# Spandan7724/Audio-Watermarking-Deep-Learning-Watermarks-for-Authenticating-Speech

Hardware: AMD Instinct MI355X
Metric: 1-s@16kHz clips/sec (gen+det+loss fwd-bwd) (higher is better)
Workload: dtype f32; 1 GPU; main16 train step: Generator+Detector+6 losses fwd-bwd + Adam, B=256 clips/GPU x 1 GPU, 1-s @ 16 kHz, message_bits=16 (BASELINE configs[2]); batch_per_gpu=256, global_batch=256, clip_len=16000, optimizer=fused flat Adam (wm_adam_step), parallelism=single

## Files before the change

### audio-watermarking-deep-learning-watermarks-for-authenticating-speech_amd/csrc/conv64.hpp

```cpp
#pragma once
#include "wm_common.hpp"
using namespace wm;
typedef _Float16 h16x2 __attribute__((ext_vector_type(2)));
typedef _Float16 h16x8 __attribute__((ext_vector_type(8)));
typedef float f32x2 __attribute__((ext_vector_type(2)));

#ifdef WM_STAMP
static __device__ unsigned long long* g_wm_stamp = nullptr;
#define STAMP(var) unsigned long long var = __builtin_amdgcn_s_memtime()
#define WM_STAMP_SETTER(name) int name(unsigned long long* buf) { return (int)hipMemcpyToSymbol(HIP_SYMBOL(g_wm_stamp), &buf, sizeof(buf)); }
#else
#define STAMP(var)
#define WM_STAMP_SETTER(name)
#endif

#ifndef WM_LOADPOS
#define WM_LOADPOS 1
#endif
#ifndef WM_LOAD_H
#define WM_LOAD_H 17
#endif
#ifndef WM_XCD_MAP
#define WM_XCD_MAP 1
#endif
#ifndef WM_TILE_CONTIG
#define WM_TILE_CONTIG 0
#endif
#ifndef WM_NT_STORE
#define WM_NT_STORE 0
#endif
#ifndef WM_BF3_MANUAL
#define WM_BF3_MANUAL 1
#endif
#ifndef WM_BF3_PIN_W
#define WM_BF3_PIN_W 1
#endif
#ifndef WM_BF7_PIPE
#define WM_BF7_PIPE 1
#endif
#ifndef WM_WGRAD_PIPE
#define WM_WGRAD_PIPE 1
#endif

namespace {
enum { PRO_NONE = 0, PRO_BNRELU = 1, PRO_ADDVEC = 2, PRO_BNBWD = 3 };
enum { EPI_BIAS = 0, EPI_RELUMASK = 1, EPI_ADD = 2, EPI_NONE = 3, EPI_BNADDRELU = 4,
       EPI_BIASELU = 5, EPI_BIASADDELU = 6, EPI_MULDELU = 7,
       EPI_ADDSTATS = 8 };

struct Conv64Args {
    const float* x;
    const float* x2;
    const float* wp;
    const float* pa;
    const float* pb;
    const float* pc;
    const float* bias;
    const float* e1;
    const float* ea;
    const float* eb;
    float* y;
    float* stats;
    int B, T;
};

template <int PRO>
__device__ __forceinline__ float pro_apply(float v, float v2, float ca, float cb, float cc, float cl = 0.f) {
    if (PRO == PRO_BNRELU) return fmaxf(fmaf(v, ca, cb), 0.f);
    if (PRO == PRO_ADDVEC) return v + ca;
    if (PRO == PRO_BNBWD) return fmaf(ca, v, fmaf(cc, v2, cb)) + cl;
    return v;
}

struct Wgrad64Args {
    const float* g;  const float* g2;
    const float* ga; const float* gb; const float* gc;
    const float* x;
    const float* xa; const float* xb;
    float* partial;
    int B, T;
};

__device__ __forceinline__ int xcd_slot() {
    const int g = gridDim.x, b = blockIdx.x;
    return (g & 7) ? b : (b & 7) * (g >> 3) + (b >> 3);
}

__device__ __forceinline__ void lds_barrier() {
    asm volatile("s_waitcnt lgkmcnt(0)\n\ts_barrier" ::: "memory");
}

__global__ __launch_bounds__(256) void wgrad64_reduce_kernel(const float* __restrict__ partial, int nparts, int KW, int mode,
                                                             float* __restrict__ dw, float* __restrict__ dbias, int accumulate) {
    __shared__ double sq[4][64];
    const int il = threadIdx.x & 63, grp = threadIdx.x >> 6, i = blockIdx.x * 64 + il;
    const int stride = KW * 4096 + 64;
    const int per = (nparts + 3) / 4, p0 = grp * per, p1 = min(p0 + per, nparts);
    double s0 = 0.0, s1 = 0.0;
    if (i < stride) {
        int p = p0;
        for (; p + 1 < p1; p += 2) {
            s0 += (double)partial[(size_t)p * stride + i];
            s1 += (double)partial[(size_t)(p + 1) * stride + i];
        }
        if (p < p1) s0 += (double)partial[(size_t)p * stride + i];
    }
    sq[grp][il] = s0 + s1;
    __syncthreads();
    if (grp != 0 || i >= stride) return;
    const float s = (float)((sq[0][il] + sq[1][il]) + (sq[2][il] + sq[3][il]));
    if (i < KW * 4096) {
        const int tap = i / 4096, out = (i / 64) % 64, in = i % 64;
        const int dst = (mode == 0) ? (out * 64 + in) * KW + tap : (in * 64 + out) * KW + (KW - 1 - tap);
        dw[dst] = accumulate ? dw[dst] + s : s;
    } else if (dbias) {
        const int c = i - KW * 4096;
        dbias[c] = accumulate ? dbias[c] + s : s;
    }
}
}
```

### audio-watermarking-deep-learning-watermarks-for-authenticating-speech_amd/csrc/conv64_fwd.hip

```cpp
#include "conv64.hpp"

namespace {

template <int PRO, int EPI, bool STATS>
__global__ __launch_bounds__(256) void conv64bf_kernel(Conv64Args a) {
    constexpr int KW = 3, PAD = 1, NT = 128, ROWS = NT + 2, PITCH = 72, NP = 3;
    constexpr int NC = 4;
    constexpr bool TWO = (PRO == PRO_BNBWD);
    constexpr bool E1 = (EPI == EPI_RELUMASK || EPI == EPI_ADD || EPI == EPI_BIASADDELU || EPI == EPI_MULDELU);
    constexpr bool HASBIAS = (EPI == EPI_BIAS || EPI == EPI_BIASELU || EPI == EPI_BIASADDELU);
    extern __shared__ __align__(16) unsigned char smem_raw[];
    unsigned short* Wb = reinterpret_cast<unsigned short*>(smem_raw);
    unsigned short* Xb = Wb + NP * KW * 64 * PITCH;
    float* Cs = reinterpret_cast<float*>(Xb + NP * ROWS * PITCH);
    const int tid = threadIdx.x, lane = tid & 63, wave = tid >> 6, half = lane >> 5, l31 = lane & 31;
    const int T = a.T;
    const int tilesPerClip = (T + NT - 1) / NT, ntiles = a.B * tilesPerClip;

    float4 sa[NC], sb[NC], sa2[TWO ? NC : 1], sb2[TWO ? NC : 1];
    float hl, hl2 = 0.f;
    auto combo = [&](int i, int& cp, int& q) {
        const int idx = tid + i * 256, widx = idx >> 6, l = idx & 63;
        cp = (widx & 3) * 8 + (l & 7);
        q = (widx >> 2) * 8 + (l >> 3);
// ... 61 lines not shown
    int tile = blockIdx.x;
    if (tile < ntiles) load_tile(tile);
    for (int i = tid; i < NP * KW * 64 * 8; i += 256) {
        const int row = i >> 3, seg = i & 7;
        *reinterpret_cast<uint4*>(Wb + row * PITCH + seg * 8) = reinterpret_cast<const uint4*>(a.wp)[i];
    }
    if (tid < 64) {
        Cs[tid] = (PRO == PRO_BNRELU || PRO == PRO_BNBWD) ? a.pa[tid] : 0.f;
        Cs[64 + tid] = (PRO == PRO_BNRELU || PRO == PRO_BNBWD) ? a.pb[tid] : 0.f;
        Cs[128 + tid] = (PRO == PRO_BNBWD) ? a.pc[tid] : 0.f;
        Cs[192 + tid] = (PRO == PRO_BNBWD) ? a.pb[64 + tid] : ((HASBIAS && a.bias) ? a.bias[tid] : 0.f);
        Cs[256 + tid] = (EPI == EPI_RELUMASK) ? a.ea[tid] : 0.f;
        Cs[320 + tid] = (EPI == EPI_RELUMASK) ? a.eb[tid] : 0.f;
    }
    __syncthreads();
    if (tile < ntiles) write_tile(tile);
    __syncthreads();

    float s1[STATS ? 32 : 1], s2[STATS ? 32 : 1];
    if (STATS) {
#pragma unroll
        for (int j = 0; j < 32; ++j) { s1[j] = 0.f; s2[j] = 0.f; }
    }
#ifdef WM_STAMP
    unsigned long long tm[6] = {0, 0, 0, 0, 0, 0};
#endif
    while (tile < ntiles) {
        STAMP(ts0);
        const int next = tile + gridDim.x;
        const int b = tile / tilesPerClip, t0 = (tile - b * tilesPerClip) * NT;
        const int tcol = t0 + wave * 32 + l31;
        float e1r[E1 ? 32 : 1];
        auto issue_loads = [&]() {
            if (next < ntiles) load_tile(next);
            if (E1) {
                const float* eb1 = a.e1 + (size_t)b * 64 * T + min(tcol, T - 1);
#pragma unroll
                for (int mt = 0; mt < 2; ++mt)
#pragma unroll
                    for (int r = 0; r < 16; ++r) e1r[mt * 16 + r] = eb1[(size_t)(mt * 32 + mfma_row(r, half)) * T];
            }
        };
        if (WM_LOADPOS == 0) issue_loads();
        STAMP(ts1);
        f32x16 acc[2];
#pragma unroll
        for (int mt = 0; mt < 2; ++mt)
#pragma unroll
            for (int r = 0; r < 16; ++r) acc[mt][r] = 0.f;
        const unsigned short* wbase = Wb + l31 * PITCH + 8 * half;
        const unsigned short* xbase = Xb + (wave * 32 + l31) * PITCH + 8 * half;
#pragma unroll 1
        for (int tap = 0; tap < KW; ++tap) {
            if (WM_LOADPOS > 0 && tap == WM_LOADPOS) issue_loads();
#pragma unroll
            for (int ch = 0; ch < 4; ++ch) {
                bf16x8 A[2][NP], Bf[NP];
#pragma unroll
                for (int p = 0; p < NP; ++p) {
                    Bf[p] = *reinterpret_cast<const bf16x8*>(xbase + (p * ROWS + tap) * PITCH + 16 * ch);
#pragma unroll
                    for (int mt = 0; mt < 2; ++mt)
                        A[mt][p] = *reinterpret_cast<const bf16x8*>(wbase + ((p * KW + tap) * 64 + mt * 32) * PITCH + 16 * ch);
                }
#pragma unroll
                for (int mt = 0; mt < 2; ++mt) {
                    acc[mt] = __builtin_amdgcn_mfma_f32_32x32x16_bf16(A[mt][1], Bf[1], acc[mt], 0, 0, 0);
                    acc[mt] = __builtin_amdgcn_mfma_f32_32x32x16_bf16(A[mt][0], Bf[2], acc[mt], 0, 0, 0);
                    acc[mt] = __builtin_amdgcn_mfma_f32_32x32x16_bf16(A[mt][2], Bf[0], acc[mt], 0, 0, 0);
                    acc[mt] = __builtin_amdgcn_mfma_f32_32x32x16_bf16(A[mt][0], Bf[1], acc[mt], 0, 0, 0);
                    acc[mt] = __builtin_amdgcn_mfma_f32_32x32x16_bf16(A[mt][1], Bf[0], acc[mt], 0, 0, 0);
                    acc[mt] = __builtin_amdgcn_mfma_f32_32x32x16_bf16(A[mt][0], Bf[0], acc[mt], 0, 0, 0);
                }
            }
        }
        STAMP(ts2);
        float* yb = a.y + (size_t)b * 64 * T + tcol;
        const bool ok = tcol < T;
#pragma unroll
        for (int mt = 0; mt < 2; ++mt)
#pragma unroll
            for (int r = 0; r < 16; ++r) {
                const int co = mt * 32 + mfma_row(r, half);
                float v = acc[mt][r];
                float q = 0.f;
                if (HASBIAS) v += Cs[192 + co];
                if (EPI == EPI_RELUMASK) { q = e1r[mt * 16 + r]; v = (fmaf(q, Cs[256 + co], Cs[320 + co]) > 0.f) ? v : 0.f; }
                if (EPI == EPI_ADD || EPI == EPI_BIASADDELU) v += e1r[mt * 16 + r];
                if (EPI == EPI_BIASELU || EPI == EPI_BIASADDELU) v = elu1(v);
                if (EPI == EPI_MULDELU) { const float yy = e1r[mt * 16 + r]; v *= (yy > 0.f ? 1.f : yy + 1.f); }
                if (ok) {
                    yb[(size_t)co * T] = v;
                    if (STATS) { s1[mt * 16 + r] += v; s2[mt * 16 + r] += (EPI == EPI_RELUMASK) ? v * q : v * v; }
                }
            }
        STAMP(ts3);
        __syncthreads();
        STAMP(ts4);
        if (next < ntiles) write_tile(next);
        STAMP(ts5);
        __syncthreads();
        STAMP(ts6);
#ifdef WM_STAMP
        tm[0] += ts1 - ts0; tm[1] += ts2 - ts1; tm[2] += ts3 - ts2; tm[3] += ts4 - ts3; tm[4] += ts5 - ts4; tm[5] += ts6 - ts5;
#endif
        tile = next;
    }
#ifdef WM_STAMP
    if (g_wm_stamp && lane == 0) {
        unsigned long long* d = g_wm_stamp + ((size_t)blockIdx.x * 4 + wave) * 6;
#pragma unroll
        for (int i = 0; i < 6; ++i) d[i] = tm[i];
    }
#endif
    if (STATS) {
        float* red = reinterpret_cast<float*>(Xb);
#pragma unroll
        for (int j = 0; j < 32; ++j) { s1[j] = half_wave_sum(s1[j]); s2[j] = half_wave_sum(s2[j]); }
        if (l31 == 0) {
#pragma unroll
            for (int mt = 0; mt < 2; ++mt)
#pragma unroll
                for (int r = 0; r < 16; ++r) {
                    const int co = mt * 32 + mfma_row(r, half);
                    red[wave * 128 + co] = s1[mt * 16 + r];
                    red[wave * 128 + 64 + co] = s2[mt * 16 + r];
                }
        }
        __syncthreads();
        if (tid < 128)
            a.stats[(size_t)blockIdx.x * 128 + tid] = red[tid] + red[128 + tid] + red[256 + tid] + red[384 + tid];
    }
}

template <int PRO, int EPI, bool STATS>
int launch_conv64bf(const Conv64Args& a, hipStream_t stream) {
    constexpr size_t lds = (size_t)(3 * 3 * 64 * 72 + 3 * 130 * 72) * 2 + 6 * 64 * sizeof(float);
    static wm::DevOnce attr_done;
    auto kern = conv64bf_kernel<PRO, EPI, STATS>;
    if (int rc = wm::lds_opt_in(reinterpret_cast<const void*>(kern), lds, attr_done)) return rc;
    const int ntiles = a.B * ((a.T + 127) / 128);
    const int grid = ntiles < kNumCU ? ntiles : kNumCU;
    if (STATS && grid < kNumCU) WM_TRY(hipMemsetAsync(a.stats, 0, sizeof(float) * 128 * kNumCU, stream));
    hipLaunchKernelGGL(kern, dim3(grid), dim3(256), lds, stream, a);
    WM_CHECK_LAUNCH();
    return 0;
}


template <int PRO, int EPI, bool STATS, bool H = false>
__global__ __launch_bounds__(256) void conv64bf3_kernel(Conv64Args a) {
    constexpr int KW = 3, NT = 128, ROWS = NT + 2, PITCH = 72, NP = H ? 2 : 3, NC = 4;
    constexpr int XBUF = NP * ROWS * PITCH;
    constexpr bool TWO = (PRO == PRO_BNBWD);
    constexpr bool E1 = (EPI == EPI_RELUMASK || EPI == EPI_ADD || EPI == EPI_BNADDRELU);
    extern __shared__ __align__(16) unsigned char smem_raw[];
    unsigned short* Xb0 = reinterpret_cast<unsigned short*>(smem_raw);
    float* Cs = reinterpret_cast<float*>(Xb0 + 2 * XBUF);
    const int tid = threadIdx.x, lane = tid & 63, half = lane >> 5, l31 = lane & 31;
    const int wave = __builtin_amdgcn_readfirstlane(tid >> 6);
    const int mt = wave & 1, nh = wave >> 1;
    const int T = a.T;
    const int tilesPerClip = (T + NT - 1) / NT, ntiles = a.B * tilesPerClip;

    u32x4 Wr[12][NP];
    {
        const uint4* wg = reinterpret_cast<const uint4*>(a.wp);
#pragma unroll
        for (int s = 0; s < 12; ++s)
#pragma unroll
            for (int p = 0; p < NP; ++p) {
                const int e = ((p * KW + (s >> 2)) * 64 + 32 * mt + l31) * 64 + 16 * (s & 3) + 8 * half;
                u32x4 w_ = __builtin_bit_cast(u32x4, wg[e >> 3]);
#if WM_BF3_PIN_W
                asm volatile("" : "+a"(w_));
#endif
                Wr[s][p] = w_;
            }
    }
    const float winv = H ? reinterpret_cast<const float*>(reinterpret_cast<const unsigned short*>(a.wp) + NP * KW * 4096)[1] : 1.f;
    const float wsc = H ? reinterpret_cast<const float*>(reinterpret_cast<const unsigned short*>(a.wp) + NP * KW * 4096)[0] : 1.f;
    const int cp = wave * 8 + (lane & 7), c0 = 2 * cp, q0 = lane >> 3;
    const int hc = (tid & 127) >> 1, hh = tid & 1;
    float4 sa[NC], sb[NC], sa2[TWO ? NC : 1], sb2[TWO ? NC : 1];
    float hl, hl2 = 0.f;
    auto load_combo = [&](int tile, int i) {
        const int b = tile / tilesPerClip, t0 = (tile - b * tilesPerClip) * NT;
        const size_t o = ((size_t)b * 64 + c0) * T + t0 + 4 * (q0 + 8 * i);
        sa[i] = *reinterpret_cast<const float4*>(a.x + o);
        sb[i] = *reinterpret_cast<const float4*>(a.x + o + T);
        if (TWO) { sa2[i] = *reinterpret_cast<const float4*>(a.x2 + o); sb2[i] = *reinterpret_cast<const float4*>(a.x2 + o + T); }
    };
    auto load_halo = [&](int tile) {
        const int b = tile / tilesPerClip, t0 = (tile - b * tilesPerClip) * NT;
        const int ht = min(max(hh ? t0 + NT : t0 - 1, 0), T - 1);
        hl = a.x[((size_t)b * 64 + hc) * T + ht];
        if (TWO) hl2 = a.x2[((size_t)b * 64 + hc) * T + ht];
    };
    auto load_tile = [&](int tile) {
#pragma unroll
        for (int i = 0; i < NC; ++i) load_combo(tile, i);
        load_halo(tile);
    };

#if WM_TILE_CONTIG
    const int chunk = (ntiles + (int)gridDim.x - 1) / (int)gridDim.x, tstep = 1;
    int tile = blockIdx.x * chunk;
    const int tend = min(tile + chunk, ntiles);
#else
    const int tstep = gridDim.x, tend = ntiles;
    int tile = WM_XCD_MAP ? xcd_slot() : (int)blockIdx.x;
#endif
    load_tile(min(tile, ntiles - 1));
    if (tid < 64) {
        Cs[tid] = (PRO == PRO_BNRELU || PRO == PRO_BNBWD) ? a.pa[tid] : 0.f;
        Cs[64 + tid] = (PRO == PRO_BNRELU || PRO == PRO_BNBWD) ? a.pb[tid] : 0.f;
        Cs[128 + tid] = (PRO == PRO_BNBWD) ? a.pc[tid] : 0.f;
        Cs[192 + tid] = (PRO == PRO_BNBWD) ? a.pb[64 + tid] : (((EPI == EPI_BIAS || EPI == EPI_BNADDRELU) && a.bias) ? a.bias[tid] : 0.f);
        Cs[256 + tid] = (EPI == EPI_RELUMASK || EPI == EPI_BNADDRELU) ? a.ea[tid] : 0.f;
        Cs[320 + tid] = (EPI == EPI_RELUMASK || EPI == EPI_BNADDRELU) ? a.eb[tid] : 0.f;
    }
    __syncthreads();
    const float ka0 = Cs[c0], ka1 = Cs[c0 + 1], kb0 = Cs[64 + c0], kb1 = Cs[64 + c0 + 1];
    const float kc0 = Cs[128 + c0], kc1 = Cs[128 + c0 + 1], kl0 = TWO ? Cs[192 + c0] : 0.f, kl1 = TWO ? Cs[192 + c0 + 1] : 0.f;
    const float ha = Cs[hc], hb = Cs[64 + hc], hcc = Cs[128 + hc], hlo = TWO ? Cs[192 + hc] : 0.f;

    auto split_unit = [&](unsigned* X32, int t0, int i, int e) {
        const float4 fa = sa[i], fb = sb[i];
        float va = (e == 0) ? fa.x : (e == 1) ? fa.y : (e == 2) ? fa.z : fa.w;
        float vb = (e == 0) ? fb.x : (e == 1) ? fb.y : (e == 2) ? fb.z : fb.w;
        if (PRO != PRO_NONE) {
            float wa = 0.f, wb = 0.f;
            if (TWO) {
                const float4 ga = sa2[i], gb = sb2[i];
                wa = (e == 0) ? ga.x : (e == 1) ? ga.y : (e == 2) ? ga.z : ga.w;
                wb = (e == 0) ? gb.x : (e == 1) ? gb.y : (e == 2) ? gb.z : gb.w;
            }
            va = pro_apply<PRO>(va, wa, ka0, kb0, kc0, kl0);
            vb = pro_apply<PRO>(vb, wb, ka1, kb1, kc1, kl1);
        }
        const int o = (1 + 4 * (q0 + 8 * i) + e) * (PITCH / 2) + cp;
        if (H) {
            const h16x2 h_ = __builtin_convertvector(f32x2{va, vb}, h16x2);
            const h16x2 l_ = __builtin_convertvector(f32x2{va - (float)h_.x, vb - (float)h_.y}, h16x2);
            X32[o] = __builtin_bit_cast(unsigned, h_); X32[(ROWS * PITCH >> 1) + o] = __builtin_bit_cast(unsigned, l_);
        } else {
            unsigned p0, p1, p2;
            split3_pair(va, vb, p0, p1, p2);
            X32[o] = p0; X32[(ROWS * PITCH >> 1) + o] = p1; X32[2 * (ROWS * PITCH >> 1) + o] = p2;
        }
    };
    auto split_halo = [&](unsigned short* X, int t0) {
        {
            const int t = hh ? t0 + NT : t0 - 1;
            float v = hl;
            if (PRO != PRO_NONE) v = pro_apply<PRO>(v, hl2, ha, hb, hcc, hlo);
            if (t < 0 || t >= T) v = 0.f;
            const int o = (hh ? NT + 1 : 0) * PITCH + hc;
            if (H) {
                const _Float16 h_ = (_Float16)v;
                const _Float16 l_ = (_Float16)(v - (float)h_);
                X[o] = __builtin_bit_cast(unsigned short, h_); X[ROWS * PITCH + o] = __builtin_bit_cast(unsigned short, l_);
            } else {
                unsigned p0, p1, p2;
                split3_pair(v, 0.f, p0, p1, p2);
                X[o] = (unsigned short)p0; X[ROWS * PITCH + o] = (unsigned short)p1; X[2 * ROWS * PITCH + o] = (unsigned short)p2;
            }
        }
    };
    float sva = 0.f, svb = 0.f;
    unsigned sp0 = 0, sp1 = 0;
    auto split_pick = [&](int i, int e) {
        const float4 fa = sa[i], fb = sb[i];
        float va = (e == 0) ? fa.x : (e == 1) ? fa.y : (e == 2) ? fa.z : fa.w;
        float vb = (e == 0) ? fb.x : (e == 1) ? fb.y : (e == 2) ? fb.z : fb.w;
        if (PRO != PRO_NONE) {
            float wa = 0.f, wb = 0.f;
            if (TWO) {
                const float4 ga = sa2[i], gb = sb2[i];
                wa = (e == 0) ? ga.x : (e == 1) ? ga.y : (e == 2) ? ga.z : ga.w;
                wb = (e == 0) ? gb.x : (e == 1) ? gb.y : (e == 2) ? gb.z : gb.w;
            }
            va = pro_apply<PRO>(va, wa, ka0, kb0, kc0, kl0);
            vb = pro_apply<PRO>(vb, wb, ka1, kb1, kc1, kl1);
        }
        sva = va; svb = vb;
        asm volatile("" : "+v"(sva), "+v"(svb));
    };
    auto split_st1 = [&]() {
        if (H) {
            const h16x2 hh_ = __builtin_convertvector(f32x2{sva, svb}, h16x2);
            sp0 = __builtin_bit_cast(unsigned, hh_);
            sva -= (float)hh_.x; svb -= (float)hh_.y;
        } else {
            const bf16x2 hh_ = {(__bf16)sva, (__bf16)svb};
            sp0 = __builtin_bit_cast(unsigned, hh_);
            sva -= __uint_as_float(sp0 << 16); svb -= __uint_as_float(sp0 & 0xffff0000u);
        }
        asm volatile("" : "+v"(sva), "+v"(svb), "+v"(sp0));
    };
    auto split_st2 = [&]() {
        if (H) return;
        const bf16x2 mm_ = {(__bf16)sva, (__bf16)svb};
        sp1 = __builtin_bit_cast(unsigned, mm_);
        sva -= __uint_as_float(sp1 << 16); svb -= __uint_as_float(sp1 & 0xffff0000u);
        asm volatile("" : "+v"(sva), "+v"(svb), "+v"(sp1));
    };
    auto last_piece = [&]() -> unsigned {
        if (H) return __builtin_bit_cast(unsigned, __builtin_convertvector(f32x2{sva, svb}, h16x2));
        const bf16x2 ll_ = {(__bf16)sva, (__bf16)svb};
        return __builtin_bit_cast(unsigned, ll_);
    };
    auto split_out = [&](unsigned* X32, int i, int e) {
        const unsigned sp2 = last_piece();
        const int o = (1 + 4 * (q0 + 8 * i) + e) * (PITCH / 2) + cp;
        X32[o] = sp0; if (!H) X32[(ROWS * PITCH >> 1) + o] = sp1; X32[(NP - 1) * (ROWS * PITCH >> 1) + o] = sp2;
    };
    auto halo_pick = [&](int t0) {
        const int t = hh ? t0 + NT : t0 - 1;
        float v = hl;
        if (PRO != PRO_NONE) v = pro_apply<PRO>(v, hl2, ha, hb, hcc, hlo);
        if (t < 0 || t >= T) v = 0.f;
        sva = v; svb = 0.f;
        asm volatile("" : "+v"(sva), "+v"(svb));
    };
    auto halo_out = [&](unsigned short* X) {
        const unsigned sp2 = last_piece();
        const int o = (hh ? NT + 1 : 0) * PITCH + hc;
        X[o] = (unsigned short)sp0; if (!H) X[ROWS * PITCH + o] = (unsigned short)sp1; X[(NP - 1) * ROWS * PITCH + o] = (unsigned short)sp2;
    };
    {
        const int t0 = (min(tile, ntiles - 1) % tilesPerClip) * NT;
#pragma unroll
        for (int u = 0; u < 16; ++u) split_unit(reinterpret_cast<unsigned*>(Xb0), t0, u >> 2, u & 3);
        split_halo(Xb0, t0);
    }
    load_tile(min(tile + tstep, ntiles - 1));
    __syncthreads();
    __builtin_amdgcn_s_waitcnt(0x0F70);

    float s1[STATS ? 16 : 1], s2[STATS ? 16 : 1];
    if (STATS) {
#pragma unroll
        for (int j = 0; j < 16; ++j) { s1[j] = 0.f; s2[j] = 0.f; }
    }
    int buf = 0;
#ifdef WM_STAMP
    unsigned long long tm[6] = {0, 0, 0, 0, 0, 0};
#endif
    f32x16 accp[2];
    int pb_ = min(tile, ntiles - 1) / tilesPerClip, pt0 = (min(tile, ntiles - 1) % tilesPerClip) * NT;
    bool any_tile = false;
    float e1r[E1 ? 32 : 1];
    constexpr bool KB = (EPI == EPI_BIAS || EPI == EPI_BNADDRELU), KE = (EPI == EPI_RELUMASK || EPI == EPI_BNADDRELU);
    float kbias[KB ? 16 : 1], kea[KE ? 16 : 1], keb[KE ? 16 : 1];
#pragma unroll
    for (int r = 0; r < 16; ++r) {
        const int co = 32 * mt + mfma_row(r, half);
        if (KB) kbias[r] = Cs[192 + co];
        if (KE) { kea[r] = Cs[256 + co]; keb[r] = Cs[320 + co]; }
    }
#pragma unroll
    for (int nt = 0; nt < 2; ++nt)
#pragma unroll
        for (int r = 0; r < 16; ++r) accp[nt][r] = (EPI == EPI_BIAS) ? -kbias[r] * wsc : 0.f;
    const unsigned lcol = (unsigned)(4 * half * T + l31) * 4u;
    unsigned rowT[16];
#pragma unroll
    for (int r = 0; r < 16; ++r) rowT[r] = (unsigned)(((r & 3) + 8 * (r >> 2)) * T) * 4u;
    auto row_srd = [&](const float* base, int cb) { return make_srd(base + ((size_t)cb * 64 + 32 * mt) * T, (size_t)32 * T * sizeof(float)); };
    wm_srd_t syp = row_srd(a.y, pb_);
    unsigned vcolp = lcol + (unsigned)(pt0 + 64 * nh) * 4u;
    if (E1) {
#pragma unroll
        for (int j = 0; j < 32; ++j) e1r[j] = 0.f;
    }
    auto epi_value = [&](int idx, bool fetch, const wm_srd_t& se1c, unsigned vcolc) {
        const int nt = idx >> 4, r = idx & 15;
        float v = accp[nt][r];
        float q = 0.f;
        if (H) v *= winv;
        if (EPI == EPI_BIAS) v += kbias[r];
        if (EPI == EPI_RELUMASK) { q = e1r[idx]; v = (fmaf(q, kea[r], keb[r]) > 0.f) ? v : 0.f; }
        if (EPI == EPI_ADD) v += e1r[idx];
        if (EPI == EPI_BNADDRELU) v = fmaxf(e1r[idx] + fmaf(v + kbias[r], kea[r], keb[r]), 0.f);
        buf_store(syp, v, vcolp + 128u * nt, rowT[r]);
        if (STATS) { s1[r] += v; s2[r] = fmaf(v, (EPI == EPI_RELUMASK) ? q : v, s2[r]); }
#if WM_BF3_MANUAL
        if (STATS) asm volatile("" : "+v"(s1[r]), "+v"(s2[r]));
#endif
        if (E1 && fetch) e1r[idx] = buf_load(se1c, vcolc + 128u * nt, rowT[r]);
    };
    auto mma = [&](const u32x4& A_, const u32x4& B_, f32x16 c) -> f32x16 {
        if (H) return __builtin_amdgcn_mfma_f32_32x32x16_f16(__builtin_bit_cast(h16x8, A_), __builtin_bit_cast(h16x8, B_), c, 0, 0, 0);
        return __builtin_amdgcn_mfma_f32_32x32x16_bf16(__builtin_bit_cast(bf16x8, A_), __builtin_bit_cast(bf16x8, B_), c, 0, 0, 0);
    };
    while (tile < tend) {
        STAMP(ts0);
        const int next = min(tile + tstep, ntiles - 1), next2 = min(tile + 2 * tstep, ntiles - 1);
        const int b = tile / tilesPerClip, t0 = (tile - b * tilesPerClip) * NT;
        const int nt0 = (next % tilesPerClip) * NT;
        const wm_srd_t se1c = E1 ? row_srd(a.e1, b) : syp;
        const unsigned vcolc = lcol + (unsigned)(t0 + 64 * nh) * 4u;
        const unsigned short* xcur = Xb0 + buf * XBUF;
        unsigned short* xnxt = Xb0 + (buf ^ 1) * XBUF;
        f32x16 acc[2];
#pragma unroll
        for (int nt = 0; nt < 2; ++nt)
#pragma unroll
            for (int r = 0; r < 16; ++r) acc[nt][r] = 0.f;
        const unsigned short* xrow = xcur + (64 * nh + l31) * PITCH + 8 * half;
        u32x4 Bq[2][NP];
#pragma unroll
        for (int p = 0; p < NP; ++p) Bq[0][p] = *reinterpret_cast<const u32x4*>(xrow + p * ROWS * PITCH);
#if WM_BF3_MANUAL
#define FENCE __builtin_amdgcn_sched_barrier(0)
#define BF3_SLICE(k)                                                                                                        \
    {                                                                                                                           \
        if (h < 16) {                                                                                                           \
            if ((k) == 0) split_pick(h >> 2, h & 3);                                                                            \
            if ((k) == 1) split_st1();                                                                                          \
            if ((k) == 2) split_st2();                                                                                          \
            if ((k) == 3) { split_out(reinterpret_cast<unsigned*>(xnxt), h >> 2, h & 3); if ((h & 3) == 3) load_combo(next2, h >> 2); } \
        } else if (h == 16) {                                                                                                   \
            if ((k) == 0) halo_pick(nt0);                                                                                       \
            if ((k) == 1) split_st1();                                                                                          \
            if ((k) == 2) split_st2();                                                                                          \
            if ((k) == 3) halo_out(xnxt);                                                                                       \
        } else if (h == 17) {                                                                                                   \
            if ((k) == 0) load_halo(next2);                                                                                     \
        }                                                                                                                       \
        if (h < 8) {                                                                                                            \
            if ((k) == 4) epi_value(2 * h, true, se1c, vcolc);                                                                              \
            if ((k) == 5) epi_value(2 * h + 1, true, se1c, vcolc);                                                                          \
        } else if ((k) == 4) epi_value(8 + h, true, se1c, vcolc);                                                                           \
    }
#pragma unroll
        for (int h = 0; h < 24; ++h) {
            const int s = h >> 1, nt = h & 1;
            if (h + 1 < 24) {
                const int s1_ = (h + 1) >> 1, n1 = (h + 1) & 1;
#pragma unroll
                for (int p = 0; p < NP; ++p)
                    Bq[(h + 1) & 1][p] = *reinterpret_cast<const u32x4*>(xrow + (p * ROWS + 32 * n1 + (s1_ >> 2)) * PITCH + 16 * (s1_ & 3));
            }
            const u32x4* Bf = Bq[h & 1];
            FENCE;
            if (H) {
                acc[nt] = mma(Wr[s][1], Bf[0], acc[nt]); FENCE; BF3_SLICE(0) FENCE; BF3_SLICE(1) FENCE;
                acc[nt] = mma(Wr[s][0], Bf[1], acc[nt]); FENCE; BF3_SLICE(3) FENCE; BF3_SLICE(4) FENCE;
                acc[nt] = mma(Wr[s][0], Bf[0], acc[nt]); FENCE; BF3_SLICE(5) FENCE;
            } else {
                acc[nt] = mma(Wr[s][1], Bf[1], acc[nt]); FENCE; BF3_SLICE(0) FENCE;
                acc[nt] = mma(Wr[s][0], Bf[2], acc[nt]); FENCE; BF3_SLICE(1) FENCE;
                acc[nt] = mma(Wr[s][2], Bf[0], acc[nt]); FENCE; BF3_SLICE(2) FENCE;
                acc[nt] = mma(Wr[s][0], Bf[1], acc[nt]); FENCE; BF3_SLICE(3) FENCE;
                acc[nt] = mma(Wr[s][1], Bf[0], acc[nt]); FENCE; BF3_SLICE(4) FENCE;
                acc[nt] = mma(Wr[s][0], Bf[0], acc[nt]); FENCE; BF3_SLICE(5) FENCE;
            }
#ifdef WM_STAMP
#ifdef WM_STAMP_FINE
            if (h == 16) { STAMP(tsa); tm[0] += tsa - ts0; }
            if (h == 17) { STAMP(tsb); tm[1] += tsb - ts0; }
            if (h == 18) { STAMP(tsb); tm[3] += tsb - ts0; }
            if (h == 20) { STAMP(tsb); tm[5] += tsb - ts0; }
#else
            if (h == 3) { STAMP(tsa); tm[0] += tsa - ts0; }
            if (h == 15) { STAMP(tsb); tm[1] += tsb - ts0; }
#endif
#endif
        }
#undef FENCE
#undef BF3_SLICE
#else
#pragma unroll
        for (int h = 0; h < 24; ++h) {
            const int s = h >> 1, nt = h & 1;
            if (h + 1 < 24) {
                const int s1_ = (h + 1) >> 1, n1 = (h + 1) & 1;
#pragma unroll
                for (int p = 0; p < NP; ++p)
                    Bq[(h + 1) & 1][p] = *reinterpret_cast<const u32x4*>(xrow + (p * ROWS + 32 * n1 + (s1_ >> 2)) * PITCH + 16 * (s1_ & 3));
            }
            const u32x4* Bf = Bq[h & 1];
            static_assert(!H, "the f16 build exists in the hand-pinned schedule only");
            acc[nt] = mma(Wr[s][1], Bf[1], acc[nt]);
            acc[nt] = mma(Wr[s][0], Bf[2], acc[nt]);
            acc[nt] = mma(Wr[s][2], Bf[0], acc[nt]);
            acc[nt] = mma(Wr[s][0], Bf[1], acc[nt]);
            acc[nt] = mma(Wr[s][1], Bf[0], acc[nt]);
            acc[nt] = mma(Wr[s][0], Bf[0], acc[nt]);
            if (h < 16) {
                split_unit(reinterpret_cast<unsigned*>(xnxt), nt0, h >> 2, h & 3);
                if ((h & 3) == 3) load_combo(next2, h >> 2);
            } else if (h == 16) split_halo(xnxt, nt0);
            else if (h == 17) load_halo(next2);
            if (h < 8) { epi_value(2 * h, true, se1c, vcolc); epi_value(2 * h + 1, true, se1c, vcolc); }
            else epi_value(8 + h, true, se1c, vcolc);
            __builtin_amdgcn_sched_group_barrier(0x100, 3, 0);
#pragma unroll
            for (int kk = 0; kk < 6; ++kk) {
                __builtin_amdgcn_sched_group_barrier(0x008, 1, 0);
                __builtin_amdgcn_sched_group_barrier(0x002, 5, 0);
                __builtin_amdgcn_sched_group_barrier(0x200, 1, 0);
                __builtin_amdgcn_sched_group_barrier(0x020, 1, 0);
                __builtin_amdgcn_sched_group_barrier(0x040, 1, 0);
            }
            __builtin_amdgcn_sched_barrier(0);
#ifdef WM_STAMP
#ifdef WM_STAMP_FINE
            if (h == 16) { STAMP(tsa); tm[0] += tsa - ts0; }
            if (h == 17) { STAMP(tsb); tm[1] += tsb - ts0; }
            if (h == 18) { STAMP(tsb); tm[3] += tsb - ts0; }
            if (h == 20) { STAMP(tsb); tm[5] += tsb - ts0; }
#else
            if (h == 3) { STAMP(tsa); tm[0] += tsa - ts0; }
            if (h == 15) { STAMP(tsb); tm[1] += tsb - ts0; }
#endif
#endif
        }
#endif
        STAMP(ts1);
        accp[0] = acc[0]; accp[1] = acc[1];
        pb_ = b; pt0 = t0; any_tile = true;
        syp = row_srd(a.y, b); vcolp = vcolc;
        STAMP(ts2);
        lds_barrier();
        STAMP(ts3);
#ifdef WM_STAMP
#ifdef WM_STAMP_FINE
        tm[2] += ts1 - ts0; tm[4] += ts3 - ts2;
#else
        tm[2] += ts1 - ts0; tm[3] += ts2 - ts1; tm[4] += ts3 - ts2;
#endif
#endif
        tile += tstep;
        buf ^= 1;
    }
#ifdef WM_STAMP
    if (g_wm_stamp && lane == 0) {
        unsigned long long* d = g_wm_stamp + ((size_t)blockIdx.x * 4 + wave) * 6;
#pragma unroll
        for (int i = 0; i < 6; ++i) d[i] = tm[i];
    }
#endif
    if (any_tile) {
#pragma unroll
        for (int idx = 0; idx < 32; ++idx) epi_value(idx, false, syp, 0u);
    }
    if (STATS) {
        float* red = reinterpret_cast<float*>(Xb0);
#pragma unroll
        for (int j = 0; j < 16; ++j) { s1[j] = half_wave_sum(s1[j]); s2[j] = half_wave_sum(s2[j]); }
        __syncthreads();
        if (l31 == 0) {
#pragma unroll
            for (int r = 0; r < 16; ++r) {
                const int co = 32 * mt + mfma_row(r, half);
                red[nh * 128 + co] = s1[r];
                red[nh * 128 + 64 + co] = s2[r];
            }
        }
        __syncthreads();
        if (tid < 128) a.stats[(size_t)blockIdx.x * 128 + tid] = red[tid] + red[128 + tid];
    }
}

template <int PRO, int EPI, bool STATS, bool H = false>
int launch_conv64bf3(const Conv64Args& a, hipStream_t stream) {
    constexpr size_t lds = (size_t)(2 * (H ? 2 : 3) * 130 * 72) * 2 + 6 * 64 * sizeof(float);
    static wm::DevOnce attr_done;
    auto kern = conv64bf3_kernel<PRO, EPI, STATS, H>;
    if (int rc = wm::lds_opt_in(reinterpret_cast<const void*>(kern), lds, attr_done)) return rc;
    const int ntiles = a.B * ((a.T + 127) / 128);
    const int grid = ntiles < kNumCU ? ntiles : kNumCU;
    if (STATS && grid < kNumCU) WM_TRY(hipMemsetAsync(a.stats, 0, sizeof(float) * 128 * kNumCU, stream));
    hipLaunchKernelGGL(kern, dim3(grid), dim3(256), lds, stream, a);
    WM_CHECK_LAUNCH();
    return 0;
}

__global__ void pack_w64_bf_kernel(const float* __restrict__ w, const float* __restrict__ row_scale,
                                   unsigned short* __restrict__ wpb, int mode) {
    const int i = blockIdx.x * blockDim.x + threadIdx.x;
    if (i >= 3 * 4096) return;
    const int tap = i / 4096, out = (i / 64) % 64, in = i % 64;
    float v = (mode == 0) ? w[(out * 64 + in) * 3 + tap] : w[(in * 64 + out) * 3 + (2 - tap)];
    if (row_scale) v *= row_scale[out];
    unsigned p0, p1, p2;
    split3_pair(v, 0.f, p0, p1, p2);
    wpb[i] = (unsigned short)p0; wpb[3 * 4096 + i] = (unsigned short)p1; wpb[2 * 3 * 4096 + i] = (unsigned short)p2;
}

__global__ __launch_bounds__(1024) void pack_w64_h_kernel(const float* __restrict__ w, const float* __restrict__ row_scale,
                                                          unsigned short* __restrict__ wph, int mode) {
    __shared__ float red[16];
    float v[12];
    float mx = 0.f;
#pragma unroll
    for (int j = 0; j < 12; ++j) {
        const int i = threadIdx.x + 1024 * j, tap = i / 4096, out = (i / 64) % 64, in = i % 64;
        v[j] = (mode == 0) ? w[(out * 64 + in) * 3 + tap] : w[(in * 64 + out) * 3 + (2 - tap)];
        if (row_scale) v[j] *= row_scale[out];
        mx = fmaxf(mx, fabsf(v[j]));
    }
#pragma unroll
    for (int o = 32; o > 0; o >>= 1) mx = fmaxf(mx, __shfl_xor(mx, o));
    if ((threadIdx.x & 63) == 0) red[threadIdx.x >> 6] = mx;
    __syncthreads();
    float m = 0.f;
#pragma unroll
    for (int i = 0; i < 16; ++i) m = fmaxf(m, red[i]);
    float ws = 1.f;
    if (m > 0.f && m < 3.0e38f) ws = exp2f(floorf(log2f(1023.f / m)));
    ws = fminf(fmaxf(ws, 1.0e-30f), 1.0e30f);
    if (threadIdx.x == 0) {
        float* tail = reinterpret_cast<float*>(wph + 2 * 3 * 4096);
        tail[0] = ws; tail[1] = 1.f / ws;
    }
#pragma unroll
    for (int j = 0; j < 12; ++j) {
        const int i = threadIdx.x + 1024 * j;
        const float x = v[j] * ws;
        const _Float16 hi = (_Float16)x;
        const _Float16 lo = (_Float16)(x - (float)hi);
        wph[i] = __builtin_bit_cast(unsigned short, hi);
        wph[3 * 4096 + i] = __builtin_bit_cast(unsigned short, lo);
    }
}

}

extern "C" {

WM_STAMP_SETTER(wm_debug_set_stamp_buffer)

int wm_pack_w64_bf(const float* w, void* wpb, int mode, hipStream_t stream) {
    if (mode < 0 || mode > 1) return (int)hipErrorInvalidValue;
    hipLaunchKernelGGL(pack_w64_bf_kernel, dim3(48), dim3(256), 0, stream, w, (const float*)nullptr, reinterpret_cast<unsigned short*>(wpb), mode);
    WM_CHECK_LAUNCH();
    return 0;
}
int wm_pack_w64_bf_scaled(const float* w, const float* row_scale, void* wpb, hipStream_t stream) {
    if (!w || !row_scale || !wpb) return (int)hipErrorInvalidValue;
    hipLaunchKernelGGL(pack_w64_bf_kernel, dim3(48), dim3(256), 0, stream, w, row_scale, reinterpret_cast<unsigned short*>(wpb), 0);
    WM_CHECK_LAUNCH();
    return 0;
}

static int g_bf_schedule = 2;
int wm_set_conv_bf_schedule(int schedule, hipStream_t) { g_bf_schedule = (schedule == 2) ? 2 : 0; return 0; }

int wm_conv64_bf(const float* x, const float* x2, const void* wpb, const float* pa, const float* pb, const float* pc,
                 const float* bias, const float* e1, const float* ea, const float* eb, float* y, float* stats,
                 int B, int T, int pro, int epi, int arith, hipStream_t stream) {
    if (B <= 0 || T <= 0 || (T & 3)) return (int)hipErrorInvalidValue;
    Conv64Args a{x, x2, reinterpret_cast<const float*>(wpb), pa, pb, pc, bias, e1, ea, eb, y, stats, B, T};
    const bool st = stats != nullptr;
    if (arith == 1) {
        if (g_bf_schedule != 2 || (T & 127)) return (int)hipErrorInvalidValue;
        if (pro == PRO_BNRELU && epi == EPI_BNADDRELU && !st) return launch_conv64bf3<PRO_BNRELU, EPI_BNADDRELU, false, true>(a, stream);
        if (epi != EPI_BIAS) return (int)hipErrorInvalidValue;
        if (pro == PRO_NONE) return st ? launch_conv64bf3<PRO_NONE, EPI_BIAS, true, true>(a, stream) : launch_conv64bf3<PRO_NONE, EPI_BIAS, false, true>(a, stream);
        if (pro == PRO_BNRELU) return st ? launch_conv64bf3<PRO_BNRELU, EPI_BIAS, true, true>(a, stream) : launch_conv64bf3<PRO_BNRELU, EPI_BIAS, false, true>(a, stream);
        return (int)hipErrorInvalidValue;
    }
    if (arith != 0) return (int)hipErrorInvalidValue;
    if (pro == PRO_NONE && !st) {
        if (epi == EPI_BIASELU) return launch_conv64bf<PRO_NONE, EPI_BIASELU, false>(a, stream);
        if (epi == EPI_BIASADDELU) return launch_conv64bf<PRO_NONE, EPI_BIASADDELU, false>(a, stream);
        if (epi == EPI_MULDELU) return launch_conv64bf<PRO_NONE, EPI_MULDELU, false>(a, stream);
        if (epi == EPI_ADD) return launch_conv64bf<PRO_NONE, EPI_ADD, false>(a, stream);
        if (epi == EPI_NONE) return launch_conv64bf<PRO_NONE, EPI_NONE, false>(a, stream);
    }
    if (g_bf_schedule == 2 && (T & 127) == 0) {
        if (pro == PRO_BNRELU && epi == EPI_BNADDRELU && !st) return launch_conv64bf3<PRO_BNRELU, EPI_BNADDRELU, false>(a, stream);
        if (pro == PRO_NONE && epi == EPI_BIAS) return st ? launch_conv64bf3<PRO_NONE, EPI_BIAS, true>(a, stream) : launch_conv64bf3<PRO_NONE, EPI_BIAS, false>(a, stream);
        if (pro == PRO_BNRELU && epi == EPI_BIAS) return st ? launch_conv64bf3<PRO_BNRELU, EPI_BIAS, true>(a, stream) : launch_conv64bf3<PRO_BNRELU, EPI_BIAS, false>(a, stream);
        if (pro == PRO_BNBWD && epi == EPI_RELUMASK && st) return launch_conv64bf3<PRO_BNBWD, EPI_RELUMASK, true>(a, stream);
        if (pro == PRO_BNBWD && epi == EPI_ADD && !st) return launch_conv64bf3<PRO_BNBWD, EPI_ADD, false>(a, stream);
        if (pro == PRO_BNBWD && epi == EPI_NONE && !st) return launch_conv64bf3<PRO_BNBWD, EPI_NONE, false>(a, stream);
        return (int)hipErrorInvalidValue;
    }
    if (pro == PRO_NONE && epi == EPI_BIAS) return st ? launch_conv64bf<PRO_NONE, EPI_BIAS, true>(a, stream) : launch_conv64bf<PRO_NONE, EPI_BIAS, false>(a, stream);
    if (pro == PRO_BNRELU && epi == EPI_BIAS) return st ? launch_conv64bf<PRO_BNRELU, EPI_BIAS, true>(a, stream) : launch_conv64bf<PRO_BNRELU, EPI_BIAS, false>(a, stream);
    if (pro == PRO_BNBWD && epi == EPI_RELUMASK && st) return launch_conv64bf<PRO_BNBWD, EPI_RELUMASK, true>(a, stream);
    if (pro == PRO_BNBWD && epi == EPI_ADD && !st) return launch_conv64bf<PRO_BNBWD, EPI_ADD, false>(a, stream);
    if (pro == PRO_BNBWD && epi == EPI_NONE && !st) return launch_conv64bf<PRO_BNBWD, EPI_NONE, false>(a, stream);
    return (int)hipErrorInvalidValue;
}

int wm_pack_w64_h(const float* w, void* wph, int mode, hipStream_t stream) {
    if (!w || !wph || mode < 0 || mode > 1) return (int)hipErrorInvalidValue;
    hipLaunchKernelGGL(pack_w64_h_kernel, dim3(1), dim3(1024), 0, stream, w, (const float*)nullptr, reinterpret_cast<unsigned short*>(wph), mode);
    WM_CHECK_LAUNCH();
    return 0;
}
int wm_pack_w64_h_scaled(const float* w, const float* row_scale, void* wph, hipStream_t stream) {
    if (!w || !row_scale || !wph) return (int)hipErrorInvalidValue;
    hipLaunchKernelGGL(pack_w64_h_kernel, dim3(1), dim3(1024), 0, stream, w, row_scale, reinterpret_cast<unsigned short*>(wph), 0);
    WM_CHECK_LAUNCH();
    return 0;
}

}
```

### audio-watermarking-deep-learning-watermarks-for-authenticating-speech_amd/csrc/lstm.hip

```cpp
#include "wm_common.hpp"
#include <type_traits>
using namespace wm;

namespace {

#ifdef WM_STAMP
__device__ unsigned long long* g_lstm_stamp = nullptr;
#define LSTAMP(var, val) unsigned long long var; asm volatile("s_memtime %0\n\ts_waitcnt lgkmcnt(0)" : "=s"(var), "+v"(val))
#define LSTAMP_ACC(i, a, b) tm[i] += (b) - (a)
#else
#define LSTAMP(var, val)
#define LSTAMP_ACC(i, a, b)
#endif

__device__ __forceinline__ int gate_row(int np) { return (np & 3) * 64 + (np >> 2); }

typedef float v2f __attribute__((ext_vector_type(2)));
template <int K>
__device__ __forceinline__ float quad_bcast(float v) {
    constexpr int ctrl = K | (K << 2) | (K << 4) | (K << 6);
    return __int_as_float(__builtin_amdgcn_update_dpp(0, __float_as_int(v), ctrl, 0xf, 0xf, false));
}

__global__ __launch_bounds__(256) void lstm_xproj_kernel(const float* __restrict__ x, const float* __restrict__ w_ih,
// ... 230 lines not shown
    const int q = lane & 3, ul = lane >> 2, u = wave * 16 + ul, n = q * 64 + u, np = wave * 64 + lane;
    float wr[64];
#pragma unroll
    for (int k = 0; k < 64; k += 4) {
        const float4 v = *reinterpret_cast<const float4*>(w_hh + n * 64 + k);
        wr[k] = v.x; wr[k + 1] = v.y; wr[k + 2] = v.z; wr[k + 3] = v.w;
    }
    bf16x8 Wi[2][4][NP];
#pragma unroll
    for (int mt = 0; mt < 2; ++mt)
#pragma unroll
        for (int ks = 0; ks < 4; ++ks) {
            const float* wp = w_ih + gate_row(wave * 64 + mt * 32 + l31) * 64 + 16 * ks + 8 * half;
            const float4 v0 = *reinterpret_cast<const float4*>(wp), v1 = *reinterpret_cast<const float4*>(wp + 4);
            unsigned a[4], m[4], l[4];
            split3_pair(v0.x, v0.y, a[0], m[0], l[0]); split3_pair(v0.z, v0.w, a[1], m[1], l[1]);
            split3_pair(v1.x, v1.y, a[2], m[2], l[2]); split3_pair(v1.z, v1.w, a[3], m[3], l[3]);
            Wi[mt][ks][0] = __builtin_bit_cast(bf16x8, make_uint4(a[0], a[1], a[2], a[3]));
            Wi[mt][ks][1] = __builtin_bit_cast(bf16x8, make_uint4(m[0], m[1], m[2], m[3]));
            Wi[mt][ks][2] = __builtin_bit_cast(bf16x8, make_uint4(l[0], l[1], l[2], l[3]));
        }
    const float bias = b_ih[n] + b_hh[n];
    if (tid < 128) hsm[tid] = 0.f;
    float c = 0.f;
    const wm_srd_t sgb = make_srd(SAVE ? gates + (size_t)b * T * 256 : hout, SAVE ? (size_t)T * 256 * sizeof(float) : 0);
    const wm_srd_t scb = make_srd(SAVE ? cst + (size_t)b * T * 64 : hout, SAVE ? (size_t)T * 64 * sizeof(float) : 0);
    const wm_srd_t shb = make_srd(hout + (size_t)b * 64 * T, (size_t)64 * T * sizeof(float));
    const unsigned vgb = (unsigned)np * 4u, vcb = (q == 1) ? (unsigned)u * 4u : 0xFFFFFF00u;
    const unsigned vhb = (unsigned)(u * T + 4 * q) * 4u;
    float* hb = hout + ((size_t)b * 64 + u) * T;
    const bool is_g = (q == 2);

    const int cp = wave * 8 + (lane & 7), tq = lane >> 3;
    const float* xc = x + ((size_t)b * 64 + 2 * cp) * T + 4 * tq;
    float4 sa, sb;
    auto load_x = [&](int t0) {
        const int t = min(t0, T - 4 - 4 * tq);
        sa = *reinterpret_cast<const float4*>(xc + max(t, -4 * tq));
        sb = *reinterpret_cast<const float4*>(xc + T + max(t, -4 * tq));
    };
    auto split_x = [&]() {
        unsigned* X32 = reinterpret_cast<unsigned*>(Xb);
        const float va[4] = {sa.x, sa.y, sa.z, sa.w}, vb[4] = {sb.x, sb.y, sb.z, sb.w};
#pragma unroll
        for (int e = 0; e < 4; ++e) {
            unsigned p0, p1, p2;
            split3_pair(va[e], vb[e], p0, p1, p2);
            const int o = (4 * tq + e) * (PITCH / 2) + cp;
            X32[o] = p0; X32[CH * PITCH / 2 + o] = p1; X32[2 * (CH * PITCH / 2) + o] = p2;
        }
    };
    f32x16 acc[2];
    bf16x8 Bf[NP];
    auto mfma_one = [&](int idx) {
        const int m = idx / 6, pr = idx % 6, ks = m >> 1, mt = m & 1;
        const int pa = (pr == 0 || pr == 4) ? 1 : (pr == 2 ? 2 : 0), pb = (pr == 0 || pr == 3) ? 1 : (pr == 1 ? 2 : 0);
        if (mt == 0 && pr == 0) {
#pragma unroll
            for (int p = 0; p < NP; ++p) Bf[p] = *reinterpret_cast<const bf16x8*>(Xb + (p * CH + l31) * PITCH + 16 * ks + 8 * half);
        }
        if (ks == 0 && pr == 0) {
#pragma unroll
            for (int r = 0; r < 16; ++r) acc[mt][r] = 0.f;
        }
        acc[mt] = __builtin_amdgcn_mfma_f32_32x32x16_bf16(Wi[mt][ks][pa], Bf[pb], acc[mt], 0, 0, 0);
    };
    auto store_xp = [&](int buf) {
        float* dst = xps + (buf * CH + l31) * XPP + wave * 64 + 4 * half;
#pragma unroll
        for (int mt = 0; mt < 2; ++mt)
#pragma unroll
            for (int r = 0; r < 16; ++r) dst[mt * 32 + (r & 3) + 8 * (r >> 2)] = acc[mt][r];
    };

    load_x(0);
    __syncthreads();
    split_x();
    load_x(CH);
    __syncthreads();
#pragma unroll
    for (int i = 0; i < 48; ++i) mfma_one(i);
    store_xp(0);
    __syncthreads();

    float hk[4];
    int t0 = 0, cbuf = 0;
#ifdef WM_STAMP
    unsigned long long tm[6] = {0, 0, 0, 0, 0, 0};
#endif
    auto run8 = [&](auto sub_c) {
        constexpr int SUB = decltype(sub_c)::value;
#pragma unroll
        for (int j8 = 0; j8 < 8; ++j8) {
            const int s = SUB * 8 + j8;
            const int t = t0 + s;
            if (s == 0) { split_x(); load_x(t0 + 2 * CH); }
            if (s >= 2 && s < 26) mfma_one(2 * (s - 2));
            if (s == 28) store_xp(cbuf ^ 1);
            if (t < T) {
                LSTAMP(ls0, c);
                const float xin = xps[(cbuf * CH + s) * XPP + np] + bias;
                const float* hcur = hsm + (s & 1) * 64;
                const float4 hq4 = *reinterpret_cast<const float4*>(hcur + 4 * (lane & 15));
                float Hh[4] = {hq4.x, hq4.y, hq4.z, hq4.w};
                float hv = Hh[0];
                LSTAMP(ls1, hv);
                Hh[0] = hv;
                if (s >= 2 && s < 26) mfma_one(2 * (s - 2) + 1);
                float pre = dot64_rowbcast(Hh, wr, xin);
                LSTAMP(ls2, pre);
                float act = gate_act(pre, is_g);
                LSTAMP(ls3, act);
                const float gi = quad_bcast<0>(act), gf = quad_bcast<1>(act), gg = quad_bcast<2>(act), go = quad_bcast<3>(act);
                c = fmaf(gf, c, gi * gg);
                float h = go * tanh_s(c);
                LSTAMP(ls4, h);
                hsm[((s + 1) & 1) * 64 + rowbcast_slot(u)] = h;
                if (SAVE) {
                    buf_store(sgb, act, vgb, (unsigned)t * 1024u);
                    buf_store(scb, c, vcb, (unsigned)t * 256u);
                }
                if (((s >> 2) & 3) == q) hk[s & 3] = h;
                if ((s & 15) == 15)
                    buf_store4(shb, f32x4{hk[0], hk[1], hk[2], hk[3]}, vhb, (unsigned)(t0 + (s - 15)) * 4u);
                LSTAMP(ls5, h);
                __syncthreads();
                LSTAMP(ls6, c);
                LSTAMP_ACC(0, ls0, ls1); LSTAMP_ACC(1, ls1, ls2); LSTAMP_ACC(2, ls2, ls3); LSTAMP_ACC(3, ls3, ls4);
                LSTAMP_ACC(4, ls4, ls5); LSTAMP_ACC(5, ls5, ls6);
            }
        }
    };
    for (; t0 < T; t0 += CH, cbuf ^= 1) {
        run8(std::integral_constant<int, 0>{});
        run8(std::integral_constant<int, 1>{});
        run8(std::integral_constant<int, 2>{});
        run8(std::integral_constant<int, 3>{});
        if (t0 + CH > T && (T & 15)) {
            const int g0 = (T >> 4) << 4, tq0 = g0 + 4 * q;
#pragma unroll
            for (int j = 0; j < 4; ++j)
                if (tq0 + j < T) hb[tq0 + j] = hk[j];
        }
    }
#ifdef WM_STAMP
    if (g_lstm_stamp && lane == 0) {
        unsigned long long* d = g_lstm_stamp + ((size_t)blockIdx.x * 4 + wave) * 6;
#pragma unroll
        for (int i = 0; i < 6; ++i) d[i] = tm[i];
    }
#endif
}

template <bool SAVE>
__global__ __launch_bounds__(512) void lstm_fwd_ws_kernel(const float* __restrict__ x, const float* __restrict__ w_ih,
                                                          const float* __restrict__ b_ih, const float* __restrict__ b_hh,
                                                          const float* __restrict__ w_hh, float* __restrict__ hout,
                                                          float* __restrict__ gates, float* __restrict__ cst, int T) {
    constexpr int CH = 32, XPP = 257, PITCH = 72, NP = 3;
    extern __shared__ __align__(16) unsigned char smem_raw[];
    float* xps = reinterpret_cast<float*>(smem_raw);
    unsigned short* Xb = reinterpret_cast<unsigned short*>(xps + 2 * CH * XPP);
    float* hsm = reinterpret_cast<float*>(Xb + NP * CH * PITCH);
    const int b = blockIdx.x, tid = threadIdx.x, lane = tid & 63, half = lane >> 5, l31 = lane & 31;
    const int wave = __builtin_amdgcn_readfirstlane(tid >> 6);
    if (wave < 4) {
        __builtin_amdgcn_s_setprio(3);
        const int q = lane & 3, ul = lane >> 2, u = wave * 16 + ul, n = q * 64 + u, np = wave * 64 + lane;
        float wr[64];
#pragma unroll
        for (int k = 0; k < 64; k += 4) {
            const float4 v = *reinterpret_cast<const float4*>(w_hh + n * 64 + k);
            wr[k] = v.x; wr[k + 1] = v.y; wr[k + 2] = v.z; wr[k + 3] = v.w;
        }
        const float bias = b_ih[n] + b_hh[n];
        if (tid < 128) hsm[tid] = 0.f;
        float c = 0.f;
        const wm_srd_t sgb = make_srd(SAVE ? gates + (size_t)b * T * 256 : hout, SAVE ? (size_t)T * 256 * sizeof(float) : 0);
        const wm_srd_t scb = make_srd(SAVE ? cst + (size_t)b * T * 64 : hout, SAVE ? (size_t)T * 64 * sizeof(float) : 0);
        const wm_srd_t shb = make_srd(hout + (size_t)b * 64 * T, (size_t)64 * T * sizeof(float));
        const unsigned vgb = (unsigned)np * 4u, vcb = (q == 1) ? (unsigned)u * 4u : 0xFFFFFF00u;
        const unsigned vhb = (unsigned)(u * T + 4 * q) * 4u;
        float* hb = hout + ((size_t)b * 64 + u) * T;
        const bool is_g = (q == 2);
        __syncthreads(); __syncthreads(); __syncthreads();
        float hk[4];
        int t0 = 0, cbuf = 0;
        auto run8 = [&](auto sub_c) {
            constexpr int SUB = decltype(sub_c)::value;
#pragma unroll
            for (int j8 = 0; j8 < 8; ++j8) {
                const int s = SUB * 8 + j8;
                const int t = t0 + s;
                if (t < T) {
                    const float xin = xps[(cbuf * CH + s) * XPP + np] + bias;
                    const float* hcur = hsm + (s & 1) * 64;
                    const float4 hq4 = *reinterpret_cast<const float4*>(hcur + 4 * (lane & 15));
                    const float Hh[4] = {hq4.x, hq4.y, hq4.z, hq4.w};
                    const float pre = dot64_rowbcast(Hh, wr, xin);
                    const float act = gate_act(pre, is_g);
                    const float gi = quad_bcast<0>(act), gf = quad_bcast<1>(act), gg = quad_bcast<2>(act), go = quad_bcast<3>(act);
                    c = fmaf(gf, c, gi * gg);
                    const float h = go * tanh_s(c);
                    hsm[((s + 1) & 1) * 64 + rowbcast_slot(u)] = h;
                    if (SAVE) {
                        buf_store(sgb, act, vgb, (unsigned)t * 1024u);
                        buf_store(scb, c, vcb, (unsigned)t * 256u);
                    }
                    if (((s >> 2) & 3) == q) hk[s & 3] = h;
                    if ((s & 15) == 15)
                        buf_store4(shb, f32x4{hk[0], hk[1], hk[2], hk[3]}, vhb, (unsigned)(t0 + (s - 15)) * 4u);
                    __syncthreads();
                }
            }
        };
        for (; t0 < T; t0 += CH, cbuf ^= 1) {
            run8(std::integral_constant<int, 0>{});
            run8(std::integral_constant<int, 1>{});
            run8(std::integral_constant<int, 2>{});
            run8(std::integral_constant<int, 3>{});
            if (t0 + CH > T && (T & 15)) {
                const int g0 = (T >> 4) << 4, tq0 = g0 + 4 * q;
#pragma unroll
                for (int j = 0; j < 4; ++j)
                    if (tq0 + j < T) hb[tq0 + j] = hk[j];
            }
        }
        return;
    }
    const int hw = wave - 4;
    bf16x8 Wi[2][4][NP];
#pragma unroll
    for (int mt = 0; mt < 2; ++mt)
#pragma unroll
        for (int ks = 0; ks < 4; ++ks) {
            const float* wp = w_ih + gate_row(hw * 64 + mt * 32 + l31) * 64 + 16 * ks + 8 * half;
            const float4 v0 = *reinterpret_cast<const float4*>(wp), v1 = *reinterpret_cast<const float4*>(wp + 4);
            unsigned a[4], m[4], l[4];
            split3_pair(v0.x, v0.y, a[0], m[0], l[0]); split3_pair(v0.z, v0.w, a[1], m[1], l[1]);
            split3_pair(v1.x, v1.y, a[2], m[2], l[2]); split3_pair(v1.z, v1.w, a[3], m[3], l[3]);
            Wi[mt][ks][0] = __builtin_bit_cast(bf16x8, make_uint4(a[0], a[1], a[2], a[3]));
            Wi[mt][ks][1] = __builtin_bit_cast(bf16x8, make_uint4(m[0], m[1], m[2], m[3]));
            Wi[mt][ks][2] = __builtin_bit_cast(bf16x8, make_uint4(l[0], l[1], l[2], l[3]));
        }
    const int cp = hw * 8 + (lane & 7), tq = lane >> 3;
    const float* xc = x + ((size_t)b * 64 + 2 * cp) * T + 4 * tq;
    float4 sa, sb;
    auto load_x = [&](int t0) {
        const int t = min(t0, T - 4 - 4 * tq);
        sa = *reinterpret_cast<const float4*>(xc + max(t, -4 * tq));
        sb = *reinterpret_cast<const float4*>(xc + T + max(t, -4 * tq));
    };
    auto split_x = [&]() {
        unsigned* X32 = reinterpret_cast<unsigned*>(Xb);
        const float va[4] = {sa.x, sa.y, sa.z, sa.w}, vb[4] = {sb.x, sb.y, sb.z, sb.w};
#pragma unroll
        for (int e = 0; e < 4; ++e) {
            unsigned p0, p1, p2;
            split3_pair(va[e], vb[e], p0, p1, p2);
            const int o = (4 * tq + e) * (PITCH / 2) + cp;
            X32[o] = p0; X32[CH * PITCH / 2 + o] = p1; X32[2 * (CH * PITCH / 2) + o] = p2;
        }
    };
    f32x16 acc[2];
    bf16x8 Bf[NP];
    auto mfma_one = [&](int idx) {
        const int m = idx / 6, pr = idx % 6, ks = m >> 1, mt = m & 1;
        const int pa = (pr == 0 || pr == 4) ? 1 : (pr == 2 ? 2 : 0), pb = (pr == 0 || pr == 3) ? 1 : (pr == 1 ? 2 : 0);
        if (mt == 0 && pr == 0) {
#pragma unroll
            for (int p = 0; p < NP; ++p) Bf[p] = *reinterpret_cast<const bf16x8*>(Xb + (p * CH + l31) * PITCH + 16 * ks + 8 * half);
        }
        if (ks == 0 && pr == 0) {
#pragma unroll
            for (int r = 0; r < 16; ++r) acc[mt][r] = 0.f;
        }
        acc[mt] = __builtin_amdgcn_mfma_f32_32x32x16_bf16(Wi[mt][ks][pa], Bf[pb], acc[mt], 0, 0, 0);
    };
    auto store_xp = [&](int buf) {
        float* dst = xps + (buf * CH + l31) * XPP + hw * 64 + 4 * half;
#pragma unroll
        for (int mt = 0; mt < 2; ++mt)
#pragma unroll
            for (int r = 0; r < 16; ++r) dst[mt * 32 + (r & 3) + 8 * (r >> 2)] = acc[mt][r];
    };
    load_x(0);
    __syncthreads();
    split_x();
    load_x(CH);
    __syncthreads();
#pragma unroll
    for (int i = 0; i < 48; ++i) mfma_one(i);
    store_xp(0);
    __syncthreads();
    int cbuf = 0;
    for (int t0 = 0; t0 < T; t0 += CH, cbuf ^= 1) {
#pragma unroll
        for (int s = 0; s < CH; ++s) {
            if (s == 0) { split_x(); load_x(t0 + 2 * CH); }
            if (s >= 1 && s <= 24) { mfma_one(2 * (s - 1)); mfma_one(2 * (s - 1) + 1); }
            if (s == 26) store_xp(cbuf ^ 1);
            if (t0 + s < T) __syncthreads();
        }
    }
}

__global__ __launch_bounds__(256) void lstm_bwd_kernel(float* __restrict__ gates, const float* __restrict__ cst,
                                                       const float* __restrict__ dh_out, const float* __restrict__ w_hh,
                                                       int T) {
    __builtin_amdgcn_s_setprio(3);
    __shared__ __align__(16) float part[2][64][4];
    const int b = blockIdx.x, tid = threadIdx.x, lane = tid & 63, wave = tid >> 6;
    const int q = lane & 3, ul = lane >> 2, u = wave * 16 + ul, np = wave * 64 + lane;
    float wt[64];
#pragma unroll
    for (int j = 0; j < 64; ++j) wt[j] = w_hh[((j & 3) * 64 + wave * 16 + (j >> 2)) * 64 + lane];
    if (tid < 512 / 4) reinterpret_cast<float4*>(&part[0][0][0])[tid] = make_float4(0.f, 0.f, 0.f, 0.f);
    float dc = 0.f;
    const wm_srd_t sgb = make_srd(gates + (size_t)b * T * 256, (size_t)T * 256 * sizeof(float));
    const wm_srd_t scb = make_srd(cst + (size_t)b * T * 64, (size_t)T * 64 * sizeof(float));
    const wm_srd_t sdh = make_srd(dh_out + (size_t)b * 64 * T, (size_t)64 * T * sizeof(float));
    const unsigned vgb = (unsigned)np * 4u, vcb = (unsigned)u * 4u, vdh = (unsigned)(u * T) * 4u;

    constexpr int CH = 8;
    struct Buf { float ga[CH], cc[CH + 1], dh[CH]; };
    Buf A, Bf;
    auto prefetch = [&](Buf& f, int t1) {
#pragma unroll
        for (int j = 0; j < CH; ++j) {
            const int t = max(t1 - CH + 1 + j, 0);
            f.ga[j] = buf_load(sgb, vgb, (unsigned)t * 1024u);
            f.dh[j] = buf_load(sdh, vdh, (unsigned)t * 4u);
        }
#pragma unroll
        for (int j = 0; j <= CH; ++j) f.cc[j] = buf_load(scb, vcb, (unsigned)max(t1 - CH + j, 0) * 256u);
    };
    const bool is0 = q == 0, is1 = q == 1, is2 = q == 2, is3 = q == 3;
    int pb = 0;
#ifdef WM_STAMP
    unsigned long long tm[6] = {0, 0, 0, 0, 0, 0};
#endif
    auto run_chunk = [&](const Buf& f, int t1) {
#pragma unroll
        for (int jj = 0; jj < CH; ++jj) {
            const int j = CH - 1 - jj, t = t1 - jj;
            if (t >= 0) {
                LSTAMP(ls0, dc);
                const float4 p = *reinterpret_cast<const float4*>(&part[pb][u][0]);
                const float act = f.ga[j];
                const float gi = quad_bcast<0>(act), gf = quad_bcast<1>(act), gg = quad_bcast<2>(act), go = quad_bcast<3>(act);
                const float tc = tanh_s(f.cc[j + 1]);
                const float cprev = (t >= 1) ? f.cc[j] : 0.f;
                const float S = is0 ? gg : (is1 ? cprev : (is2 ? gi : tc));
                const float D = is2 ? fmaf(-act, act, 1.f) : act * (1.f - act);
                const float M = S * D;
                const float K = go * fmaf(-tc, tc, 1.f);
                float dht = f.dh[j] + ((p.x + p.y) + (p.z + p.w));
                LSTAMP(ls1, dht);
                const float dct = fmaf(dht, K, dc);
                float da = (is3 ? dht : dct) * M;
                dc = dct * gf;
                LSTAMP(ls2, da);
                buf_store(sgb, da, vgb, (unsigned)t * 1024u);
                float Dd[4];
                rows_replicate(da, Dd);
                float psum = dot64_rowbcast(Dd, wt);
                LSTAMP(ls3, psum);
                part[pb ^ 1][lane][wave] = psum;
                pb ^= 1;
                LSTAMP(ls4, psum);
                __syncthreads();
                LSTAMP(ls5, dc);
                LSTAMP_ACC(0, ls0, ls1); LSTAMP_ACC(1, ls1, ls2); LSTAMP_ACC(2, ls2, ls3); LSTAMP_ACC(3, ls3, ls4); LSTAMP_ACC(4, ls4, ls5);
            }
        }
    };
    prefetch(A, T - 1);
    __syncthreads();
    for (int t1 = T - 1; t1 >= 0; t1 -= 2 * CH) {
        prefetch(Bf, t1 - CH);
        run_chunk(A, t1);
        prefetch(A, t1 - 2 * CH);
        run_chunk(Bf, t1 - CH);
    }
#ifdef WM_STAMP
    if (g_lstm_stamp && lane == 0) {
        unsigned long long* d = g_lstm_stamp + ((size_t)blockIdx.x * 4 + wave) * 6;
#pragma unroll
        for (int i = 0; i < 6; ++i) d[i] = tm[i];
    }
#endif
}

__global__ __launch_bounds__(512) void lstm_bwd_ws_kernel(float* __restrict__ gates, const float* __restrict__ cst,
                                                          const float* __restrict__ dh_out, const float* __restrict__ w_hh,
                                                          const float* __restrict__ x, const float* __restrict__ hseq,
                                                          float* __restrict__ partial, int T) {
    constexpr int CT = 32, PT = 36;
    extern __shared__ __align__(16) unsigned char smem_raw[];
    float* daT = reinterpret_cast<float*>(smem_raw);
    float (*part)[64][4] = reinterpret_cast<float (*)[64][4]>(daT + 2 * 256 * PT);
    const int b = blockIdx.x, tid = threadIdx.x, lane = tid & 63;
    const int wave = __builtin_amdgcn_readfirstlane(tid >> 6);
    float* out = partial + (size_t)b * (256 * 128 + 256);
    if (wave < 4) {
        __builtin_amdgcn_s_setprio(3);
        const int q = lane & 3, ul = lane >> 2, u = wave * 16 + ul, np = wave * 64 + lane;
        float wt[64];
#pragma unroll
        for (int j = 0; j < 64; ++j) wt[j] = w_hh[((j & 3) * 64 + wave * 16 + (j >> 2)) * 64 + lane];
        if (tid < 512 / 4) reinterpret_cast<float4*>(&part[0][0][0])[tid] = make_float4(0.f, 0.f, 0.f, 0.f);
        float dc = 0.f, dbs = 0.f;
        const wm_srd_t sgb = make_srd(gates + (size_t)b * T * 256, (size_t)T * 256 * sizeof(float));
        const wm_srd_t scb = make_srd(cst + (size_t)b * T * 64, (size_t)T * 64 * sizeof(float));
        const wm_srd_t sdh = make_srd(dh_out + (size_t)b * 64 * T, (size_t)64 * T * sizeof(float));
        const unsigned vgb = (unsigned)np * 4u, vcb = (unsigned)u * 4u, vdh = (unsigned)(u * T) * 4u;
        constexpr int CH = 8;
        struct Buf { float ga[CH], cc[CH + 1], dh[CH]; };
        Buf A, Bf;
        auto prefetch = [&](Buf& f, int t1) {
#pragma unroll
            for (int j = 0; j < CH; ++j) {
                const int t = max(t1 - CH + 1 + j, 0);
                f.ga[j] = buf_load(sgb, vgb, (unsigned)t * 1024u);
                f.dh[j] = buf_load(sdh, vdh, (unsigned)t * 4u);
            }
#pragma unroll
            for (int j = 0; j <= CH; ++j) f.cc[j] = buf_load(scb, vcb, (unsigned)max(t1 - CH + j, 0) * 256u);
        };
        const bool is0 = q == 0, is1 = q == 1, is2 = q == 2, is3 = q == 3;
        int pb = 0;
        auto run_chunk = [&](const Buf& f, int t1) {
            float dav[CH];
#pragma unroll
            for (int jj = 0; jj < CH; ++jj) {
                const int j = CH - 1 - jj, t = t1 - jj;
                const float4 p = *reinterpret_cast<const float4*>(&part[pb][u][0]);
                const float act = f.ga[j];
                const float gi = quad_bcast<0>(act), gf = quad_bcast<1>(act), gg = quad_bcast<2>(act), go = quad_bcast<3>(act);
                const float tc = tanh_s(f.cc[j + 1]);
                const float cprev = (t >= 1) ? f.cc[j] : 0.f;
                const float S = is0 ? gg : (is1 ? cprev : (is2 ? gi : tc));
                const float D = is2 ? fmaf(-act, act, 1.f) : act * (1.f - act);
                const float M = S * D;
                const float K = go * fmaf(-tc, tc, 1.f);
                const float dht = f.dh[j] + ((p.x + p.y) + (p.z + p.w));
                const float dct = fmaf(dht, K, dc);
                const float da = (is3 ? dht : dct) * M;
                dc = dct * gf;
                dav[j] = da;
                buf_store(sgb, da, vgb, (unsigned)t * 1024u);
                float Dd[4];
                rows_replicate(da, Dd);
                const float psum = dot64_rowbcast(Dd, wt);
// ... 537 lines not shown
        } else {
            const int k = p & 1, i = tid + k * 256, j = i >> 3, q = i & 7;
            const size_t row = ((size_t)b * 64 + j) * T;
            if (p < 10) sx[k] = *reinterpret_cast<const float4*>(x + row + min(t0 + 4 * q, T - 4));
            else {
#pragma unroll
                for (int e = 0; e < 4; ++e) sh[k][e] = h[row + min(max(t0 + 4 * q + e - 1, 0), T - 1)];
            }
        }
    };
    auto put4 = [&](unsigned short* d, int stride_p, float v0, float v1, float v2, float v3) {
        unsigned a0, a1, a2, b0, b1, b2;
        split3_pair(v0, v1, a0, a1, a2);
        split3_pair(v2, v3, b0, b1, b2);
        *reinterpret_cast<uint2*>(d) = make_uint2(a0, b0);
        *reinterpret_cast<uint2*>(d + stride_p) = make_uint2(a1, b1);
        *reinterpret_cast<uint2*>(d + 2 * stride_p) = make_uint2(a2, b2);
    };
    auto write_tile = [&](int tile) {
        const int t0 = (tile % tilesPerClip) * NT;
#pragma unroll
        for (int p = 0; p < 8; ++p) {
            const int tt = (tid >> 6) + 4 * p;
            float4 v = sd[p];
            if (t0 + tt >= T) v = make_float4(0.f, 0.f, 0.f, 0.f);
            bs[0] += v.x; bs[1] += v.y; bs[2] += v.z; bs[3] += v.w;
            put4(Dd + tt * PDD + 4 * (tid & 63), NT * PDD, v.x, v.y, v.z, v.w);
        }
#pragma unroll
        for (int k = 0; k < 2; ++k) {
            const int i = tid + k * 256, j = i >> 3, q = i & 7;
            put4(Zb + j * PZ + 4 * q, 128 * PZ, sx[k].x, sx[k].y, sx[k].z, sx[k].w);
            float hv[4];
#pragma unroll
            for (int e = 0; e < 4; ++e) hv[e] = (t0 + 4 * q + e - 1 >= 0) ? sh[k][e] : 0.f;
            put4(Zb + (64 + j) * PZ + 4 * q, 128 * PZ, hv[0], hv[1], hv[2], hv[3]);
        }
    };
    int tile = blockIdx.x;
#pragma unroll
    for (int p = 0; p < 12; ++p) load_piece(min(tile, ntiles - 1), p);
    __syncthreads();
    write_tile(min(tile, ntiles - 1));
    __syncthreads();
    while (tile < ntiles) {
        const int next = tile + gridDim.x, nextc = min(next, ntiles - 1);
#pragma unroll
        for (int kb = 0; kb < 2; ++kb) {
            const int e0 = kb * 16 + 8 * half;
            bf16x8 Bf[4][NP];
#pragma unroll
            for (int nt = 0; nt < 4; ++nt)
#pragma unroll
                for (int p = 0; p < NP; ++p)
                    Bf[nt][p] = *reinterpret_cast<const bf16x8*>(Zb + (p * 128 + nt * 32 + l31) * PZ + e0);
#pragma unroll
            for (int mt = 0; mt < 2; ++mt) {
                bf16x8 A[NP];
#pragma unroll
                for (int p = 0; p < NP; ++p) {
                    const unsigned short* col = Dd + (p * NT + e0) * PDD + wave * 64 + mt * 32 + l31;
                    unsigned w[4];
#pragma unroll
                    for (int j = 0; j < 4; ++j) w[j] = (unsigned)col[(2 * j) * PDD] | ((unsigned)col[(2 * j + 1) * PDD] << 16);
                    A[p] = __builtin_bit_cast(bf16x8, make_uint4(w[0], w[1], w[2], w[3]));
                }
#pragma unroll
                for (int nt = 0; nt < 4; ++nt) {
                    acc[mt][nt] = mfma_bf16x6(A, Bf[nt], acc[mt][nt]);
                    if ((kb * 2 + mt) * 4 + nt < 12) load_piece(nextc, (kb * 2 + mt) * 4 + nt);
                }
            }
        }
        __syncthreads();
        if (next < ntiles) write_tile(next);
        __syncthreads();
        tile = next;
    }
    float* out = partial + (size_t)blockIdx.x * (256 * 128 + 256);
#pragma unroll
    for (int mt = 0; mt < 2; ++mt)
#pragma unroll
        for (int nt = 0; nt < 4; ++nt)
#pragma unroll
            for (int r = 0; r < 16; ++r)
                out[(wave * 64 + mt * 32 + mfma_row(r, half)) * 128 + nt * 32 + l31] = acc[mt][nt][r];
    float* red = reinterpret_cast<float*>(smem_raw);
    __syncthreads();
#pragma unroll
    for (int e = 0; e < 4; ++e) red[(tid >> 6) * 256 + 4 * (tid & 63) + e] = bs[e];
    __syncthreads();
    out[256 * 128 + tid] = (red[tid] + red[256 + tid]) + (red[512 + tid] + red[768 + tid]);
}

constexpr int kWgradSlab = 256 * 128 + 256;
__global__ __launch_bounds__(512) void lstm_wgrad_reduce_kernel(const float* __restrict__ partial, int nparts, float* dw_ih,
                                                                float* dw_hh, float* db_ih, float* db_hh, int accumulate) {
    __shared__ double sq[8][64];
    const int i = blockIdx.x * 64 + (threadIdx.x & 63);
    const float s = (float)column_sum_d<8>(partial, nparts, (size_t)kWgradSlab, i, true, sq);
    if (threadIdx.x >= 64) return;
    if (i < 256 * 128) {
        const int n = gate_row(i >> 7), j = i & 127;
        float* dst = (j < 64) ? dw_ih + n * 64 + j : dw_hh + n * 64 + (j - 64);
        *dst = accumulate ? *dst + s : s;
    } else {
        const int n = gate_row(i - 256 * 128);
        db_ih[n] = accumulate ? db_ih[n] + s : s;
        db_hh[n] = accumulate ? db_hh[n] + s : s;
    }
}
static_assert(kWgradSlab % 64 == 0, "lstm_wgrad_reduce_kernel: whole 64-column blocks");

}

extern "C" {

#ifdef WM_STAMP
int wm_debug_set_lstm_stamp_buffer(unsigned long long* buf) {
    return (int)hipMemcpyToSymbol(HIP_SYMBOL(g_lstm_stamp), &buf, sizeof(buf));
}
#endif

int wm_lstm_xproj(const float* x, const float* w_ih, const float* b_ih, const float* b_hh, float* xp, int B, int T,
                  hipStream_t stream) {
    if (T & 3) return (int)hipErrorInvalidValue;
    hipLaunchKernelGGL(lstm_xproj_kernel, dim3(B * ((T + 127) / 128)), dim3(256), 0, stream, x, w_ih, b_ih, b_hh, xp, T);
    WM_CHECK_LAUNCH();
    return 0;
}

int wm_lstm_fwd(const float* xp, const float* w_hh, float* hout, float* gates, float* cst, int B, int T, hipStream_t stream) {
    if (T & 3) return (int)hipErrorInvalidValue;
    if (gates && cst) hipLaunchKernelGGL(lstm_fwd_kernel<true>, dim3(B), dim3(256), 0, stream, xp, w_hh, hout, gates, cst, T);
    else hipLaunchKernelGGL(lstm_fwd_kernel<false>, dim3(B), dim3(256), 0, stream, xp, w_hh, hout, gates, cst, T);
    WM_CHECK_LAUNCH();
    return 0;
}

static int g_lstm_fwd_ws = 1;
int wm_set_lstm_fwd_wave_specialised(int on, hipStream_t) { g_lstm_fwd_ws = on ? 1 : 0; return 0; }

int wm_lstm_fwd_fused(const float* x, const float* w_ih, const float* b_ih, const float* b_hh, const float* w_hh, float* hout,
                      float* gates, float* cst, int B, int T, hipStream_t stream) {
    if ((T & 3) || T < 8) return (int)hipErrorInvalidValue;
    constexpr size_t lds = (size_t)2 * 32 * 257 * sizeof(float) + (size_t)3 * 32 * 72 * 2 + 128 * sizeof(float);
    static wm::DevOnce done[2];
    if (int rc = wm::lds_opt_in(reinterpret_cast<const void*>(lstm_fwd_fused_kernel<true>), lds, done[0])) return rc;
    if (int rc = wm::lds_opt_in(reinterpret_cast<const void*>(lstm_fwd_fused_kernel<false>), lds, done[1])) return rc;
    if (g_lstm_fwd_ws) {
        static wm::DevOnce donew[2];
        if (int rc = wm::lds_opt_in(reinterpret_cast<const void*>(lstm_fwd_ws_kernel<true>), lds, donew[0])) return rc;
        if (int rc = wm::lds_opt_in(reinterpret_cast<const void*>(lstm_fwd_ws_kernel<false>), lds, donew[1])) return rc;
        if (gates && cst) hipLaunchKernelGGL(lstm_fwd_ws_kernel<true>, dim3(B), dim3(512), lds, stream, x, w_ih, b_ih, b_hh, w_hh, hout, gates, cst, T);
        else hipLaunchKernelGGL(lstm_fwd_ws_kernel<false>, dim3(B), dim3(512), lds, stream, x, w_ih, b_ih, b_hh, w_hh, hout, gates, cst, T);
        WM_CHECK_LAUNCH();
        return 0;
    }
    if (gates && cst) hipLaunchKernelGGL(lstm_fwd_fused_kernel<true>, dim3(B), dim3(256), lds, stream, x, w_ih, b_ih, b_hh, w_hh, hout, gates, cst, T);
    else hipLaunchKernelGGL(lstm_fwd_fused_kernel<false>, dim3(B), dim3(256), lds, stream, x, w_ih, b_ih, b_hh, w_hh, hout, gates, cst, T);
    WM_CHECK_LAUNCH();
    return 0;
}

int wm_lstm_bwd(float* gates, const float* cst, const float* dh_out, const float* w_hh, int B, int T, hipStream_t stream) {
    hipLaunchKernelGGL(lstm_bwd_kernel, dim3(B), dim3(256), 0, stream, gates, cst, dh_out, w_hh, T);
    WM_CHECK_LAUNCH();
    return 0;
}

int wm_lstm_bwd_fused(float* gates, const float* cst, const float* dh_out, const float* w_hh, const float* w_ih, float* dx,
                      int B, int T, hipStream_t stream) {
    if ((T & 3) || T < 4) return (int)hipErrorInvalidValue;
    constexpr size_t lds = (size_t)2 * 4 * 3 * 32 * 72 * 2 + (size_t)(4 * 64 * 33 + 4 * 64 + 2 * 64 * 4) * sizeof(float);
    static wm::DevOnce done;
    if (int rc = wm::lds_opt_in(reinterpret_cast<const void*>(lstm_bwd_fused_kernel), lds, done)) return rc;
    hipLaunchKernelGGL(lstm_bwd_fused_kernel, dim3(B), dim3(256), lds, stream, gates, cst, dh_out, w_hh, w_ih, dx, T);
    WM_CHECK_LAUNCH();
    return 0;
}

int wm_lstm_bwd_wgrad(float* gates, const float* cst, const float* dh_out, const float* w_hh, const float* x, const float* h,
                      float* partial, float* dw_ih, float* dw_hh, float* db_ih, float* db_hh, int B, int T, int accumulate,
                      hipStream_t stream) {
    if (B <= 0 || (T & 31) || T < 64) return (int)hipErrorInvalidValue;
    constexpr size_t lds = (size_t)(2 * 256 * 36 + 2 * 64 * 4) * sizeof(float);
    static wm::DevOnce done;
    if (int rc = wm::lds_opt_in(reinterpret_cast<const void*>(lstm_bwd_ws_kernel), lds, done)) return rc;
    hipLaunchKernelGGL(lstm_bwd_ws_kernel, dim3(B), dim3(512), lds, stream, gates, cst, dh_out, w_hh, x, h, partial, T);
    WM_CHECK_LAUNCH();
    hipLaunchKernelGGL(lstm_wgrad_reduce_kernel, dim3(kWgradSlab / 64), dim3(512), 0, stream, (const float*)partial, B,
                       dw_ih, dw_hh, db_ih, db_hh, accumulate);
    WM_CHECK_LAUNCH();
    return 0;
}

static int g_lstm_dx_bf = 1;
int wm_set_lstm_dx_bf16x6(int on, hipStream_t) { g_lstm_dx_bf = on ? 1 : 0; return 0; }

int wm_lstm_dx(const float* da, const float* w_ih, float* dx, int B, int T, hipStream_t stream) {
    const int ntiles = B * ((T + 63) / 64);
    if (g_lstm_dx_bf) {
        constexpr size_t ldsb = (size_t)3 * 64 * 264 * 2;
        static wm::DevOnce doneb;
        if (int rc = wm::lds_opt_in(reinterpret_cast<const void*>(lstm_dx_bf_kernel), ldsb, doneb)) return rc;
        hipLaunchKernelGGL(lstm_dx_bf_kernel, dim3(ntiles < kNumCU ? ntiles : kNumCU), dim3(256), ldsb, stream, da, w_ih, dx, B, T);
        WM_CHECK_LAUNCH();
        return 0;
    }
    constexpr size_t lds = (size_t)(256 * 64 + 64 * 257) * sizeof(float);
    static wm::DevOnce done;
    if (int rc = wm::lds_opt_in(reinterpret_cast<const void*>(lstm_dx_kernel), lds, done)) return rc;
    hipLaunchKernelGGL(lstm_dx_kernel, dim3(ntiles < kNumCU ? ntiles : kNumCU), dim3(256), lds, stream, da, w_ih, dx, B, T);
    WM_CHECK_LAUNCH();
    return 0;
}

int wm_lstm_wgrad(const float* da, const float* x, const float* h, float* partial, float* dw_ih, float* dw_hh,
                  float* db_ih, float* db_hh, int B, int T, int accumulate, hipStream_t stream) {
    int grid;
    if (g_lstm_dx_bf) {
        constexpr size_t ldsb = (size_t)(3 * 32 * 264 + 3 * 128 * 40) * 2;
        static wm::DevOnce doneb;
        if (int rc = wm::lds_opt_in(reinterpret_cast<const void*>(lstm_wgrad_bf_kernel), ldsb, doneb)) return rc;
        const int ntiles = B * ((T + 31) / 32);
        grid = ntiles < kNumCU ? ntiles : kNumCU;
        hipLaunchKernelGGL(lstm_wgrad_bf_kernel, dim3(grid), dim3(256), ldsb, stream, da, x, h, partial, B, T);
    } else {
        constexpr size_t lds = (size_t)(64 * 256 + 128 * 67) * sizeof(float);
        static wm::DevOnce done;
        if (int rc = wm::lds_opt_in(reinterpret_cast<const void*>(lstm_wgrad_kernel), lds, done)) return rc;
        const int ntiles = B * ((T + 63) / 64);
        grid = ntiles < kNumCU ? ntiles : kNumCU;
        hipLaunchKernelGGL(lstm_wgrad_kernel, dim3(grid), dim3(256), lds, stream, da, x, h, partial, B, T);
    }
    WM_CHECK_LAUNCH();
    hipLaunchKernelGGL(lstm_wgrad_reduce_kernel, dim3(kWgradSlab / 64), dim3(512), 0, stream, (const float*)partial, grid,
                       dw_ih, dw_hh, db_ih, db_hh, accumulate);
    WM_CHECK_LAUNCH();
    return 0;
}

}
```

### audio-watermarking-deep-learning-watermarks-for-authenticating-speech_amd/csrc/wm_common.hpp

```cpp
#pragma once
#include <hip/hip_runtime.h>
#include <stdint.h>
#include <atomic>

#define WM_CHECK_LAUNCH() do { hipError_t e_ = hipGetLastError(); if (e_ != hipSuccess) return (int)e_; } while (0)
#define WM_TRY(expr) do { hipError_t e_ = (expr); if (e_ != hipSuccess) return (int)e_; } while (0)

namespace wm {

struct DevOnce {
    std::atomic<unsigned long long> mask{0};
};
inline bool dev_done(const DevOnce& d) {
    int dev = 0;
    if (hipGetDevice(&dev) != hipSuccess) return false;
    return (d.mask.load(std::memory_order_acquire) >> (dev & 63)) & 1ull;
}
inline void dev_mark(DevOnce& d) {
    int dev = 0;
    if (hipGetDevice(&dev) != hipSuccess) return;
    d.mask.fetch_or(1ull << (dev & 63), std::memory_order_release);
}
inline int lds_opt_in(const void* kern, size_t lds, DevOnce& once) {
    if (dev_done(once)) return 0;
// ... 68 lines not shown
template <int NW>
__device__ __forceinline__ float block_sum(float v, float* scratch) {
    v = wave_sum(v);
    const int lane = threadIdx.x & 63, w = threadIdx.x >> 6;
    __syncthreads();
    if (lane == 0) scratch[w] = v;
    __syncthreads();
    float r = 0.f;
#pragma unroll
    for (int i = 0; i < NW; ++i) r += scratch[i];
    return r;
}
template <int NW>
__device__ __forceinline__ double block_sum_d(double v, double* scratch) {
    v = wave_sum_d(v);
    const int lane = threadIdx.x & 63, w = threadIdx.x >> 6;
    __syncthreads();
    if (lane == 0) scratch[w] = v;
    __syncthreads();
    double r = 0.0;
#pragma unroll
    for (int i = 0; i < NW; ++i) r += scratch[i];
    return r;
}

template <int NG>
__device__ __forceinline__ double column_sum_d(const float* __restrict__ partial, int nparts, size_t stride, int i, bool valid,
                                               double (&sq)[NG][64]) {
    const int il = threadIdx.x & 63, grp = threadIdx.x >> 6;
    const int per = (nparts + NG - 1) / NG, p0 = grp * per, p1 = min(p0 + per, nparts);
    double s0 = 0.0, s1 = 0.0, s2 = 0.0, s3 = 0.0;
    if (valid) {
        const float* col = partial + i;
        int p = p0;
        for (; p + 3 < p1; p += 4) {
            const float v0 = col[(size_t)p * stride], v1 = col[(size_t)(p + 1) * stride];
            const float v2 = col[(size_t)(p + 2) * stride], v3 = col[(size_t)(p + 3) * stride];
            s0 += (double)v0; s1 += (double)v1; s2 += (double)v2; s3 += (double)v3;
        }
        if (p < p1) s0 += (double)col[(size_t)p * stride];
        if (p + 1 < p1) s1 += (double)col[(size_t)(p + 1) * stride];
        if (p + 2 < p1) s2 += (double)col[(size_t)(p + 2) * stride];
    }
    sq[grp][il] = (s0 + s1) + (s2 + s3);
    __syncthreads();
    double s = 0.0;
    if (grp == 0) {
#pragma unroll
        for (int g = 0; g < NG; ++g) s += sq[g][il];
    }
    return s;
}

__device__ __forceinline__ float sigmoidf_acc(float x) { return 1.0f / (1.0f + expf(-x)); }

__device__ __forceinline__ float softplus_neg_abs(float x) {
    const float u = __expf(-fabsf(x));
    return (u < 0.01f) ? u * fmaf(u, fmaf(u, 0.33333334f, -0.5f), 1.0f) : __logf(1.0f + u);
}
__device__ __forceinline__ float bce_logits(float x, float y) { return fmaxf(x, 0.f) - x * y + softplus_neg_abs(x); }
__device__ __forceinline__ float bce_logits_grad(float x, float y, float k) {
    const float sg = __builtin_amdgcn_rcpf(1.0f + __expf(-x));
    return k * (sg - y);
}

int launch_sum_scale2(const float* partial, int n, double scale, float* out, hipStream_t stream);

#ifndef WM_STREAM_NT
#define WM_STREAM_NT 1
#endif
__device__ __forceinline__ float4 stream_load(const float4* p) {
#if WM_STREAM_NT
    const f32x4 v = __builtin_nontemporal_load(reinterpret_cast<const f32x4*>(p));
    return make_float4(v.x, v.y, v.z, v.w);
#else
    return *p;
#endif
}
__device__ __forceinline__ void stream_store(float4* p, const float4& v) {
#if WM_STREAM_NT
    __builtin_nontemporal_store(f32x4{v.x, v.y, v.z, v.w}, reinterpret_cast<f32x4*>(p));
#else
    *p = v;
#endif
}
__device__ __forceinline__ float stream_load(const float* p) {
#if WM_STREAM_NT
    return __builtin_nontemporal_load(p);
#else
    return *p;
#endif
}
__device__ __forceinline__ void stream_store(float* p, float v) {
#if WM_STREAM_NT
    __builtin_nontemporal_store(v, p);
#else
    *p = v;
#endif
}

__device__ __forceinline__ float elu1(float v) {
    const float p = v * (1.f + v * (0.5f + v * (0.16666667f + v * (0.041666668f + v * (0.0083333338f + v * 0.0013888889f)))));
    const float e = __expf(v) - 1.f;
    const float n = v > -0.35f ? p : e;
    return v > 0.f ? v : n;
}



typedef __bf16 bf16x8 __attribute__((ext_vector_type(8)));
typedef __bf16 bf16x2 __attribute__((ext_vector_type(2)));

__device__ __forceinline__ void split3_pair(float a, float b, unsigned& p0, unsigned& p1, unsigned& p2) {
    bf16x2 h = {(__bf16)a, (__bf16)b};
    p0 = __builtin_bit_cast(unsigned, h);
    a -= __uint_as_float(p0 << 16); b -= __uint_as_float(p0 & 0xffff0000u);
    bf16x2 m = {(__bf16)a, (__bf16)b};
    p1 = __builtin_bit_cast(unsigned, m);
    a -= __uint_as_float(p1 << 16); b -= __uint_as_float(p1 & 0xffff0000u);
    bf16x2 l = {(__bf16)a, (__bf16)b};
    p2 = __builtin_bit_cast(unsigned, l);
}

__device__ __forceinline__ f32x16 mfma_bf16x6(const bf16x8 (&A)[3], const bf16x8 (&B)[3], f32x16 acc) {
    acc = __builtin_amdgcn_mfma_f32_32x32x16_bf16(A[1], B[1], acc, 0, 0, 0);
    acc = __builtin_amdgcn_mfma_f32_32x32x16_bf16(A[0], B[2], acc, 0, 0, 0);
    acc = __builtin_amdgcn_mfma_f32_32x32x16_bf16(A[2], B[0], acc, 0, 0, 0);
    acc = __builtin_amdgcn_mfma_f32_32x32x16_bf16(A[0], B[1], acc, 0, 0, 0);
    acc = __builtin_amdgcn_mfma_f32_32x32x16_bf16(A[1], B[0], acc, 0, 0, 0);
    acc = __builtin_amdgcn_mfma_f32_32x32x16_bf16(A[0], B[0], acc, 0, 0, 0);
    return acc;
}

typedef __amdgpu_buffer_rsrc_t wm_srd_t;

__device__ __forceinline__ wm_srd_t make_srd(const float* p, size_t bytes) {
    return __builtin_amdgcn_make_buffer_rsrc(const_cast<float*>(p), (short)0, (int)(bytes > 0xfffff000ull ? 0xfffff000ull : bytes),
                                             0x00020000);
}
__device__ __forceinline__ float buf_load(wm_srd_t srd, unsigned voff_bytes, unsigned soff_bytes) {
    return __builtin_bit_cast(float, __builtin_amdgcn_raw_buffer_load_b32(srd, (int)voff_bytes, (int)soff_bytes, 0));
}
typedef unsigned u32x4 __attribute__((ext_vector_type(4)));
__device__ __forceinline__ f32x4 buf_load4(wm_srd_t srd, unsigned voff_bytes, unsigned soff_bytes) {
    return __builtin_bit_cast(f32x4, __builtin_amdgcn_raw_buffer_load_b128(srd, (int)voff_bytes, (int)soff_bytes, 0));
}
__device__ __forceinline__ void buf_store4(wm_srd_t srd, f32x4 v, unsigned voff_bytes, unsigned soff_bytes) {
    __builtin_amdgcn_raw_buffer_store_b128(__builtin_bit_cast(u32x4, v), srd, (int)voff_bytes, (int)soff_bytes, 0);
}
__device__ __forceinline__ void buf_store(wm_srd_t srd, float v, unsigned voff_bytes, unsigned soff_bytes) {
    __builtin_amdgcn_raw_buffer_store_b32(__builtin_bit_cast(unsigned, v), srd, (int)voff_bytes, (int)soff_bytes, 0);
}

}
```

### audio-watermarking-deep-learning-watermarks-for-authenticating-speech_amd/modules.py

```python
from __future__ import annotations

import torch
import torch.nn as nn

from . import ops


class ResBlock(nn.Module):

    def __init__(self, ch):
        super().__init__()
        if ch != 64:
            raise ValueError("the MI355X hot path is built for the reference's 64-channel ResBlock")
        self.block = nn.Sequential(
            nn.Conv1d(ch, ch, 3, padding=1),
            nn.BatchNorm1d(ch),
            nn.ReLU(),
            nn.Conv1d(ch, ch, 3, padding=1),
            nn.BatchNorm1d(ch),
        )
        self.relu = nn.ReLU()

    def forward(self, x):
        return ops.ResBlockFn.apply(x, *_rb_args(self), self.training)


def _rb_args(m):
    c1, n1, _, c2, n2 = m.block
    return (c1.weight, c1.bias, n1.weight, n1.bias, c2.weight, c2.bias, n2.weight, n2.bias,
            n1.running_mean, n1.running_var, n1.num_batches_tracked, n2.running_mean, n2.running_var, n2.num_batches_tracked)


def _hooked(*modules):
    return any(m._forward_hooks or m._forward_pre_hooks for m in modules)


def resblock_pair(m1, m2, x):
    if m1.training and m2.training and not _hooked(m1, m2) and ops.pair_node_applies(x):
        return ops.ResBlockPairFn.apply(x, *_rb_args(m1), *_rb_args(m2), True)
    return m2(m1(x))


class _Stem(nn.Conv1d):
    def forward(self, x, grad_rows=None):
        return ops.StemFn.apply(x, self.weight, self.bias, grad_rows)


class _Head1(nn.Conv1d):
    def forward(self, x):
        return ops.Head1Fn.apply(x, self.weight, self.bias)


class Generator(nn.Module):

    def __init__(self, message_bits=0):
        super().__init__()
        self.message_bits = message_bits
        self.encoder = nn.Sequential(_Stem(1, 64, 7, padding=3), ResBlock(64), ResBlock(64))
        self.lstm = nn.LSTM(64, 64, batch_first=True)
        if message_bits > 0:
            self.embedding = nn.Embedding(2 ** message_bits, 64)
        self.decoder = nn.Sequential(nn.ConvTranspose1d(64, 64, 7, padding=3), ResBlock(64), _Head1(64, 1, 1))

    def forward(self, s, message=None):
        x = resblock_pair(self.encoder[1], self.encoder[2], self.encoder[0](s))
        x = ops.LSTMFn.apply(x, self.lstm.weight_ih_l0, self.lstm.weight_hh_l0, self.lstm.bias_ih_l0, self.lstm.bias_hh_l0)
        vec = None
        if self.message_bits > 0 and message is not None:
            if message.dim() != 1 or message.shape[0] != s.shape[0]:
                raise ValueError(f"message must have shape ({s.shape[0]},), got {tuple(message.shape)}")
            vec = ops.EmbedFn.apply(self.embedding.weight, message.to(torch.int64))
        ct = self.decoder[0]
        x = ops.ConvT7Fn.apply(x, vec, ct.weight, ct.bias)
        rb, head = self.decoder[1], self.decoder[2]
        if rb.training and not _hooked(rb, head) and ops.tail_in_head_applies(x):
            return ops.ResBlockHead1Fn.apply(x, *_rb_args(rb), head.weight, head.bias)
        return head(rb(x))


class _HeadN(nn.Conv1d):
    def forward(self, x):
        return ops.HeadNFn.apply(x, self.weight, self.bias)


class Detector(nn.Module):

    def __init__(self, message_bits=0):
        super().__init__()
        self.message_bits = message_bits
        output_dim = 1 + message_bits
        self.model = nn.Sequential(_Stem(1, 64, kernel_size=7, padding=3), ResBlock(64), ResBlock(64),
                                   _HeadN(64, output_dim, kernel_size=1))

    def forward(self, x, input_grad_rows=None):
        x = self.model[0](x) if input_grad_rows is None else self.model[0](x, input_grad_rows)
        return self.model[3](resblock_pair(self.model[1], self.model[2], x))

    def forward_with_losses(self, x, message, input_grad_rows=None):
        m1, m2, head = self.model[1], self.model[2], self.model[3]
        ok = (m1.training and m2.training and not _hooked(self, self.model, m1, m2, head) and ops.tail_in_head_applies(x)
              and ops.pair_node_applies(x) and 1 <= head.weight.shape[0] <= 64 and isinstance(message, torch.Tensor) and message.is_cuda
              and message.dtype == torch.int64 and message.dim() == 1 and x.shape[0] == 2 * message.shape[0])
        if not ok:
            return None
        x = self.model[0](x) if input_grad_rows is None else self.model[0](x, input_grad_rows)
        return ops.DetectorTailFn.apply(x, message.contiguous(), *_rb_args(m1), *_rb_args(m2), head.weight, head.bias)


def load_state_dict_strip_prefix(model, state_dict, prefix="_orig_mod."):
    cleaned = {(k[len(prefix):] if k.startswith(prefix) else k): v for k, v in state_dict.items()}
    return model.load_state_dict(cleaned, strict=False)
```

### audio-watermarking-deep-learning-watermarks-for-authenticating-speech_amd/ops.py

```python
from __future__ import annotations

import contextlib
import math
import os

import torch

from ._lib import lib

NCU = 256
BN_EPS = 1e-5
BN_MOMENTUM = 0.1


def _stream():
    return torch.cuda.current_stream().cuda_stream


def _p(t):
    return None if t is None else t.data_ptr()


def _chk(t: torch.Tensor, name: str, ndim: int | None = None, dtype=torch.float32) -> torch.Tensor:
    if not isinstance(t, torch.Tensor):
# ... 101 lines not shown

def _on_side(inputs, fn, defer=True):
    _ASYNC["deferred"].append((inputs, fn))
    if not defer:
        release_deferred_wgrads()


def _wgrad_dst(gdst, device, *shapes):
    if all(g is not None for g in gdst):
        return gdst, True, _on_side
    return tuple(_f32(*shape, device=device) for shape in shapes), False, lambda inputs, fn: fn()


SWITCHES = {
    "bf16x6": ("conv", "bf16x6", "WM_CONV_BF16X6", True, None, "64->64 convolutions on the bf16x6 / f16 split builds | native fp32 MFMA"),
    "schedule": ("conv", "schedule", "WM_CONV_BF_SCHEDULE", 2, "wm_set_conv_bf_schedule", "an integer: 2 register-resident weights + interleaved split | 0 phase-serial"),
    "one_launch_eval": ("conv", "one_launch_eval", "WM_RESBLOCK_ONE_LAUNCH", True, None, "inference ResBlock as one launch | two"),
    "fused_bwd": ("conv", "fused_bwd", "WM_FUSED_BWD", True, None, "ResBlock backward: data + weight gradient of a convolution in one launch | two"),
    "mask_on_load": ("conv", "mask_on_load", "WM_MASK_ON_LOAD", True, None, "fused ResBlock backward masks g on load | writes the masked gradient first"),
    "pair_fold": ("conv", "pair_fold", "WM_PAIR_FOLD", True, None, "two ResBlocks in a row as one tape node | two nodes"),
    "bwd_f16x3": ("conv", "bwd_f16x3", "WM_BWD_F16X3", True, None, "fused ResBlock backward on the f16 two-piece split | bf16x6"),
    "fwd_f16x3": ("conv", "fwd_f16x3", "WM_FWD_F16X3", True, None, "ResBlock forward convolutions on the f16 two-piece split | bf16x6"),
    "conv7_f16x3": ("conv", "conv7_f16x3", "WM_CONV7_F16X3", True, None, "ConvTranspose1d(64,64,7) on the f16 two-piece split | bf16x6"),
    "eval_f16x3": ("conv", "eval_f16x3", "WM_EVAL_F16X3", True, None, "one-launch inference ResBlock on the f16 two-piece split | bf16x6"),
    "lstm_fused": ("lstm", "fused", "WM_LSTM_FUSED", True, None, "LSTM input projection inside the recurrence kernel | wm_lstm_xproj + wm_lstm_fwd"),
    "lstm_bwd_fused": ("lstm", "bwd_fused", "WM_LSTM_BWD_FUSED", False, None, "wm_lstm_bwd + wm_lstm_dx as one launch | two (the default)"),
    "lstm_bwd_ws": ("lstm", "bwd_ws", "WM_LSTM_BWD_WS", True, None, "LSTM weight gradients on helper waves beside the BPTT | wm_lstm_bwd + wm_lstm_wgrad"),
    "lstm_fwd_ws": ("lstm", "fwd_ws", "WM_LSTM_FWD_WS", True, "wm_set_lstm_fwd_wave_specialised", "LSTM forward input projection on helper waves | in the recurrence's own waves"),
    "gconv_f16x3": ("gconv", "f16x3", "WM_GCONV_F16X3", True, None, "main14b_2 generic convolutions on the f16 two-piece split | native fp32 MFMA"),
    "fused_strided_dgrad": ("main14b_2", "_FUSED_STRIDED_DGRAD", "WM_FUSED_STRIDED_DGRAD", True, None, "main14b_2 down-sampling block: both data gradients into x in one launch | two"),
}


def read_switches(environ) -> dict:
    out = {"conv": {}, "lstm": {}, "gconv": {}, "main14b_2": {}, "library": []}
    for name, (store, key, env, default, libfn, _) in SWITCHES.items():
        raw = environ.get(env)
        out[store][key] = default if raw is None else int(raw) if type(default) is int else raw == "1"
        if libfn and raw is not None:
            out["library"].append(name)
    return out


_LIVE = read_switches(os.environ)
_CONV, _LSTM, _GCONV = _LIVE["conv"], _LIVE["lstm"], _LIVE["gconv"]


def bind_store(store, namespace):
    namespace.update(_LIVE[store])
    _LIVE[store] = namespace


def set_switch(name, value):
    store, key, _, default, libfn, _ = SWITCHES[name]
    value = type(default)(value)
    if libfn:
        getattr(lib, libfn)(int(value), None)
    _LIVE[store][key] = value


for _name in _LIVE["library"]:
    set_switch(_name, _LIVE[SWITCHES[_name][0]][SWITCHES[_name][1]])


@contextlib.contextmanager
def switches(**values):
    prev = {name: _LIVE[SWITCHES[name][0]][SWITCHES[name][1]] for name in values}
    try:
        for name, value in values.items():
            set_switch(name, value)
        yield
    finally:
        for name, value in prev.items():
            set_switch(name, value)


def set_conv_bf_schedule(schedule: int):
    set_switch("schedule", schedule)


def set_conv_bf16x6(on: bool):
    set_switch("bf16x6", on)


def set_fused_backward(on: bool):
    set_switch("fused_bwd", on)


def set_mask_on_load(on: bool):
    set_switch("mask_on_load", on)


def set_bwd_f16x3(on: bool):
    set_switch("bwd_f16x3", on)


def set_fwd_f16x3(on: bool):
    set_switch("fwd_f16x3", on)


def set_eval_f16x3(on: bool):
    set_switch("eval_f16x3", on)


def pack_w64_h(w: torch.Tensor, mode: int) -> torch.Tensor:
    wph = torch.empty(2 * 3 * 4096 + 4, dtype=torch.int16, device=w.device)
    lib.wm_pack_w64_h(_p(w), _p(wph), mode, _stream())
    return wph


def set_pair_fold(on: bool):
    set_switch("pair_fold", on)


def set_resblock_one_launch(on: bool):
    set_switch("one_launch_eval", on)


def conv_bf16x6() -> bool:
    return _CONV["bf16x6"]


def pack_w64_bf(w: torch.Tensor, mode: int) -> torch.Tensor:
    wpb = torch.empty(3 * 3 * 4096, dtype=torch.int16, device=w.device)
    lib.wm_pack_w64_bf(_p(w), _p(wpb), mode, _stream())
    return wpb


def set_conv7_f16x3(on: bool):
    set_switch("conv7_f16x3", on)


def pack_w64_h7(w: torch.Tensor, mode: int) -> torch.Tensor:
    wph = torch.empty(2 * 7 * 4096 + 4, dtype=torch.int16, device=w.device)
    lib.wm_pack_w64_h7(_p(w), _p(wph), mode, _stream())
    return wph


def set_lstm_fwd_wave_specialised(on: bool):
    set_switch("lstm_fwd_ws", on)


def set_lstm_bwd_wave_specialised(on: bool):
    set_switch("lstm_bwd_ws", on)


_HEADS = {"tail_in_head": os.environ.get("WM_TAIL_IN_HEAD", "1") == "1"}


def set_tail_in_head(on: bool):
    _HEADS["tail_in_head"] = bool(on)


def set_gconv_f16x3(on: bool):
    set_switch("gconv_f16x3", on)


_GMAX = {}


def _note_gmax(t: torch.Tensor, maxes: torch.Tensor, per_clip: bool = False):
    import weakref
    if len(_GMAX) > 256:
        _GMAX.clear()
    _GMAX[id(t)] = (weakref.ref(t), t._version, maxes, per_clip)


def _noted(t: torch.Tensor, pop: bool):
    e = _GMAX.pop(id(t), None) if pop else _GMAX.get(id(t))
    return e if e is not None and e[0]() is t and e[1] == t._version else None


def gscale_of(g: torch.Tensor, log2_target: float = 12.0) -> torch.Tensor:
    e = _noted(g, pop=True)
    if e is not None:
        gsc = _f32(2, device=g.device)
        lib.wm_gscale_from_max(_p(e[2]), e[2].numel(), float(log2_target), _p(gsc), _stream())
        return gsc
    return gscale_absmax(g, log2_target)


_ZPOOL = {"buf": None, "used": 0}


def zeroed_slots(n: int, device) -> torch.Tensor:
    p = _ZPOOL
    if p["buf"] is None or p["buf"].device != torch.device(device) or p["used"] + n > p["buf"].numel():
        p["buf"], p["used"] = torch.zeros(max(1 << 16, n), dtype=torch.float32, device=device), 0
    s = p["buf"][p["used"]:p["used"] + n]
    p["used"] += n
    return s


def amax_per_clip(x: torch.Tensor) -> torch.Tensor:
    e = _noted(x, pop=False)
    if e is not None and e[3]:
        return e[2]
    NB = x.shape[0]
    m = zeroed_slots(NB, x.device)
    lib.wm_absmax_rows(_p(x), NB, x.numel() // NB, _p(m), _stream())
    _note_gmax(x, m, per_clip=True)
    return m


def gscale_absmax(g: torch.Tensor, log2_target: float = 12.0) -> torch.Tensor:
    gsc, scratch = _f32(2, device=g.device), _f32(1024, device=g.device)
    lib.wm_gscale_absmax(_p(g), g.numel(), _p(scratch), float(log2_target), _p(gsc), _stream())
    return gsc


def pack_w64_bf7(w: torch.Tensor, mode: int) -> torch.Tensor:
    wpb = torch.empty(3 * 7 * 4096, dtype=torch.int16, device=w.device)
    lib.wm_pack_w64_bf7(_p(w), _p(wpb), mode, _stream())
    return wpb


def _conv3(x, x2, w, mode, pa, pb, pc, bias, e1, ea, eb, y, stats, B, T, pro, epi):
    if _CONV["bf16x6"]:
        h = (_CONV["fwd_f16x3"] and mode == 0 and (pro, epi) in ((0, 0), (1, 0), (1, 4)) and _CONV["schedule"] == 2 and T % 128 == 0)
        lib.wm_conv64_bf(_p(x), _p(x2), _p(pack_w64_h(w, 0) if h else pack_w64_bf(w, mode)), _p(pa), _p(pb), _p(pc), _p(bias), _p(e1),
                         _p(ea), _p(eb), _p(y), _p(stats), B, T, pro, epi, 1 if h else 0, _stream())
    else:
        lib.wm_conv64(_p(x), _p(x2), _p(pack_w64(w, 3, mode)), _p(pa), _p(pb), _p(pc), _p(bias), _p(e1), _p(ea), _p(eb), _p(y),
                      _p(stats), B, T, 3, pro, epi, _stream())


def pack_w64(w: torch.Tensor, kw: int, mode: int) -> torch.Tensor:
    wp = _f32(kw * 4096, device=w.device)
    lib.wm_pack_w64(_p(w), _p(wp), kw, mode, _stream())
    return wp


def _resblock_fwd(x, params, training, want_grad, tail=True):
    w1, b1, g1, be1, w2, b2, g2, be2, rm1, rv1, nbt1, rm2, rv2, nbt2 = params
    x = _frames(x, "ResBlock input", 64)
    B, _, T = x.shape
    dev, st = x.device, _stream()
    out = torch.empty_like(x) if tail else None
    cst = _f32(8, 64, device=dev)
    sc1, sh1, mu1, is1, sc2, sh2, mu2, is2 = cst.unbind(0)
    if training:
        y1, y2 = torch.empty_like(x), torch.empty_like(x)
        stats = _f32(NCU * 128, device=dev)
        _conv3(x, None, w1, 0, None, None, None, b1, None, None, None, y1, stats, B, T, 0, 0)
        lib.wm_bn_finalize(_p(stats), NCU, float(B * T), _p(g1), _p(be1), _p(rm1), _p(rv1), _p(nbt1), BN_MOMENTUM, BN_EPS,
                           _p(sc1), _p(sh1), _p(mu1), _p(is1), st)
        _conv3(y1, None, w2, 0, sc1, sh1, None, b2, None, None, None, y2, stats, B, T, 1, 0)
        lib.wm_bn_finalize(_p(stats), NCU, float(B * T), _p(g2), _p(be2), _p(rm2), _p(rv2), _p(nbt2), BN_MOMENTUM, BN_EPS,
                           _p(sc2), _p(sh2), _p(mu2), _p(is2), st)
    else:
        lib.wm_bn_eval_scale_shift(_p(g1), _p(be1), _p(rm1), _p(rv1), BN_EPS, _p(sc1), _p(sh1), st)
        lib.wm_bn_eval_scale_shift(_p(g2), _p(be2), _p(rm2), _p(rv2), BN_EPS, _p(sc2), _p(sh2), st)
        if not want_grad and _CONV["bf16x6"] and _CONV["one_launch_eval"]:
            h = _CONV["eval_f16x3"]
            wp1 = torch.empty((2 * 3 * 4096 + 4) if h else 3 * 3 * 4096, dtype=torch.int16, device=dev)
            wp2 = torch.empty_like(wp1)
            pack = lib.wm_pack_w64_h_scaled if h else lib.wm_pack_w64_bf_scaled
            pack(_p(w1), _p(sc1), _p(wp1), st)
            pack(_p(w2), _p(sc2), _p(wp2), st)
            lib.wm_resblock_eval_bf(_p(x), _p(wp1), _p(wp2), _p(b1), _p(sc1), _p(sh1), _p(b2), _p(sc2), _p(sh2), _p(out), B, T,
                                    1 if h else 0, st)
            return out, None
        y1 = torch.empty_like(x)
        _conv3(x, None, w1, 0, None, None, None, b1, None, None, None, y1, None, B, T, 0, 0)
        if not want_grad and _CONV["bf16x6"] and _CONV["schedule"] == 2 and T % 128 == 0:
            _conv3(y1, None, w2, 0, sc1, sh1, None, b2, x, sc2, sh2, out, None, B, T, 1, 4)
            return out, None
        y2 = torch.empty_like(x)
        _conv3(y1, None, w2, 0, sc1, sh1, None, b2, None, None, None, y2, None, B, T, 1, 0)
        mu1.copy_(rm1); is1.copy_(torch.rsqrt(rv1 + BN_EPS)); mu2.copy_(rm2); is2.copy_(torch.rsqrt(rv2 + BN_EPS))
    if not tail:
        return None, (x, y1, y2, None, cst, w1, w2, g1, g2)
    if want_grad:
        mask = torch.empty(B * 64 * ((T + 31) // 32), dtype=torch.int32, device=dev)
        lib.wm_bn_add_relu_mask(_p(x), _p(y2), _p(sc2), _p(sh2), _p(out), _p(mask), B, T, st)
    else:
        mask = None
        lib.wm_bn_add_relu(_p(x), _p(y2), _p(sc2), _p(sh2), _p(out), B, T, st)
    return out, (x, y1, y2, mask, cst, w1, w2, g1, g2)


class ResBlockFn(GradAwareFunction):

    @staticmethod
    def forward(ctx, x, *args):
        params, training = args[:14], args[14]
        out, saved = _resblock_fwd(x, params, training, wants_grad(ctx))
        if saved is not None:
            ctx.training = bool(training)
            ctx.gdst = _gdst(params[0], params[1], params[4], params[5])
            ctx.save_for_backward(*saved)
        return out

    @staticmethod
    def backward(ctx, g_out):
        return _resblock_bwd(ctx.saved_tensors, ctx.training, ctx.gdst, g_out) + (None,) * 7


def _resblock_bwd(saved, training, gdst, g_out):
    x, y1, y2, mask, cst, w1, w2, g1, g2 = saved
    sc1, sh1, mu1, is1, sc2, sh2, mu2, is2 = cst.unbind(0)
    g_out = g_out.contiguous()
    B, _, T = x.shape
    dev, st = x.device, _stream()
    ev = 0 if training else 1
    n = float(B * T)
    if _CONV["bf16x6"] and _CONV["fused_bwd"] and T % 64 == 0 and not all(g is not None for g in gdst):
        dx, grads, _ = _resblock_bwd_fused(saved, training, g_out)
        return (dx,) + grads
    (dw1, db1, dw2, db2), acc, launch = _wgrad_dst(gdst, dev, w1.shape, (64,), w2.shape, (64,))
    part = _f32(max(B, 1) * 128, device=dev)
    dz2 = torch.empty_like(x)
    lib.wm_relu_bwd_reduce_mask(_p(g_out), _p(mask), _p(y2), _p(dz2), _p(part), None, B, T, st)
    k2 = _f32(4, 64, device=dev)
    dg2, dbe2 = _f32(64, device=dev), _f32(64, device=dev)
    lib.wm_bn_bwd_finalize(_p(part), B, n, _p(g2), _p(mu2), _p(is2), _p(k2[0]), _p(k2[1]), _p(k2[3]), _p(dg2), _p(dbe2), 0, ev, None, 0, None, st)
    dz1 = torch.empty_like(x)
    stats = _f32(NCU * 128, device=dev)
    _conv3(dz2, y2, w2, 1, k2[0], k2[1], k2[3], None, y1, sc1, sh1, dz1, stats, B, T, 3, 1)

    def wgrad(dz, y, k, xin, sc, sh, xpro, dw, db):
        wpart = _f32(2 * NCU * (3 * 4096 + 64), device=dev)
        if _CONV["bf16x6"]:
            lib.wm_wgrad64_bf(_p(dz), _p(y), _p(k[0]), _p(k[1]), _p(k[3]), _p(xin), _p(sc), _p(sh), _p(wpart), _p(dw), _p(db),
                              B, T, 3, xpro, 3 if acc else 0, _stream())
        else:
            lib.wm_wgrad64(_p(dz), _p(y), _p(k[0]), _p(k[1]), _p(k[3]), _p(xin), _p(sc), _p(sh), _p(wpart), _p(dw), _p(db),
                           B, T, 3, 3, xpro, 0, 1 if acc else 0, _stream())
    launch((dz2, y2, k2, y1, cst), lambda: wgrad(dz2, y2, k2, y1, sc1, sh1, 1, dw2, db2))
    k1 = _f32(4, 64, device=dev)
    dg1, dbe1 = _f32(64, device=dev), _f32(64, device=dev)
    lib.wm_bn_bwd_finalize(_p(stats), NCU, n, _p(g1), _p(mu1), _p(is1), _p(k1[0]), _p(k1[1]), _p(k1[3]), _p(dg1), _p(dbe1), 0, ev, None, 0, None, st)
    dx = torch.empty_like(x)
    _conv3(dz1, y1, w1, 1, k1[0], k1[1], k1[3], None, dz2, None, None, dx, None, B, T, 3, 2)
    launch((dz1, y1, k1, x), lambda: wgrad(dz1, y1, k1, x, None, None, 0, dw1, db1))
    g1_, g2_ = ((None, None),) * 2 if acc else ((dw1, db1), (dw2, db2))
    return (dx,) + g1_ + (dg1, dbe1) + g2_ + (dg2, dbe2)


def _resblock_bwd_fused(saved, training, g_out, pre=None, fold=None):
    x, y1, y2, mask, cst, w1, w2, g1, g2 = saved
    sc1, sh1, mu1, is1, sc2, sh2, mu2, is2 = cst.unbind(0)
    B, _, T = x.shape
    dev, st = x.device, _stream()
    ev = 0 if training else 1
    n = float(B * T)
    h = 1 if _CONV["bwd_f16x3"] else 0
    pack = pack_w64_h if h else pack_w64_bf
    k2 = _f32(4, 64, device=dev)
    dg2, dbe2 = _f32(64, device=dev), _f32(64, device=dev)
    gs2 = _f32(2, device=dev) if h else None
    if pre is not None:
        ppart, pmax = pre
        gsrc, gm = g_out, None
        lib.wm_bn_bwd_finalize(_p(ppart), NCU, n, _p(g2), _p(mu2), _p(is2), _p(k2[0]), _p(k2[1]), _p(k2[3]), _p(dg2), _p(dbe2), 0, ev,
                               _p(pmax) if h else None, NCU, _p(gs2), st)
    else:
        part = _f32(max(B, 1) * 128, device=dev)
        dzm = _f32(B * 64, device=dev) if h else None
        dz2 = None if _CONV["mask_on_load"] else torch.empty_like(x)
        lib.wm_relu_bwd_reduce_mask(_p(g_out), _p(mask), _p(y2), _p(dz2), _p(part), _p(dzm), B, T, st)
        lib.wm_bn_bwd_finalize(_p(part), B, n, _p(g2), _p(mu2), _p(is2), _p(k2[0]), _p(k2[1]), _p(k2[3]), _p(dg2), _p(dbe2), 0, ev,
                               _p(dzm), B * 64, _p(gs2), st)
        gsrc, gm = (g_out, mask) if dz2 is None else (dz2, None)
    dz1 = torch.empty_like(x)
    stats = _f32(NCU * 128, device=dev)
    dzm1 = _f32(NCU, device=dev) if h else None
    dw2, db2, dw1, db1 = torch.empty_like(w2), _f32(64, device=dev), torch.empty_like(w1), _f32(64, device=dev)
    wpart = _f32(NCU * (3 * 4096 + 64), device=dev)
    lib.wm_dwgrad64_bf(_p(gsrc), _p(y2), _p(k2[0]), _p(k2[1]), _p(k2[3]), _p(pack(w2, 1)), _p(y1), _p(sc1), _p(sh1),
                       _p(y1), _p(sc1), _p(sh1), _p(dz1), _p(stats), _p(wpart), _p(dw2), _p(db2), B, T, 1, 1, 0, _p(gm), h, _p(gs2), _p(dzm1), st)
    k1 = _f32(4, 64, device=dev)
    dg1, dbe1 = _f32(64, device=dev), _f32(64, device=dev)
    gs1 = _f32(2, device=dev) if h else None
    lib.wm_bn_bwd_finalize(_p(stats), NCU, n, _p(g1), _p(mu1), _p(is1), _p(k1[0]), _p(k1[1]), _p(k1[3]), _p(dg1), _p(dbe1), 0, ev,
                           _p(dzm1), NCU, _p(gs1), st)
    dx = torch.empty_like(x)
    fout = None
    if fold is not None and gm is not None:
        pmask, py2 = fold
        fpart = _f32(NCU * 128, device=dev)
        fmax = _f32(NCU, device=dev) if h else None
        lib.wm_dwgrad64_bf(_p(dz1), _p(y1), _p(k1[0]), _p(k1[1]), _p(k1[3]), _p(pack(w1, 1)), _p(x), None, None,
                           _p(gsrc), _p(py2), _p(pmask), _p(dx), _p(fpart), _p(wpart), _p(dw1), _p(db1), B, T, 0, 8, 0, _p(gm), h, _p(gs1), _p(fmax), st)
        fout = (fpart, fmax)
    else:
        xmax = _f32(NCU, device=dev) if h else None
        lib.wm_dwgrad64_bf(_p(dz1), _p(y1), _p(k1[0]), _p(k1[1]), _p(k1[3]), _p(pack(w1, 1)), _p(x), None, None,
                           _p(gsrc), None, None, _p(dx), None, _p(wpart), _p(dw1), _p(db1), B, T, 0, 2, 0, _p(gm), h, _p(gs1), _p(xmax), st)
        if h:
            _note_gmax(dx, xmax)
    return dx, (dw1, db1, dg1, dbe1, dw2, db2, dg2, dbe2), fout


def pair_node_applies(x) -> bool:
    return (torch.is_grad_enabled() and x.is_cuda and x.dim() == 3 and x.shape[-1] % 64 == 0 and _CONV["bf16x6"]
            and _CONV["fused_bwd"] and _CONV["mask_on_load"] and _CONV["pair_fold"] and not _ASYNC["on"])


class ResBlockPairFn(GradAwareFunction):

    @staticmethod
    def forward(ctx, x, *args):
        p1, p2, training = args[:14], args[14:28], args[28]
        mid, first = _resblock_fwd(x, p1, training, wants_grad(ctx))
        out, second = _resblock_fwd(mid, p2, training, wants_grad(ctx))
        ctx.save_for_backward(*(first + second))
        ctx.training = bool(training)
        return out

    @staticmethod
    def backward(ctx, g_out):
        sv = ctx.saved_tensors
        s1_, s2_ = sv[:9], sv[9:]
        g_out = g_out.contiguous()
        dmid, grads2, fout = _resblock_bwd_fused(s2_, ctx.training, g_out, fold=(s1_[3], s1_[2]))
        dx, grads1, _ = _resblock_bwd_fused(s1_, ctx.training, dmid, pre=fout)
        return (dx,) + grads1 + (None,) * 6 + grads2 + (None,) * 6 + (None,)


class StemFn(torch.autograd.Function):

    @staticmethod
    def forward(ctx, s, w, b, grad_rows=None):
        s = _frames(s, "clip batch", 1)
        B, _, T = s.shape
        y = _f32(B, 64, T, device=s.device)
        lib.wm_stem_fwd(_p(s), _p(w), _p(b), _p(y), B, T, _stream())
        ctx.save_for_backward(s, w)
        ctx.grad_rows = B if grad_rows is None else max(0, min(int(grad_rows), B))
        return y

    @staticmethod
    def backward(ctx, g):
        s, w = ctx.saved_tensors
        g = g.contiguous()
        B, _, T = s.shape
        ds = None
        if ctx.needs_input_grad[0]:
            ds = torch.empty_like(s) if ctx.grad_rows == B else torch.zeros_like(s)
        part = _f32(2 * NCU * 512, device=s.device)
        dw, db = torch.empty_like(w), _f32(64, device=s.device)
        lib.wm_stem_bwd(_p(g), _p(s), _p(w), _p(ds), _p(part), _p(dw), _p(db), B, T, ctx.grad_rows, 0, _stream())
        return ds, dw, db, None


class Head1Fn(torch.autograd.Function):

    @staticmethod
    def forward(ctx, x, w, b):
        x = _frames(x, "head input", 64)
        B, _, T = x.shape
        y = _f32(B, 1, T, device=x.device)
        lib.wm_head1_fwd(_p(x), _p(w), _p(b), _p(y), B, T, _stream())
        ctx.save_for_backward(x, w)
        return y

    @staticmethod
    def backward(ctx, g):
        x, w = ctx.saved_tensors
        g = g.contiguous()
        B, _, T = x.shape
        dx = torch.empty_like(x)
        part = _f32(1024 * 65, device=x.device)
        dw, db = torch.empty_like(w), _f32(1, device=x.device)
        lib.wm_head1_bwd(_p(g), _p(x), _p(w), _p(dx), _p(part), _p(dw), _p(db), B, T, 0, _stream())
        return dx, dw, db


class HeadNFn(torch.autograd.Function):

    @staticmethod
    def forward(ctx, x, w, b):
        x = _frames(x, "head input", 64)
        B, _, T = x.shape
        NO = w.shape[0]
        if not 1 <= NO <= 64:
            raise ValueError(f"Detector head: 1+message_bits must be in 1..64 (message ids are int64, so a message "
                             f"carries at most 63 bits), got {NO}")
        y = _f32(B, T, NO, device=x.device)
        lib.wm_headN_fwd(_p(x), _p(w), _p(b), _p(y), B, T, NO, _stream())
        ctx.save_for_backward(x, w)
        return y

    @staticmethod
    def backward(ctx, g):
        x, w = ctx.saved_tensors
        g = g.contiguous()
        B, _, T = x.shape
        NO = w.shape[0]
        dx = torch.empty_like(x)
        part = _f32(NCU * (NO * 64 + NO), device=x.device)
        dw, db = torch.empty_like(w), _f32(NO, device=x.device)
        lib.wm_headN_bwd(_p(g), _p(x), _p(w), _p(dx), _p(part), _p(dw), _p(db), B, T, NO, 0, _stream())
        return dx, dw, db


def tail_in_head_applies(x) -> bool:
    return _HEADS["tail_in_head"] and x.is_cuda and x.dim() == 3 and not _ASYNC["on"]


def _tail_mask(x, want_grad):
    B, _, T = x.shape
    return torch.empty(B * 64 * ((T + 31) // 32), dtype=torch.int32, device=x.device) if want_grad else None


class ResBlockHead1Fn(GradAwareFunction):

    @staticmethod
    def forward(ctx, x, *args):
        params, hw, hb = args[:14], args[14], args[15]
        want = wants_grad(ctx)
        _, saved = _resblock_fwd(x, params, True, want, tail=False)
        x, _, y2, _, cst = saved[:5]
        B, _, T = x.shape
        out, mask = torch.empty_like(x), _tail_mask(x, want)
        y = _f32(B, 1, T, device=x.device)
        lib.wm_head1_tail_fwd(_p(x), _p(y2), _p(cst[4]), _p(cst[5]), _p(hw), _p(hb), _p(out), _p(mask), _p(y), B, T, _stream())
        if want:
            ctx.save_for_backward(*(saved[:3] + (mask,) + saved[4:] + (out, hw)))
        return y

    @staticmethod
    def backward(ctx, g):
        sv = ctx.saved_tensors
        out, hw = sv[9], sv[10]
        B, _, T = out.shape
        dout = torch.empty_like(out)
        part = _f32(1024 * 65, device=out.device)
        dhw, dhb = torch.empty_like(hw), _f32(1, device=out.device)
        lib.wm_head1_bwd(_p(g.contiguous()), _p(out), _p(hw), _p(dout), _p(part), _p(dhw), _p(dhb), B, T, 0, _stream())
        return _resblock_bwd(sv[:9], True, (None,) * 4, dout) + (None,) * 6 + (dhw, dhb)


class DetectorTailFn(GradAwareFunction):

    @staticmethod
    def forward(ctx, x, message, *args):
        p1, p2, hw, hb = args[:14], args[14:28], args[28], args[29]
        want = wants_grad(ctx)
        mid, first = _resblock_fwd(x, p1, True, want)
        _, second = _resblock_fwd(mid, p2, True, want, tail=False)
        y2, cst = second[2], second[4]
        R, _, T = mid.shape
        NO, B, dev = hw.shape[0], message.shape[0], mid.device
        out, mask = torch.empty_like(mid), _tail_mask(mid, want)
        logits = _f32(R, T, NO, device=dev)
        part = _f32(2 * R * ((T + 255) // 256), device=dev)
        losses = torch.zeros(2, dtype=torch.float32, device=dev)
        lib.wm_headN_tail_fwd(_p(mid), _p(y2), _p(cst[4]), _p(cst[5]), _p(hw), _p(hb), _p(message), B, _p(part), _p(losses[0]), _p(losses[1]),
                              _p(out), _p(mask), _p(logits), R, T, NO, _stream())
        ctx.set_materialize_grads(False)
        if want:
            ctx.save_for_backward(*(first + second[:3] + (mask,) + second[4:] + (out, hw, logits, message)))
        return logits, losses[0], losses[1]

    @staticmethod
    def backward(ctx, g_logits, g_loc, g_bce):
        sv = ctx.saved_tensors
        s1_, s2_, (out, hw, logits, message) = sv[:9], sv[9:18], sv[18:]
        R, T, NO = logits.shape
        dev, st = logits.device, _stream()
        gl = g_loc.contiguous().float().reshape(1) if g_loc is not None else torch.zeros(1, device=dev)
        gb = g_bce.contiguous().float().reshape(1) if g_bce is not None else torch.zeros(1, device=dev)
        dout = torch.empty_like(out)
        part = _f32(NCU * (NO * 64 + NO), device=dev)
        dhw, dhb = torch.empty_like(hw), _f32(NO, device=dev)
        if g_logits is None:
            lib.wm_headN_bwd_bce(_p(logits), _p(message), _p(gl), _p(gb), _p(out), _p(hw), _p(dout), _p(part), _p(dhw), _p(dhb),
                                 message.shape[0], R, T, NO, 0, st)
        else:
            d = torch.empty_like(logits)
            lib.wm_bce_bwd(_p(logits), _p(message), _p(gl), _p(gb), _p(d), message.shape[0], R, T, NO, st)
            d += g_logits
            lib.wm_headN_bwd(_p(d), _p(out), _p(hw), _p(dout), _p(part), _p(dhw), _p(dhb), R, T, NO, 0, st)
        dmid, grads2, fout = _resblock_bwd_fused(s2_, True, dout, fold=(s1_[3], s1_[2]))
        dx, grads1, _ = _resblock_bwd_fused(s1_, True, dmid, pre=fout)
        return (dx, None) + grads1 + (None,) * 6 + grads2 + (None,) * 6 + (dhw, dhb)


class LSTMFn(GradAwareFunction):

    @staticmethod
    def forward(ctx, x, w_ih, w_hh, b_ih, b_hh):
        x = _frames(x, "LSTM input", 64)
        B, _, T = x.shape
        dev, st = x.device, _stream()
        need_grad = wants_grad(ctx)
        h = torch.empty_like(x)
        release_deferred_wgrads()
        cst = _f32(B, T, 64, device=dev) if need_grad else None
        if _LSTM["fused"] and T >= 8:
            gates = _f32(B, T, 256, device=dev) if need_grad else None
            lib.wm_lstm_fwd_fused(_p(x), _p(w_ih), _p(b_ih), _p(b_hh), _p(w_hh), _p(h), _p(gates), _p(cst), B, T, st)
        else:
            xp = _f32(B, T, 256, device=dev)
            lib.wm_lstm_xproj(_p(x), _p(w_ih), _p(b_ih), _p(b_hh), _p(xp), B, T, st)
            gates = xp if need_grad else None
            lib.wm_lstm_fwd(_p(xp), _p(w_hh), _p(h), _p(gates), _p(cst), B, T, st)
        if need_grad:
            ctx.gdst = _gdst(w_ih, w_hh, b_ih, b_hh)
            ctx.save_for_backward(x, h, gates, cst, w_ih, w_hh)
        return h

    @staticmethod
    def backward(ctx, dh):
        x, h, gates, cst, w_ih, w_hh = ctx.saved_tensors
        _single_backward(ctx, "LSTMFn")
        dh = dh.contiguous()
        B, _, T = x.shape
        dev, st = x.device, _stream()
        dx = torch.empty_like(x)
        release_deferred_wgrads()
        dst, acc, launch = _wgrad_dst(ctx.gdst, dev, w_ih.shape, w_hh.shape, (256,), (256,))
        if _LSTM["bwd_ws"] and not _LSTM["bwd_fused"] and T % 32 == 0 and T >= 64:
            part = _f32(B * (256 * 128 + 256), device=dev)
            lib.wm_lstm_bwd_wgrad(_p(gates), _p(cst), _p(dh), _p(w_hh), _p(x), _p(h), _p(part), *map(_p, dst), B, T, int(acc), st)
            lib.wm_lstm_dx(_p(gates), _p(w_ih), _p(dx), B, T, st)
            return (dx,) + ((None,) * 4 if acc else dst)
        if _LSTM["bwd_fused"]:
            lib.wm_lstm_bwd_fused(_p(gates), _p(cst), _p(dh), _p(w_hh), _p(w_ih), _p(dx), B, T, st)
        else:
            lib.wm_lstm_bwd(_p(gates), _p(cst), _p(dh), _p(w_hh), B, T, st)
            lib.wm_lstm_dx(_p(gates), _p(w_ih), _p(dx), B, T, st)

        def wg():
            part = _f32(NCU * (256 * 128 + 256), device=dev)
            lib.wm_lstm_wgrad(_p(gates), _p(x), _p(h), _p(part), *map(_p, dst), B, T, int(acc), _stream())
        launch((gates, x, h), wg)
        return (dx,) + ((None,) * 4 if acc else dst)


_CHECK_INDEX = {"mode": {"1": "sync", "0": "off"}.get(os.environ.get("WM_CHECK_INDEX", "1"), os.environ.get("WM_CHECK_INDEX", "sync")),
                "pending": []}


def set_index_check(mode):
    _CHECK_INDEX["mode"] = {True: "sync", False: "off"}.get(mode, mode)
    if _CHECK_INDEX["mode"] not in ("sync", "deferred", "off"):
        raise ValueError("index check mode must be 'sync', 'deferred' or 'off'")


@contextlib.contextmanager
def index_check_mode(mode=None):
    prev = _CHECK_INDEX["mode"]
    set_index_check(("deferred" if prev == "sync" else prev) if mode is None else mode)
    try:
        yield
    finally:
        _CHECK_INDEX["mode"] = prev


def index_check() -> str:
    return _CHECK_INDEX["mode"]


def check_message_ids(wait=True, what="an earlier Generator call"):
    keep = []
    for ev, host, nrows in _CHECK_INDEX["pending"]:
        if not wait and not ev.query():
            keep.append((ev, host, nrows))
            continue
        ev.synchronize()
        if int(host[0]) != 0:
            _CHECK_INDEX["pending"] = []
            raise IndexError(f"message id out of range for an embedding table of {nrows} rows (deferred check of {what})")
    _CHECK_INDEX["pending"] = keep


def drop_pending_message_checks():
    _CHECK_INDEX["pending"] = []


def _note_index_error(err, nrows):
    mode = _CHECK_INDEX["mode"]
    if mode == "off":
        return
    if mode == "sync":
        if int(err.item()) != 0:
            raise IndexError(f"message id out of range for an embedding table of {nrows} rows")
        return
    check_message_ids(wait=False)
    host = torch.empty(1, dtype=torch.int32, pin_memory=True)
    host.copy_(err, non_blocking=True)
    ev = torch.cuda.Event()
    ev.record()
    _CHECK_INDEX["pending"].append((ev, host, nrows))


class EmbedFn(torch.autograd.Function):

    @staticmethod
    def forward(ctx, table, message):
        table = _chk(table, "embedding.weight", 2)
        message = _chk(message, "message", 1, torch.int64)
        B = message.shape[0]
        vec = _f32(B, 64, device=table.device)
        err = torch.zeros(1, dtype=torch.int32, device=table.device)
        lib.wm_embed_gather(_p(table), _p(message), _p(vec), B, table.shape[0], _p(err), _stream())
        _note_index_error(err, table.shape[0])
        ctx.save_for_backward(message)
        ctx.nrows = table.shape[0]
        return vec

    @staticmethod
    def backward(ctx, dvec):
        (message,) = ctx.saved_tensors
        dtable = torch.zeros(ctx.nrows, 64, dtype=torch.float32, device=dvec.device)
        lib.wm_embed_scatter_add(_p(dtable), _p(message), _p(dvec.contiguous()), message.shape[0], ctx.nrows, _stream())
        return dtable, None


def _conv7_arith(T) -> str:
    return "fp32" if not _CONV["bf16x6"] else "f16x3" if _CONV["conv7_f16x3"] and T % 128 == 0 else "bf16x6"


def _conv7(arith, x, w, wmode, vec, b, y, B, T, pro, epi, gsc, st):
    if arith == "fp32":
        lib.wm_conv64(_p(x), None, _p(pack_w64(w, 7, wmode)), _p(vec), None, None, _p(b), None, None, None, _p(y), None, B, T, 7, pro, epi, st)
    else:
        h = arith == "f16x3"
        lib.wm_conv64_bf7(_p(x), _p((pack_w64_h7 if h else pack_w64_bf7)(w, wmode)), _p(vec), _p(b), _p(y), B, T, pro, epi, int(h), _p(gsc), st)


class ConvT7Fn(torch.autograd.Function):

    @staticmethod
    def forward(ctx, x, vec, w, b):
        x = _frames(x, "decoder input", 64)
        B, _, T = x.shape
        y = torch.empty_like(x)
        _conv7(_conv7_arith(T), x, w, 2, vec, b, y, B, T, 2 if vec is not None else 0, 0, None, _stream())
        ctx.has_vec = vec is not None
        ctx.gdst = _gdst(w, b)
        ctx.save_for_backward(x, w, vec if vec is not None else x.new_empty(0))
        return y

    @staticmethod
    def backward(ctx, g):
        x, w, vec = ctx.saved_tensors
        vec = vec if ctx.has_vec else None
        g = g.contiguous()
        B, _, T = x.shape
        dev, st = x.device, _stream()
        dx = torch.empty_like(x)
        arith = _conv7_arith(T)
        h = arith == "f16x3"
        gsc = gscale_of(g) if h else None
        _conv7(arith, g, w, 3, None, None, dx, B, T, 0, 3, gsc, st)
        (dw, db), acc, launch = _wgrad_dst(ctx.gdst, dev, w.shape, (64,))
        pro = 2 if vec is not None else 0

        def wg():
            part = _f32(2 * NCU * (7 * 4096 + 64), device=dev)
            if arith == "fp32":
                lib.wm_wgrad64(_p(g), None, None, None, None, _p(x), _p(vec), None, _p(part), _p(dw), _p(db), B, T, 7, 0, pro, 1, int(acc),
                               _stream())
            else:
                lib.wm_wgrad64_bf7(_p(g), _p(x), _p(vec), _p(part), _p(dw), _p(db), B, T, pro, int(acc), int(h), _p(gsc), _stream())
        launch((g, x, vec, gsc), wg)
        dvec = None
        if vec is not None and ctx.needs_input_grad[1]:
            dvec = _f32(B, 64, device=dev)
            lib.wm_rowsum(_p(dx), _p(dvec), B * 64, T, st)
        return (dx, dvec) + ((None, None) if acc else (dw, db))


class PostprocFn(torch.autograd.Function):

    @staticmethod
    def forward(ctx, delta, taps, thr, max_rms, eps, stages):
        delta = _frames(delta, "delta", 1)
        B, _, T = delta.shape
        dev = delta.device
        out = torch.empty_like(delta)
        need = ctx.needs_input_grad[0]
        f = torch.empty_like(delta) if need else None
        stats = _f32(B, 2, device=dev)
        lib.wm_postproc_fwd(_p(delta), _p(taps), taps.numel(), thr, max_rms, eps, stages, _p(f), _p(out), _p(stats), B, T, _stream())
        if need:
            ctx.save_for_backward(f, stats, taps)
        ctx.cfg = (thr, max_rms, stages)
        return out
# ... 851 lines not shown
```

### include/wm_hip.h

```cpp
#ifndef WM_HIP_H
#define WM_HIP_H

#ifdef __cplusplus
extern "C" {
#endif

typedef struct ihipStream_t* wm_stream_t;


int wm_pack_w64(const float* w, float* wp, int KW, int mode, wm_stream_t stream);

int wm_conv64(const float* x, const float* x2, const float* wp, const float* pa, const float* pb, const float* pc,
              const float* bias, const float* e1, const float* ea, const float* eb, float* y, float* stats,
              int B, int T, int KW, int pro, int epi, wm_stream_t stream);

int wm_pack_w64_bf(const float* w, void* wpb, int mode, wm_stream_t stream);
int wm_set_conv_bf_schedule(int schedule, wm_stream_t stream);
int wm_conv64_bf(const float* x, const float* x2, const void* wpb, const float* pa, const float* pb, const float* pc,
                 const float* bias, const float* e1, const float* ea, const float* eb, float* y, float* stats,
                 int B, int T, int pro, int epi, int arith, wm_stream_t stream);

int wm_pack_w64_bf_scaled(const float* w, const float* row_scale, void* wpb, wm_stream_t stream);
int wm_resblock_eval_bf(const float* x, const void* w1pb, const void* w2pb, const float* b1, const float* sc1, const float* sh1,
                        const float* b2, const float* sc2, const float* sh2, float* y, int B, int T, int arith, wm_stream_t stream);
int wm_pack_w64_h_scaled(const float* w, const float* row_scale, void* wph, wm_stream_t stream);

int wm_dwgrad64_bf(const float* g, const float* g2, const float* ga, const float* gb, const float* gc, const void* wpb,
                   const float* x, const float* xa, const float* xb, const float* e1, const float* ea, const float* eb,
                   float* y, float* stats, float* partial, float* dw, float* dbias, int B, int T, int xpro, int epi, int accumulate,
                   const void* gmask, int arith, const float* gscale, float* dzmax, wm_stream_t stream);
int wm_pack_w64_h(const float* w, void* wph, int mode, wm_stream_t stream);

int wm_pack_w64_bf7(const float* w, void* wpb, int mode, wm_stream_t stream);
int wm_conv64_bf7(const float* x, const void* wpb, const float* vec, const float* bias, float* y, int B, int T, int pro, int epi,
                  int arith, const float* gscale, wm_stream_t stream);
int wm_pack_w64_h7(const float* w, void* wph, int mode, wm_stream_t stream);
int wm_gscale_absmax(const float* x, long long n, float* scratch, float log2_target, float* gscale, wm_stream_t stream);
int wm_gscale_from_max(const float* maxes, int n, float log2_target, float* gscale, wm_stream_t stream);
int wm_absmax_rows(const float* x, int rows, long long row_len, float* out, wm_stream_t stream);

int wm_wgrad64_bf7(const float* g, const float* x, const float* vec, float* partial, float* dw, float* dbias, int B, int T,
                   int xpro, int accumulate, int arith, const float* gscale, wm_stream_t stream);

int wm_wgrad64_bf(const float* g, const float* g2, const float* ga, const float* gb, const float* gc,
                  const float* x, const float* xa, const float* xb, float* partial, float* dw, float* dbias,
                  int B, int T, int gpro, int xpro, int accumulate, wm_stream_t stream);

int wm_wgrad64(const float* g, const float* g2, const float* ga, const float* gb, const float* gc,
               const float* x, const float* xa, const float* xb, float* partial, float* dw, float* dbias,
               int B, int T, int KW, int gpro, int xpro, int layout, int accumulate, wm_stream_t stream);

int wm_bn_finalize(const float* partials, int nparts, double count, const float* gamma, const float* beta,
                   float* running_mean, float* running_var, long long* num_batches_tracked, float momentum, float eps,
                   float* scale, float* shift, float* save_mean, float* save_invstd, wm_stream_t stream);
int wm_bn_eval_scale_shift(const float* gamma, const float* beta, const float* running_mean, const float* running_var,
                           float eps, float* scale, float* shift, wm_stream_t stream);
int wm_bn_add_relu(const float* x, const float* y2, const float* scale, const float* shift, float* out, int B, int T,
                   wm_stream_t stream);
int wm_relu_bwd_reduce(const float* g, const float* out, const float* y2, float* dz, float* partial, int B, int T,
                       wm_stream_t stream);
int wm_bn_add_relu_mask(const float* x, const float* y2, const float* scale, const float* shift, float* out, void* mask, int B, int T,
                        wm_stream_t stream);
int wm_relu_bwd_reduce_mask(const float* g, const void* mask, const float* y2, float* dz, float* partial, float* dzmax, int B, int T,
                            wm_stream_t stream);
int wm_bn_bwd_finalize(const float* partials, int nparts, double count, const float* gamma, const float* save_mean,
                       const float* save_invstd, float* A, float* Bc, float* Cc, float* dgamma, float* dbeta,
                       int accumulate, int eval_mode, const float* dzmax, int nmax, float* gscale, wm_stream_t stream);

int wm_stem_fwd(const float* s, const float* w, const float* bias, float* y, int B, int T, wm_stream_t stream);
int wm_stem_bwd(const float* g, const float* s, const float* w, float* ds, float* partial, float* dw, float* db, int B,
                int T, int nds, int accumulate, wm_stream_t stream);
int wm_head1_fwd(const float* x, const float* w, const float* bias, float* y, int B, int T, wm_stream_t stream);
int wm_head1_bwd(const float* g, const float* x, const float* w, float* dx, float* partial, float* dw, float* db, int B,
                 int T, int accumulate, wm_stream_t stream);
int wm_headN_fwd(const float* x, const float* w, const float* bias, float* y, int B, int T, int NO, wm_stream_t stream);
int wm_headN_bwd(const float* g, const float* x, const float* w, float* dx, float* partial, float* dw, float* db, int B,
                 int T, int NO, int accumulate, wm_stream_t stream);
int wm_head1_tail_fwd(const float* x, const float* y2, const float* scale, const float* shift, const float* w, const float* bias,
                      float* out, void* mask, float* y, int B, int T, wm_stream_t stream);
int wm_headN_tail_fwd(const float* x, const float* y2, const float* scale, const float* shift, const float* w, const float* bias,
                      const long long* message, int B, float* partial, float* loc_out, float* bce_out, float* out, void* mask,
                      float* logits, int R, int T, int NO, wm_stream_t stream);
int wm_headN_bwd_bce(const float* logits, const long long* message, const float* g_loc, const float* g_bce, const float* x,
                     const float* w, float* dx, float* partial, float* dw, float* db, int B, int R, int T, int NO, int accumulate,
                     wm_stream_t stream);

int wm_lstm_xproj(const float* x, const float* w_ih, const float* b_ih, const float* b_hh, float* xp, int B, int T,
                  wm_stream_t stream);
int wm_lstm_fwd(const float* xp, const float* w_hh, float* hout, float* gates, float* cst, int B, int T, wm_stream_t stream);
int wm_lstm_fwd_fused(const float* x, const float* w_ih, const float* b_ih, const float* b_hh, const float* w_hh,
                      float* hout, float* gates, float* cst, int B, int T, wm_stream_t stream);
int wm_set_lstm_fwd_wave_specialised(int on, wm_stream_t stream);
int wm_lstm_bwd(float* gates, const float* cst, const float* dh_out, const float* w_hh, int B, int T, wm_stream_t stream);
int wm_lstm_dx(const float* da, const float* w_ih, float* dx, int B, int T, wm_stream_t stream);
int wm_set_lstm_dx_bf16x6(int on, wm_stream_t stream);
int wm_lstm_bwd_fused(float* gates, const float* cst, const float* dh_out, const float* w_hh, const float* w_ih, float* dx,
                      int B, int T, wm_stream_t stream);
int wm_lstm_wgrad(const float* da, const float* x, const float* h, float* partial, float* dw_ih, float* dw_hh,
                  float* db_ih, float* db_hh, int B, int T, int accumulate, wm_stream_t stream);
int wm_lstm_bwd_wgrad(float* gates, const float* cst, const float* dh_out, const float* w_hh, const float* x, const float* h,
                      float* partial, float* dw_ih, float* dw_hh, float* db_ih, float* db_hh, int B, int T, int accumulate,
                      wm_stream_t stream);

int wm_embed_gather(const float* table, const long long* message, float* vec, int B, int nrows, int* err, wm_stream_t stream);
int wm_embed_scatter_add(float* dtable, const long long* message, const float* dvec, int B, int nrows, wm_stream_t stream);
int wm_rowsum(const float* x, float* out, int rows, int T, wm_stream_t stream);

int wm_postproc_fwd(const float* d_in, const float* taps, int ntaps, float thr, float max_rms, float eps, int stages,
                    float* f_out, float* d_out, float* stats, int B, int T, wm_stream_t stream);
int wm_postproc_bwd(const float* g, const float* f_in, const float* stats, const float* taps, int ntaps, float thr,
                    float max_rms, int stages, float* d_raw, int B, int T, wm_stream_t stream);

int wm_mel_loss(const float* clean, const float* wm, const float* fb, const int* klo, const int* khi, const int* mlo,
                float* gframes, float* partial, float* loss_out, float* dsig, int B, int T, wm_stream_t stream);
int wm_loud_loss(const float* clean, const float* wm, float thresh, float* gframes, float* partial, float* loss_out,
                 float* dsig, int B, int T, wm_stream_t stream);
int wm_hf_penalty(const float* delta, int kcut, float* gframes, float* partial, float* loss_out, float* dsig, int B, int T,
                  wm_stream_t stream);

int wm_bce_fwd(const float* logits, const long long* message, float* partial, float* loc_out, float* bce_out, int B, int R,
               int T, int NO, wm_stream_t stream);
int wm_bce_bwd(const float* logits, const long long* message, const float* g_loc, const float* g_bce, float* dlogits, int B,
               int R, int T, int NO, wm_stream_t stream);
int wm_l1_fwd(const float* x, float* partial, float* out, long long n, wm_stream_t stream);
int wm_l1_bwd(const float* x, const float* g, float* dx, long long n, wm_stream_t stream);
int wm_adam_step(float* p, const float* g, float* m, float* v, long long n, double lr, double beta1, double beta2, double eps,
                 int step, wm_stream_t stream);

int wm_gconv(const float* x, const float* wp, const float* bias, const float* vec, const float* res, float* y, int NB,
             int Cin, int Lin, int K, int S, int P, int Mtot, int Nout, int st, int shp, int Cout, int Lout, int act,
             const float* x2, int Cin1, int nph, wm_stream_t stream);
int wm_gconv_h(const float* x, const void* wph, const float* bias, const float* vec, const float* res, float* y, int NB,
               int Cin, int Lin, int K, int S, int P, int Mtot, int Nout, int st, int shp, int Cout, int Lout, int act,
               const float* x2, int Cin1, int nph, const float* gscale, float* ymax, int per_clip, wm_stream_t stream);
int wm_gconv_pack_h(const float* wp, void* wph, float* scratch, int Cin, int K, int Mtot, wm_stream_t stream);
int wm_gconv_pack_h_conv(const float* w, void* wph, int Cout, int Cin, int K, int mode, wm_stream_t stream);
int wm_gwgrad_plan(int NB, int Ca, int Cb, int La, int K, long long* slab_floats, wm_stream_t stream);
int wm_gwgrad(const float* A, const float* Bx, float* G, float* dbias, float* slab, int NB, int Ca, int Cb, int La, int Lb,
              int K, int P, long long b_clip_stride, int remap, int r1, int r2, int accumulate, wm_stream_t stream);
int wm_gather_taps(const float* x, float* y, int NB, int C, int Lin, int K, int S, int P, int Lout, int order, wm_stream_t stream);
int wm_elu_bwd(const float* g, const float* y, float* dz, long long n, wm_stream_t stream);
int wm_channel_sum(const float* x, float* out, float* partial, int NB, int C, int L, int accumulate, wm_stream_t stream);
int wm_rowsum_any(const float* x, float* out, int rows, int L, wm_stream_t stream);
int wm_rows_scatter_add(float* dtable, const long long* idx, const float* dvec, int Bn, int dim, int nrows, wm_stream_t stream);
int wm_permute_acl(const float* x, float* y, int A, int C, int L, wm_stream_t stream);
int wm_lstm_seq_fwd(float* xp, const float* whh, float* hs, float* cs, int T, int H, int B, int save, wm_stream_t stream);
int wm_lstm_seq_bwd(float* gates, const float* cs, const float* dout, const float* whhT, float* dc, int T, int H, int B,
                    wm_stream_t stream);

int wm_resample_plan(int P, int Q, int width, int W, long long* tile_periods, wm_stream_t stream);
int wm_resample(const float* x, const float* taps, const int* first, float* y, int C, long long N, int P, int Q, int width, int W,
                long long L, long long total, wm_stream_t stream);

int wm_resample_add(const float* d, const float* taps, const int* first, const float* x, float* out, float* up, int C, long long N,
                    long long Nd, int P, int Q, int width, int W, wm_stream_t stream);

int wm_resample_rows(const float* x, const float* taps, const int* first, float* y, long long rows, long long N, long long L, int P, int Q,
                     int width, int W, wm_stream_t stream);

int wm_biquad_plan(int warm, int* chunk_len, wm_stream_t stream);
int wm_biquad(const float* x, void* out, void* mask_out, const void* mask_in, float b0, float b1, float b2, float a1, float a2,
              long long rows, long long n, int warm, int mode, int clamp, int reverse, wm_stream_t stream);

int wm_distort_plan(long long rows, long long n, long long* scratch_floats, wm_stream_t stream);
int wm_distort(const float* x, float* y, float* stat, float* scratch, long long rows, long long n, long long row0, long long seed,
               long long draw, float gain_lo, float gain_hi, float snr_lo, float snr_hi, float p_noise, wm_stream_t stream);
int wm_distort_bwd(const float* dy, const float* x, const float* stat, float* dx, float* scratch, long long rows, long long n,
                   long long row0, long long seed, long long draw, int through, wm_stream_t stream);

int wm_mdct_codec_plan(long long n, int M, int* frames_per_workgroup, long long* workgroups_per_row, wm_stream_t stream);
int wm_mdct_codec(const float* x, float* y, void* codes_out, const void* mask_in, const float* snr_db, long long rows, long long n, int M,
                  int band, int kcut, float floor_step, int quantise, wm_stream_t stream);

int wm_fir_rows(const float* x, const float* h, float* y, long long rows, long long n, int K, long long h_stride, int reverse,
                wm_stream_t stream);

int wm_rir_synth(const float* params, float* h, long long rows, int K, float sample_rate, long long row0, long long seed, long long draw,
                 wm_stream_t stream);

int wm_time_warp(const float* x, const float* params, const float* tab, float* y, long long rows, long long n, int zeros, int res,
                 int adjoint, wm_stream_t stream);

int wm_stoi_plan(long long rows, long long n, long long* scratch_bytes, wm_stream_t stream);
int wm_stoi(const float* x, const float* y, float* d, int* kept, void* scratch, long long rows, long long n, wm_stream_t stream);

int wm_splice(const float* a, const float* b, float* y, int* lab, long long rows, long long n, long long row0, long long seed,
              long long draw, int max_spans, float p_span, long long len_lo, long long len_hi, float p_original, float p_silence,
              wm_stream_t stream);
int wm_splice_bwd(const float* dy, const int* lab, float* da, long long rows, long long n, wm_stream_t stream);
int wm_bce_masked_fwd(const float* logits, const long long* message, const int* lab, float* partial, long long* count_out,
                      float* loc_out, float* bce_out, int B, int R, int T, int NO, wm_stream_t stream);
int wm_bce_masked_bwd(const float* logits, const long long* message, const int* lab, const long long* count, const float* g_loc,
                      const float* g_bce, float* dlogits, int B, int R, int T, int NO, wm_stream_t stream);
int wm_loc_score(const float* logits, const int* lab, float thr_logit, int* counts, int* pred, int R, int T, int NO,
                 int lab_rows, wm_stream_t stream);

#ifdef __cplusplus
}
#endif
#endif
```

Measured before the change: 5447 clips/s.

## Fuse residual-block tail into next conv prologue and LSTM forward input load

```diff
diff --git a/audio-watermarking-deep-learning-watermarks-for-authenticating-speech_amd/csrc/conv64.hpp b/audio-watermarking-deep-learning-watermarks-for-authenticating-speech_amd/csrc/conv64.hpp
--- a/audio-watermarking-deep-learning-watermarks-for-authenticating-speech_amd/csrc/conv64.hpp
+++ b/audio-watermarking-deep-learning-watermarks-for-authenticating-speech_amd/csrc/conv64.hpp
@@ -43,7 +43,8 @@
 #endif
 
 namespace {
-enum { PRO_NONE = 0, PRO_BNRELU = 1, PRO_ADDVEC = 2, PRO_BNBWD = 3 };
+enum { PRO_NONE = 0, PRO_BNRELU = 1, PRO_ADDVEC = 2, PRO_BNBWD = 3,
+       PRO_TAIL = 4 };
 enum { EPI_BIAS = 0, EPI_RELUMASK = 1, EPI_ADD = 2, EPI_NONE = 3, EPI_BNADDRELU = 4,
        EPI_BIASELU = 5, EPI_BIASADDELU = 6, EPI_MULDELU = 7,
        EPI_ADDSTATS = 8 };
@@ -62,6 +63,8 @@
     float* y;
     float* stats;
     int B, T;
+    float* tout = nullptr;
+    unsigned* tmask = nullptr;
 };
 
 template <int PRO>
@@ -69,6 +72,7 @@
     if (PRO == PRO_BNRELU) return fmaxf(fmaf(v, ca, cb), 0.f);
     if (PRO == PRO_ADDVEC) return v + ca;
     if (PRO == PRO_BNBWD) return fmaf(ca, v, fmaf(cc, v2, cb)) + cl;
+    if (PRO == PRO_TAIL) return fmaxf(v + fmaf(v2, ca, cb), 0.f);
     return v;
 }
 
diff --git a/audio-watermarking-deep-learning-watermarks-for-authenticating-speech_amd/csrc/conv64_fwd.hip b/audio-watermarking-deep-learning-watermarks-for-authenticating-speech_amd/csrc/conv64_fwd.hip
--- a/audio-watermarking-deep-learning-watermarks-for-authenticating-speech_amd/csrc/conv64_fwd.hip
+++ b/audio-watermarking-deep-learning-watermarks-for-authenticating-speech_amd/csrc/conv64_fwd.hip
@@ -237,7 +237,9 @@
 __global__ __launch_bounds__(256) void conv64bf3_kernel(Conv64Args a) {
     constexpr int KW = 3, NT = 128, ROWS = NT + 2, PITCH = 72, NP = H ? 2 : 3, NC = 4;
     constexpr int XBUF = NP * ROWS * PITCH;
-    constexpr bool TWO = (PRO == PRO_BNBWD);
+    constexpr bool TAIL = (PRO == PRO_TAIL);
+    constexpr bool TWO = (PRO == PRO_BNBWD || TAIL);
+    static_assert(!TAIL || H, "the tail prologue exists in the f16 build only");
     constexpr bool E1 = (EPI == EPI_RELUMASK || EPI == EPI_ADD || EPI == EPI_BNADDRELU);
     extern __shared__ __align__(16) unsigned char smem_raw[];
     unsigned short* Xb0 = reinterpret_cast<unsigned short*>(smem_raw);
@@ -298,8 +300,8 @@
 #endif
     load_tile(min(tile, ntiles - 1));
     if (tid < 64) {
-        Cs[tid] = (PRO == PRO_BNRELU || PRO == PRO_BNBWD) ? a.pa[tid] : 0.f;
-        Cs[64 + tid] = (PRO == PRO_BNRELU || PRO == PRO_BNBWD) ? a.pb[tid] : 0.f;
+        Cs[tid] = (PRO == PRO_BNRELU || PRO == PRO_BNBWD || TAIL) ? a.pa[tid] : 0.f;
+        Cs[64 + tid] = (PRO == PRO_BNRELU || PRO == PRO_BNBWD || TAIL) ? a.pb[tid] : 0.f;
         Cs[128 + tid] = (PRO == PRO_BNBWD) ? a.pc[tid] : 0.f;
         Cs[192 + tid] = (PRO == PRO_BNBWD) ? a.pb[64 + tid] : (((EPI == EPI_BIAS || EPI == EPI_BNADDRELU) && a.bias) ? a.bias[tid] : 0.f);
         Cs[256 + tid] = (EPI == EPI_RELUMASK || EPI == EPI_BNADDRELU) ? a.ea[tid] : 0.f;
@@ -307,8 +309,23 @@
     }
     __syncthreads();
     const float ka0 = Cs[c0], ka1 = Cs[c0 + 1], kb0 = Cs[64 + c0], kb1 = Cs[64 + c0 + 1];
-    const float kc0 = Cs[128 + c0], kc1 = Cs[128 + c0 + 1], kl0 = TWO ? Cs[192 + c0] : 0.f, kl1 = TWO ? Cs[192 + c0 + 1] : 0.f;
-    const float ha = Cs[hc], hb = Cs[64 + hc], hcc = Cs[128 + hc], hlo = TWO ? Cs[192 + hc] : 0.f;
+    const float kc0 = Cs[128 + c0], kc1 = Cs[128 + c0 + 1];
+    const float kl0 = (PRO == PRO_BNBWD) ? Cs[192 + c0] : 0.f, kl1 = (PRO == PRO_BNBWD) ? Cs[192 + c0 + 1] : 0.f;
+    const float ha = Cs[hc], hb = Cs[64 + hc], hcc = Cs[128 + hc], hlo = (PRO == PRO_BNBWD) ? Cs[192 + hc] : 0.f;
+
+    auto keep_formed = [&](int i, int e, float va, float vb) {
+        if (e == 0) { sa[i].x = va; sb[i].x = vb; } else if (e == 1) { sa[i].y = va; sb[i].y = vb; }
+        else if (e == 2) { sa[i].z = va; sb[i].z = vb; } else { sa[i].w = va; sb[i].w = vb; }
+    };
+    const wm_srd_t smask = make_srd(reinterpret_cast<const float*>(a.tmask), (TAIL && a.tmask) ? (size_t)a.B * 64 * (T >> 5) * 4 : 0);
+    auto tail_store = [&](int tb, int tt0, int i) {
+        const size_t o = ((size_t)tb * 64 + c0) * T + tt0 + 4 * (q0 + 8 * i);
+        *reinterpret_cast<float4*>(a.tout + o) = sa[i];
+        *reinterpret_cast<float4*>(a.tout + o + T) = sb[i];
+        const unsigned ma = mask_merge8(sign_nibble(sa[i]) << (4 * q0)), mb = mask_merge8(sign_nibble(sb[i]) << (4 * q0));
+        const unsigned word = (unsigned)(tb * 64 + c0 + (q0 & 1)) * (unsigned)(T >> 5) + (unsigned)((tt0 >> 5) + i);
+        __builtin_amdgcn_raw_buffer_store_b32((q0 & 1) ? mb : ma, smask, (int)(q0 < 2 ? word * 4u : 0xFFFFFF00u), 0, 0);
+    };
 
     auto split_unit = [&](unsigned* X32, int t0, int i, int e) {
         const float4 fa = sa[i], fb = sb[i];
@@ -323,6 +340,7 @@
             }
             va = pro_apply<PRO>(va, wa, ka0, kb0, kc0, kl0);
             vb = pro_apply<PRO>(vb, wb, ka1, kb1, kc1, kl1);
+            if (TAIL) keep_formed(i, e, va, vb);
         }
         const int o = (1 + 4 * (q0 + 8 * i) + e) * (PITCH / 2) + cp;
         if (H) {
@@ -368,6 +386,7 @@
             }
             va = pro_apply<PRO>(va, wa, ka0, kb0, kc0, kl0);
             vb = pro_apply<PRO>(vb, wb, ka1, kb1, kc1, kl1);
+            if (TAIL) keep_formed(i, e, va, vb);
         }
         sva = va; svb = vb;
         asm volatile("" : "+v"(sva), "+v"(svb));
@@ -419,6 +438,10 @@
 #pragma unroll
         for (int u = 0; u < 16; ++u) split_unit(reinterpret_cast<unsigned*>(Xb0), t0, u >> 2, u & 3);
         split_halo(Xb0, t0);
+        if (TAIL) {
+#pragma unroll
+            for (int i = 0; i < NC; ++i) tail_store(min(tile, ntiles - 1) / tilesPerClip, t0, i);
+        }
     }
     load_tile(min(tile + tstep, ntiles - 1));
     __syncthreads();
@@ -484,7 +507,7 @@
         STAMP(ts0);
         const int next = min(tile + tstep, ntiles - 1), next2 = min(tile + 2 * tstep, ntiles - 1);
         const int b = tile / tilesPerClip, t0 = (tile - b * tilesPerClip) * NT;
-        const int nt0 = (next % tilesPerClip) * NT;
+        const int nb_ = next / tilesPerClip, nt0 = (next - nb_ * tilesPerClip) * NT;
         const wm_srd_t se1c = E1 ? row_srd(a.e1, b) : syp;
         const unsigned vcolc = lcol + (unsigned)(t0 + 64 * nh) * 4u;
         const unsigned short* xcur = Xb0 + buf * XBUF;
@@ -505,7 +528,7 @@
         if (h < 16) {                                                                                                           \
             if ((k) == 0) split_pick(h >> 2, h & 3);                                                                            \
             if ((k) == 1) split_st1();                                                                                          \
-            if ((k) == 2) split_st2();                                                                                          \
+            if ((k) == 2) { split_st2(); if (TAIL && (h & 3) == 3) tail_store(nb_, nt0, h >> 2); }                              \
             if ((k) == 3) { split_out(reinterpret_cast<unsigned*>(xnxt), h >> 2, h & 3); if ((h & 3) == 3) load_combo(next2, h >> 2); } \
         } else if (h == 16) {                                                                                                   \
             if ((k) == 0) halo_pick(nt0);                                                                                       \
@@ -533,8 +556,13 @@
             FENCE;
             if (H) {
                 acc[nt] = mma(Wr[s][1], Bf[0], acc[nt]); FENCE; BF3_SLICE(0) FENCE; BF3_SLICE(1) FENCE;
-                acc[nt] = mma(Wr[s][0], Bf[1], acc[nt]); FENCE; BF3_SLICE(3) FENCE; BF3_SLICE(4) FENCE;
-                acc[nt] = mma(Wr[s][0], Bf[0], acc[nt]); FENCE; BF3_SLICE(5) FENCE;
+                if (TAIL) {
+                    acc[nt] = mma(Wr[s][0], Bf[1], acc[nt]); FENCE; BF3_SLICE(2) FENCE; BF3_SLICE(3) FENCE;
+                    acc[nt] = mma(Wr[s][0], Bf[0], acc[nt]); FENCE; BF3_SLICE(4) FENCE; BF3_SLICE(5) FENCE;
+                } else {
+                    acc[nt] = mma(Wr[s][0], Bf[1], acc[nt]); FENCE; BF3_SLICE(3) FENCE; BF3_SLICE(4) FENCE;
+                    acc[nt] = mma(Wr[s][0], Bf[0], acc[nt]); FENCE; BF3_SLICE(5) FENCE;
+                }
             } else {
                 acc[nt] = mma(Wr[s][1], Bf[1], acc[nt]); FENCE; BF3_SLICE(0) FENCE;
                 acc[nt] = mma(Wr[s][0], Bf[2], acc[nt]); FENCE; BF3_SLICE(1) FENCE;
@@ -775,6 +803,16 @@
     return (int)hipErrorInvalidValue;
 }
 
+int wm_conv64_bf_tail(const float* x, const float* y2, const void* wpb_h, const float* sc2, const float* sh2, const float* bias,
+                      float* out, void* mask, float* y, float* stats, int B, int T, hipStream_t stream) {
+    if (B <= 0 || T <= 0 || (T & 127) || g_bf_schedule != 2) return (int)hipErrorInvalidValue;
+    if (!x || !y2 || !wpb_h || !sc2 || !sh2 || !out || !y || !stats) return (int)hipErrorInvalidValue;
+    if ((unsigned long long)B * 64ull * (unsigned long long)(T >> 5) * 4ull >= 0xfffff000ull) return (int)hipErrorInvalidValue;
+    Conv64Args a{x, y2, reinterpret_cast<const float*>(wpb_h), sc2, sh2, nullptr, bias, nullptr, nullptr, nullptr, y, stats, B, T,
+                 out, reinterpret_cast<unsigned*>(mask)};
+    return launch_conv64bf3<PRO_TAIL, EPI_BIAS, true, true>(a, stream);
+}
+
 int wm_pack_w64_h(const float* w, void* wph, int mode, hipStream_t stream) {
     if (!w || !wph || mode < 0 || mode > 1) return (int)hipErrorInvalidValue;
     hipLaunchKernelGGL(pack_w64_h_kernel, dim3(1), dim3(1024), 0, stream, w, (const float*)nullptr, reinterpret_cast<unsigned short*>(wph), mode);
diff --git a/audio-watermarking-deep-learning-watermarks-for-authenticating-speech_amd/csrc/lstm.hip b/audio-watermarking-deep-learning-watermarks-for-authenticating-speech_amd/csrc/lstm.hip
--- a/audio-watermarking-deep-learning-watermarks-for-authenticating-speech_amd/csrc/lstm.hip
+++ b/audio-watermarking-deep-learning-watermarks-for-authenticating-speech_amd/csrc/lstm.hip
@@ -406,11 +406,19 @@
 #endif
 }
 
-template <bool SAVE>
+template <bool TAIL>
+struct LstmTailArgs {};
+template <>
+struct LstmTailArgs<true> {
+    const float* y2; const float* sc2; const float* sh2;
+    float* out; unsigned* mask;
+};
+template <bool SAVE, bool TAIL = false>
 __global__ __launch_bounds__(512) void lstm_fwd_ws_kernel(const float* __restrict__ x, const float* __restrict__ w_ih,
                                                           const float* __restrict__ b_ih, const float* __restrict__ b_hh,
                                                           const float* __restrict__ w_hh, float* __restrict__ hout,
-                                                          float* __restrict__ gates, float* __restrict__ cst, int T) {
+                                                          float* __restrict__ gates, float* __restrict__ cst, int T,
+                                                          LstmTailArgs<TAIL> tl) {
     constexpr int CH = 32, XPP = 257, PITCH = 72, NP = 3;
     extern __shared__ __align__(16) unsigned char smem_raw[];
     float* xps = reinterpret_cast<float*>(smem_raw);
@@ -500,14 +508,36 @@
     const int cp = hw * 8 + (lane & 7), tq = lane >> 3;
     const float* xc = x + ((size_t)b * 64 + 2 * cp) * T + 4 * tq;
     float4 sa, sb;
+    [[maybe_unused]] float4 sa2, sb2, oa, ob;
+    [[maybe_unused]] const float* yc = nullptr;
+    [[maybe_unused]] float* oc = nullptr;
+    [[maybe_unused]] float tsc0 = 0.f, tsc1 = 0.f, tsh0 = 0.f, tsh1 = 0.f;
+    if constexpr (TAIL) {
+        yc = tl.y2 + ((size_t)b * 64 + 2 * cp) * T + 4 * tq;
+        oc = tl.out + ((size_t)b * 64 + 2 * cp) * T + 4 * tq;
+        tsc0 = tl.sc2[2 * cp]; tsc1 = tl.sc2[2 * cp + 1]; tsh0 = tl.sh2[2 * cp]; tsh1 = tl.sh2[2 * cp + 1];
+    }
     auto load_x = [&](int t0) {
         const int t = min(t0, T - 4 - 4 * tq);
         sa = *reinterpret_cast<const float4*>(xc + max(t, -4 * tq));
         sb = *reinterpret_cast<const float4*>(xc + T + max(t, -4 * tq));
+        if constexpr (TAIL) {
+            sa2 = *reinterpret_cast<const float4*>(yc + max(t, -4 * tq));
+            sb2 = *reinterpret_cast<const float4*>(yc + T + max(t, -4 * tq));
+        }
     };
     auto split_x = [&]() {
         unsigned* X32 = reinterpret_cast<unsigned*>(Xb);
-        const float va[4] = {sa.x, sa.y, sa.z, sa.w}, vb[4] = {sb.x, sb.y, sb.z, sb.w};
+        float va[4] = {sa.x, sa.y, sa.z, sa.w}, vb[4] = {sb.x, sb.y, sb.z, sb.w};
+        if constexpr (TAIL) {
+            const float wa[4] = {sa2.x, sa2.y, sa2.z, sa2.w}, wb[4] = {sb2.x, sb2.y, sb2.z, sb2.w};
+#pragma unroll
+            for (int e = 0; e < 4; ++e) {
+                va[e] = fmaxf(va[e] + fmaf(wa[e], tsc0, tsh0), 0.f);
+                vb[e] = fmaxf(vb[e] + fmaf(wb[e], tsc1, tsh1), 0.f);
+            }
+            oa = make_float4(va[0], va[1], va[2], va[3]); ob = make_float4(vb[0], vb[1], vb[2], vb[3]);
+        }
 #pragma unroll
         for (int e = 0; e < 4; ++e) {
             unsigned p0, p1, p2;
@@ -538,9 +568,21 @@
 #pragma unroll
             for (int r = 0; r < 16; ++r) dst[mt * 32 + (r & 3) + 8 * (r >> 2)] = acc[mt][r];
     };
+    [[maybe_unused]] auto store_tail = [&](int tc) {
+        if constexpr (TAIL) {
+            *reinterpret_cast<float4*>(oc + tc) = oa;
+            *reinterpret_cast<float4*>(oc + T + tc) = ob;
+            const wm_srd_t smask = make_srd(reinterpret_cast<const float*>(tl.mask) + (size_t)b * 64 * (T >> 5),
+                                            tl.mask ? (size_t)64 * (T >> 5) * 4 : 0);
+            const unsigned ma = mask_merge8(sign_nibble(oa) << (4 * tq)), mb = mask_merge8(sign_nibble(ob) << (4 * tq));
+            const unsigned word = (unsigned)(2 * cp + (tq & 1)) * (unsigned)(T >> 5) + (unsigned)(tc >> 5);
+            __builtin_amdgcn_raw_buffer_store_b32((tq & 1) ? mb : ma, smask, (int)(tq < 2 ? word * 4u : 0xFFFFFF00u), 0, 0);
+        }
+    };
     load_x(0);
     __syncthreads();
     split_x();
+    store_tail(0);
     load_x(CH);
     __syncthreads();
 #pragma unroll
@@ -554,6 +596,7 @@
             if (s == 0) { split_x(); load_x(t0 + 2 * CH); }
             if (s >= 1 && s <= 24) { mfma_one(2 * (s - 1)); mfma_one(2 * (s - 1) + 1); }
             if (s == 26) store_xp(cbuf ^ 1);
+            if (TAIL && s == 27 && t0 + CH < T) store_tail(t0 + CH);
             if (t0 + s < T) __syncthreads();
         }
     }
@@ -1397,13 +1440,28 @@
         static wm::DevOnce donew[2];
         if (int rc = wm::lds_opt_in(reinterpret_cast<const void*>(lstm_fwd_ws_kernel<true>), lds, donew[0])) return rc;
         if (int rc = wm::lds_opt_in(reinterpret_cast<const void*>(lstm_fwd_ws_kernel<false>), lds, donew[1])) return rc;
-        if (gates && cst) hipLaunchKernelGGL(lstm_fwd_ws_kernel<true>, dim3(B), dim3(512), lds, stream, x, w_ih, b_ih, b_hh, w_hh, hout, gates, cst, T);
-        else hipLaunchKernelGGL(lstm_fwd_ws_kernel<false>, dim3(B), dim3(512), lds, stream, x, w_ih, b_ih, b_hh, w_hh, hout, gates, cst, T);
+        if (gates && cst) hipLaunchKernelGGL(lstm_fwd_ws_kernel<true>, dim3(B), dim3(512), lds, stream, x, w_ih, b_ih, b_hh, w_hh, hout, gates, cst, T, LstmTailArgs<false>{});
+        else hipLaunchKernelGGL(lstm_fwd_ws_kernel<false>, dim3(B), dim3(512), lds, stream, x, w_ih, b_ih, b_hh, w_hh, hout, gates, cst, T, LstmTailArgs<false>{});
         WM_CHECK_LAUNCH();
         return 0;
     }
     if (gates && cst) hipLaunchKernelGGL(lstm_fwd_fused_kernel<true>, dim3(B), dim3(256), lds, stream, x, w_ih, b_ih, b_hh, w_hh, hout, gates, cst, T);
     else hipLaunchKernelGGL(lstm_fwd_fused_kernel<false>, dim3(B), dim3(256), lds, stream, x, w_ih, b_ih, b_hh, w_hh, hout, gates, cst, T);
+    WM_CHECK_LAUNCH();
+    return 0;
+}
+
+int wm_lstm_fwd_tail(const float* xres, const float* y2, const float* sc2, const float* sh2, float* out, void* mask, const float* w_ih,
+                     const float* b_ih, const float* b_hh, const float* w_hh, float* hout, float* gates, float* cst, int B, int T,
+                     hipStream_t stream) {
+    if (B <= 0 || T < 32 || (T & 31) || !xres || !y2 || !sc2 || !sh2 || !out) return (int)hipErrorInvalidValue;
+    constexpr size_t lds = (size_t)2 * 32 * 257 * sizeof(float) + (size_t)3 * 32 * 72 * 2 + 128 * sizeof(float);
+    static wm::DevOnce done[2];
+    if (int rc = wm::lds_opt_in(reinterpret_cast<const void*>(lstm_fwd_ws_kernel<true, true>), lds, done[0])) return rc;
+    if (int rc = wm::lds_opt_in(reinterpret_cast<const void*>(lstm_fwd_ws_kernel<false, true>), lds, done[1])) return rc;
+    const LstmTailArgs<true> tl{y2, sc2, sh2, out, reinterpret_cast<unsigned*>(mask)};
+    if (gates && cst) hipLaunchKernelGGL((lstm_fwd_ws_kernel<true, true>), dim3(B), dim3(512), lds, stream, xres, w_ih, b_ih, b_hh, w_hh, hout, gates, cst, T, tl);
+    else hipLaunchKernelGGL((lstm_fwd_ws_kernel<false, true>), dim3(B), dim3(512), lds, stream, xres, w_ih, b_ih, b_hh, w_hh, hout, gates, cst, T, tl);
     WM_CHECK_LAUNCH();
     return 0;
 }
diff --git a/audio-watermarking-deep-learning-watermarks-for-authenticating-speech_amd/csrc/wm_common.hpp b/audio-watermarking-deep-learning-watermarks-for-authenticating-speech_amd/csrc/wm_common.hpp
--- a/audio-watermarking-deep-learning-watermarks-for-authenticating-speech_amd/csrc/wm_common.hpp
+++ b/audio-watermarking-deep-learning-watermarks-for-authenticating-speech_amd/csrc/wm_common.hpp
@@ -244,4 +244,15 @@
     __builtin_amdgcn_raw_buffer_store_b32(__builtin_bit_cast(unsigned, v), srd, (int)voff_bytes, (int)soff_bytes, 0);
 }
 
-}
+__device__ __forceinline__ unsigned sign_nibble(const float4& v) {
+    return ((v.x > 0.f) ? 1u : 0u) | ((v.y > 0.f) ? 2u : 0u) | ((v.z > 0.f) ? 4u : 0u) | ((v.w > 0.f) ? 8u : 0u);
+}
+__device__ __forceinline__ unsigned mask_merge8(unsigned m) {
+    m |= (unsigned)__builtin_amdgcn_update_dpp(0, (int)m, 0x128, 0xf, 0xf, true);
+    const auto r16 = __builtin_amdgcn_permlane16_swap(m, m, false, false);
+    m = r16[0] | r16[1];
+    const auto r32 = __builtin_amdgcn_permlane32_swap(m, m, false, false);
+    return r32[0] | r32[1];
+}
+
+}
diff --git a/audio-watermarking-deep-learning-watermarks-for-authenticating-speech_amd/modules.py b/audio-watermarking-deep-learning-watermarks-for-authenticating-speech_amd/modules.py
--- a/audio-watermarking-deep-learning-watermarks-for-authenticating-speech_amd/modules.py
+++ b/audio-watermarking-deep-learning-watermarks-for-authenticating-speech_amd/modules.py
@@ -63,8 +63,12 @@
         self.decoder = nn.Sequential(nn.ConvTranspose1d(64, 64, 7, padding=3), ResBlock(64), _Head1(64, 1, 1))
 
     def forward(self, s, message=None):
-        x = resblock_pair(self.encoder[1], self.encoder[2], self.encoder[0](s))
-        x = ops.LSTMFn.apply(x, self.lstm.weight_ih_l0, self.lstm.weight_hh_l0, self.lstm.bias_ih_l0, self.lstm.bias_hh_l0)
+        e1, e2, x = self.encoder[1], self.encoder[2], self.encoder[0](s)
+        lstm = (self.lstm.weight_ih_l0, self.lstm.weight_hh_l0, self.lstm.bias_ih_l0, self.lstm.bias_hh_l0)
+        if (e1.training and e2.training and not _hooked(self.encoder, e1, e2, self.lstm) and ops.tail_in_consumer_applies(x, lstm=True)):
+            x = ops.EncoderLSTMFn.apply(x, *_rb_args(e1), *_rb_args(e2), *lstm)
+        else:
+            x = ops.LSTMFn.apply(resblock_pair(e1, e2, x), *lstm)
         vec = None
         if self.message_bits > 0 and message is not None:
             if message.dim() != 1 or message.shape[0] != s.shape[0]:
diff --git a/audio-watermarking-deep-learning-watermarks-for-authenticating-speech_amd/ops.py b/audio-watermarking-deep-learning-watermarks-for-authenticating-speech_amd/ops.py
--- a/audio-watermarking-deep-learning-watermarks-for-authenticating-speech_amd/ops.py
+++ b/audio-watermarking-deep-learning-watermarks-for-authenticating-speech_amd/ops.py
@@ -277,6 +277,27 @@
     _HEADS["tail_in_head"] = bool(on)
 
 
+def read_tail_in_consumer(environ) -> bool:
+    return environ.get("WM_TAIL_IN_CONSUMER", "1") == "1"
+
+
+_TAILC = {"on": read_tail_in_consumer(os.environ)}
+
+
+def set_tail_in_consumer(on: bool):
+    _TAILC["on"] = bool(on)
+
+
+def _tail_in_consumer_launches(x, lstm: bool = False) -> bool:
+    ok = (_TAILC["on"] and x.is_cuda and x.dim() == 3 and x.shape[-1] % 128 == 0 and _CONV["bf16x6"] and _CONV["fwd_f16x3"]
+          and _CONV["schedule"] == 2)
+    return bool(ok and (not lstm or (_LSTM["fused"] and _LSTM["fwd_ws"])))
+
+
+def tail_in_consumer_applies(x, lstm: bool = False) -> bool:
+    return _tail_in_consumer_launches(x, lstm) and bool(pair_node_applies(x))
+
+
 def set_gconv_f16x3(on: bool):
     set_switch("gconv_f16x3", on)
 
@@ -356,8 +377,11 @@
     return wp
 
 
-def _resblock_fwd(x, params, training, want_grad, tail=True):
+def _resblock_fwd(x, params, training, want_grad, tail=True, pending=None):
     w1, b1, g1, be1, w2, b2, g2, be2, rm1, rv1, nbt1, rm2, rv2, nbt2 = params
+    if pending is not None:
+        px, py2, pcst = pending[0], pending[2], pending[4]
+        x, pmask = torch.empty_like(px), _tail_mask(px, want_grad)
     x = _frames(x, "ResBlock input", 64)
     B, _, T = x.shape
     dev, st = x.device, _stream()
@@ -367,7 +391,11 @@
     if training:
         y1, y2 = torch.empty_like(x), torch.empty_like(x)
         stats = _f32(NCU * 128, device=dev)
-        _conv3(x, None, w1, 0, None, None, None, b1, None, None, None, y1, stats, B, T, 0, 0)
+        if pending is not None:
+            lib.wm_conv64_bf_tail(_p(px), _p(py2), _p(pack_w64_h(w1, 0)), _p(pcst[4]), _p(pcst[5]), _p(b1), _p(x), _p(pmask), _p(y1),
+                                  _p(stats), B, T, st)
+        else:
+            _conv3(x, None, w1, 0, None, None, None, b1, None, None, None, y1, stats, B, T, 0, 0)
         lib.wm_bn_finalize(_p(stats), NCU, float(B * T), _p(g1), _p(be1), _p(rm1), _p(rv1), _p(nbt1), BN_MOMENTUM, BN_EPS,
                            _p(sc1), _p(sh1), _p(mu1), _p(is1), st)
         _conv3(y1, None, w2, 0, sc1, sh1, None, b2, None, None, None, y2, stats, B, T, 1, 0)
@@ -394,15 +422,16 @@
         y2 = torch.empty_like(x)
         _conv3(y1, None, w2, 0, sc1, sh1, None, b2, None, None, None, y2, None, B, T, 1, 0)
         mu1.copy_(rm1); is1.copy_(torch.rsqrt(rv1 + BN_EPS)); mu2.copy_(rm2); is2.copy_(torch.rsqrt(rv2 + BN_EPS))
+    more = () if pending is None else (pmask,)
     if not tail:
-        return None, (x, y1, y2, None, cst, w1, w2, g1, g2)
+        return (None, (x, y1, y2, None, cst, w1, w2, g1, g2)) + more
     if want_grad:
         mask = torch.empty(B * 64 * ((T + 31) // 32), dtype=torch.int32, device=dev)
         lib.wm_bn_add_relu_mask(_p(x), _p(y2), _p(sc2), _p(sh2), _p(out), _p(mask), B, T, st)
     else:
         mask = None
         lib.wm_bn_add_relu(_p(x), _p(y2), _p(sc2), _p(sh2), _p(out), B, T, st)
-    return out, (x, y1, y2, mask, cst, w1, w2, g1, g2)
+    return (out, (x, y1, y2, mask, cst, w1, w2, g1, g2)) + more
 
 
 class ResBlockFn(GradAwareFunction):
@@ -523,13 +552,22 @@
             and _CONV["fused_bwd"] and _CONV["mask_on_load"] and _CONV["pair_fold"] and not _ASYNC["on"])
 
 
+def _pair_fwd(x, p1, p2, training, want_grad, tail=True):
+    if training and _tail_in_consumer_launches(x):
+        _, first = _resblock_fwd(x, p1, True, want_grad, tail=False)
+        out, second, pmask = _resblock_fwd(None, p2, True, want_grad, tail=tail, pending=first)
+        return out, first[:3] + (pmask,) + first[4:], second
+    mid, first = _resblock_fwd(x, p1, training, want_grad)
+    out, second = _resblock_fwd(mid, p2, training, want_grad, tail=tail)
+    return out, first, second
+
+
 class ResBlockPairFn(GradAwareFunction):
 
     @staticmethod
     def forward(ctx, x, *args):
         p1, p2, training = args[:14], args[14:28], args[28]
-        mid, first = _resblock_fwd(x, p1, training, wants_grad(ctx))
-        out, second = _resblock_fwd(mid, p2, training, wants_grad(ctx))
+        out, first, second = _pair_fwd(x, p1, p2, training, wants_grad(ctx))
         ctx.save_for_backward(*(first + second))
         ctx.training = bool(training)
         return out
@@ -664,9 +702,8 @@
     def forward(ctx, x, message, *args):
         p1, p2, hw, hb = args[:14], args[14:28], args[28], args[29]
         want = wants_grad(ctx)
-        mid, first = _resblock_fwd(x, p1, True, want)
-        _, second = _resblock_fwd(mid, p2, True, want, tail=False)
-        y2, cst = second[2], second[4]
+        _, first, second = _pair_fwd(x, p1, p2, True, want, tail=False)
+        mid, y2, cst = second[0], second[2], second[4]
         R, _, T = mid.shape
         NO, B, dev = hw.shape[0], message.shape[0], mid.device
         out, mask = torch.empty_like(mid), _tail_mask(mid, want)
@@ -708,52 +745,95 @@
 
     @staticmethod
     def forward(ctx, x, w_ih, w_hh, b_ih, b_hh):
-        x = _frames(x, "LSTM input", 64)
-        B, _, T = x.shape
-        dev, st = x.device, _stream()
         need_grad = wants_grad(ctx)
-        h = torch.empty_like(x)
-        release_deferred_wgrads()
-        cst = _f32(B, T, 64, device=dev) if need_grad else None
-        if _LSTM["fused"] and T >= 8:
-            gates = _f32(B, T, 256, device=dev) if need_grad else None
-            lib.wm_lstm_fwd_fused(_p(x), _p(w_ih), _p(b_ih), _p(b_hh), _p(w_hh), _p(h), _p(gates), _p(cst), B, T, st)
-        else:
-            xp = _f32(B, T, 256, device=dev)
-            lib.wm_lstm_xproj(_p(x), _p(w_ih), _p(b_ih), _p(b_hh), _p(xp), B, T, st)
-            gates = xp if need_grad else None
-            lib.wm_lstm_fwd(_p(xp), _p(w_hh), _p(h), _p(gates), _p(cst), B, T, st)
+        h, saved = _lstm_fwd(x, w_ih, w_hh, b_ih, b_hh, need_grad)
         if need_grad:
             ctx.gdst = _gdst(w_ih, w_hh, b_ih, b_hh)
-            ctx.save_for_backward(x, h, gates, cst, w_ih, w_hh)
+            ctx.save_for_backward(*saved)
         return h
 
     @staticmethod
     def backward(ctx, dh):
-        x, h, gates, cst, w_ih, w_hh = ctx.saved_tensors
+        saved = ctx.saved_tensors
         _single_backward(ctx, "LSTMFn")
-        dh = dh.contiguous()
-        B, _, T = x.shape
-        dev, st = x.device, _stream()
-        dx = torch.empty_like(x)
-        release_deferred_wgrads()
-        dst, acc, launch = _wgrad_dst(ctx.gdst, dev, w_ih.shape, w_hh.shape, (256,), (256,))
-        if _LSTM["bwd_ws"] and not _LSTM["bwd_fused"] and T % 32 == 0 and T >= 64:
-            part = _f32(B * (256 * 128 + 256), device=dev)
-            lib.wm_lstm_bwd_wgrad(_p(gates), _p(cst), _p(dh), _p(w_hh), _p(x), _p(h), _p(part), *map(_p, dst), B, T, int(acc), st)
-            lib.wm_lstm_dx(_p(gates), _p(w_ih), _p(dx), B, T, st)
-            return (dx,) + ((None,) * 4 if acc else dst)
-        if _LSTM["bwd_fused"]:
-            lib.wm_lstm_bwd_fused(_p(gates), _p(cst), _p(dh), _p(w_hh), _p(w_ih), _p(dx), B, T, st)
-        else:
-            lib.wm_lstm_bwd(_p(gates), _p(cst), _p(dh), _p(w_hh), B, T, st)
-            lib.wm_lstm_dx(_p(gates), _p(w_ih), _p(dx), B, T, st)
-
-        def wg():
-            part = _f32(NCU * (256 * 128 + 256), device=dev)
-            lib.wm_lstm_wgrad(_p(gates), _p(x), _p(h), _p(part), *map(_p, dst), B, T, int(acc), _stream())
-        launch((gates, x, h), wg)
+        return _lstm_bwd(saved, ctx.gdst, dh)
+
+
+def _lstm_fwd(x, w_ih, w_hh, b_ih, b_hh, need_grad, tail=None):
+    if tail is not None:
+        xres, y2, sc2, sh2, mask = tail
+        x = torch.empty_like(xres)
+    x = _frames(x, "LSTM input", 64)
+    B, _, T = x.shape
+    dev, st = x.device, _stream()
+    h = torch.empty_like(x)
+    release_deferred_wgrads()
+    cst = _f32(B, T, 64, device=dev) if need_grad else None
+    if tail is not None:
+        gates = _f32(B, T, 256, device=dev) if need_grad else None
+        lib.wm_lstm_fwd_tail(_p(xres), _p(y2), _p(sc2), _p(sh2), _p(x), _p(mask), _p(w_ih), _p(b_ih), _p(b_hh), _p(w_hh), _p(h),
+                             _p(gates), _p(cst), B, T, st)
+    elif _LSTM["fused"] and T >= 8:
+        gates = _f32(B, T, 256, device=dev) if need_grad else None
+        lib.wm_lstm_fwd_fused(_p(x), _p(w_ih), _p(b_ih), _p(b_hh), _p(w_hh), _p(h), _p(gates), _p(cst), B, T, st)
+    else:
+        xp = _f32(B, T, 256, device=dev)
+        lib.wm_lstm_xproj(_p(x), _p(w_ih), _p(b_ih), _p(b_hh), _p(xp), B, T, st)
+        gates = xp if need_grad else None
+        lib.wm_lstm_fwd(_p(xp), _p(w_hh), _p(h), _p(gates), _p(cst), B, T, st)
+    return h, ((x, h, gates, cst, w_ih, w_hh) if need_grad else None)
+
+
+def _lstm_bwd(saved, gdst, dh):
+    x, h, gates, cst, w_ih, w_hh = saved
+    dh = dh.contiguous()
+    B, _, T = x.shape
+    dev, st = x.device, _stream()
+    dx = torch.empty_like(x)
+    release_deferred_wgrads()
+    dst, acc, launch = _wgrad_dst(gdst, dev, w_ih.shape, w_hh.shape, (256,), (256,))
+    if _LSTM["bwd_ws"] and not _LSTM["bwd_fused"] and T % 32 == 0 and T >= 64:
+        part = _f32(B * (256 * 128 + 256), device=dev)
+        lib.wm_lstm_bwd_wgrad(_p(gates), _p(cst), _p(dh), _p(w_hh), _p(x), _p(h), _p(part), *map(_p, dst), B, T, int(acc), st)
+        lib.wm_lstm_dx(_p(gates), _p(w_ih), _p(dx), B, T, st)
         return (dx,) + ((None,) * 4 if acc else dst)
+    if _LSTM["bwd_fused"]:
+        lib.wm_lstm_bwd_fused(_p(gates), _p(cst), _p(dh), _p(w_hh), _p(w_ih), _p(dx), B, T, st)
+    else:
+        lib.wm_lstm_bwd(_p(gates), _p(cst), _p(dh), _p(w_hh), B, T, st)
+        lib.wm_lstm_dx(_p(gates), _p(w_ih), _p(dx), B, T, st)
+
+    def wg():
+        part = _f32(NCU * (256 * 128 + 256), device=dev)
+        lib.wm_lstm_wgrad(_p(gates), _p(x), _p(h), _p(part), *map(_p, dst), B, T, int(acc), _stream())
+    launch((gates, x, h), wg)
+    return (dx,) + ((None,) * 4 if acc else dst)
+
+
+class EncoderLSTMFn(GradAwareFunction):
+
+    @staticmethod
+    def forward(ctx, x, *args):
+        p1, p2, (w_ih, w_hh, b_ih, b_hh) = args[:14], args[14:28], args[28:32]
+        want = wants_grad(ctx)
+        _, first, second = _pair_fwd(x, p1, p2, True, want, tail=False)
+        mid, y2, cst = second[0], second[2], second[4]
+        mask = _tail_mask(mid, want)
+        h, lsaved = _lstm_fwd(None, w_ih, w_hh, b_ih, b_hh, want, tail=(mid, y2, cst[4], cst[5], mask))
+        if want:
+            ctx.gdst = _gdst(w_ih, w_hh, b_ih, b_hh)
+            ctx.save_for_backward(*(first + second[:3] + (mask,) + second[4:] + lsaved))
+        return h
+
+    @staticmethod
+    def backward(ctx, dh):
+        sv = ctx.saved_tensors
+        _single_backward(ctx, "EncoderLSTMFn")
+        s1_, s2_ = sv[:9], sv[9:18]
+        lgrads = _lstm_bwd(sv[18:], ctx.gdst, dh)
+        dmid, grads2, fout = _resblock_bwd_fused(s2_, True, lgrads[0], fold=(s1_[3], s1_[2]))
+        dx, grads1, _ = _resblock_bwd_fused(s1_, True, dmid, pre=fout)
+        return (dx,) + grads1 + (None,) * 6 + grads2 + (None,) * 6 + lgrads[1:]
 
 
 _CHECK_INDEX = {"mode": {"1": "sync", "0": "off"}.get(os.environ.get("WM_CHECK_INDEX", "1"), os.environ.get("WM_CHECK_INDEX", "sync")),
diff --git a/include/wm_hip.h b/include/wm_hip.h
--- a/include/wm_hip.h
+++ b/include/wm_hip.h
@@ -19,6 +19,8 @@
 int wm_conv64_bf(const float* x, const float* x2, const void* wpb, const float* pa, const float* pb, const float* pc,
                  const float* bias, const float* e1, const float* ea, const float* eb, float* y, float* stats,
                  int B, int T, int pro, int epi, int arith, wm_stream_t stream);
+int wm_conv64_bf_tail(const float* x, const float* y2, const void* wpb_h, const float* sc2, const float* sh2, const float* bias,
+                      float* out, void* mask, float* y, float* stats, int B, int T, wm_stream_t stream);
 
 int wm_pack_w64_bf_scaled(const float* w, const float* row_scale, void* wpb, wm_stream_t stream);
 int wm_resblock_eval_bf(const float* x, const void* w1pb, const void* w2pb, const float* b1, const float* sc1, const float* sh1,
@@ -91,6 +93,9 @@
 int wm_lstm_fwd_fused(const float* x, const float* w_ih, const float* b_ih, const float* b_hh, const float* w_hh,
                       float* hout, float* gates, float* cst, int B, int T, wm_stream_t stream);
 int wm_set_lstm_fwd_wave_specialised(int on, wm_stream_t stream);
+int wm_lstm_fwd_tail(const float* xres, const float* y2, const float* sc2, const float* sh2, float* out, void* mask, const float* w_ih,
+                     const float* b_ih, const float* b_hh, const float* w_hh, float* hout, float* gates, float* cst, int B, int T,
+                     wm_stream_t stream);
 int wm_lstm_bwd(float* gates, const float* cst, const float* dh_out, const float* w_hh, int B, int T, wm_stream_t stream);
 int wm_lstm_dx(const float* da, const float* w_ih, float* dx, int B, int T, wm_stream_t stream);
 int wm_set_lstm_dx_bf16x6(int on, wm_stream_t stream);
```

New measurement: 5538 clips/s, median of 6. +1.7%, better.
